# eriksandstroem/Loopy-SLAM

Measured on AMD Instinct MI355X. Metric: rays/s (track+map, Replica room0 per-frame budget, 640x480 synthetic RGB-D), higher is better.
Workload: dtype f32 (decoder products as split products on the 16-bit matrix pipe: fp16x3 forward, bf16x6 / pre-scaled fp16x3 backward, fp32 accumulate; weight gradients on pre-scaled fp16x3 too); 1 GPU; Replica room0 budget: 40 track it x 1500 rays + 60 map it x 5000 rays per frame (24 geometry + 36 colour) on the frustum rows of the mapped frame, S=5, k=8, C=32, rel-pos colour MLP, N=99999 points laid down by radius-de-duplicated insertion (lk_add_points, r_add 0.04), 640x480 synthetic room

## Files before the change

### include/loopy_hip.h

```cpp
#ifndef LOOPY_HIP_H
#define LOOPY_HIP_H

#include <stdint.h>

#ifdef __cplusplus
extern "C" {
#endif

#define LK_ABI_VERSION 1
#define LK_K 8
#define LK_C 32
#define LK_S_MAX 8

#define LK_OK 0
#define LK_ERR_ARG (-1)
#define LK_ERR_HIP (-2)
#define LK_ERR_STATE (-3)
#define LK_ERR_RANGE (-4)

typedef struct lk_knn_s* lk_knn_t;

int lk_version(void);
const char* lk_last_error(void);

// ... 94 lines not shown
    float loss_w_color;
} lk_render_desc;

int64_t lk_render_act_floats(int32_t R, int32_t S, uint32_t flags);
int64_t lk_render_bwd_scratch_floats(int32_t R, int32_t S, uint32_t flags);
int lk_render_fwd(const lk_render_desc* d, void* stream);
int lk_render_bwd(const lk_render_desc* d, void* stream);

#define LK_TRACK_USE_COLOR   1
#define LK_TRACK_MEDIAN_MASK 2
int lk_loss_mapper(int32_t R, const float* depth, const float* color, const uint8_t* valid_ray,
                   const float* gt_depth, const float* gt_color, float w_color, int32_t use_color,
                   float* d_depth, float* d_color, float* out_loss, void* stream);
int lk_loss_tracker(int32_t R, const float* depth, const float* var, const float* color,
                    const float* gt_depth, const float* gt_color, float w_color, int32_t use_color,
                    float* d_depth, float* d_color, float* out_loss, float* scratch , void* stream);

#define LK_ADAM_MAX_SEG 16
typedef struct {
    float* p; float* g; float* m; float* v;
    int64_t n;
    float lr; int32_t step;
    const int32_t* row_index;
    int32_t row_len;
    int32_t zero_grad;
    int32_t p_f16;
    const uint8_t* row_flags;
    int32_t g_compact;
} lk_adam_seg;
int lk_adam_step(const lk_adam_seg* host_segs, int32_t n_seg, float beta1, float beta2, float eps, void* stream);

#define LK_EXPOSURE_MAX_F 32
#define LK_EXPOSURE_GRAD_FLOATS (1024 + 128 + 1536 + 12 + LK_EXPOSURE_MAX_F * 8)
int lk_exposure_fwd(const float* feats, const float* W1, const float* b1, const float* W2, const float* b2, int32_t F,
                    float* aff, float* hid, void* stream);
int lk_exposure_bwd(const float* feats, const float* W1, const float* W2, const float* hid, const float* g_aff, int32_t F,
                    float* g, void* stream);
int lk_loss_mapper_exposure(int32_t R, const float* depth, const float* logits, const uint8_t* valid_ray, const float* gt_depth,
                            const float* gt_color, const int32_t* frame_id, const float* aff, int32_t F, float w_color,
                            float* d_depth, float* d_logits, float* out_loss, float* g_aff, void* stream);

typedef struct lk_copy_seg {
    float* data;
    int64_t n;
    const int32_t* row_index;
    int32_t row_len;
} lk_copy_seg;
int lk_bucket_copy(const lk_copy_seg* host_segs, int32_t n_seg, float* bucket, int32_t unpack, void* stream);

int lk_rays_from_pose(const float* cam7, const float* pix_i, const float* pix_j, int32_t R,
                      float fx, float fy, float cx, float cy, float* rays_o, float* rays_d, void* stream);
int lk_gather_rays(const float* depth_stack, const float* color_stack, const float* c2w_stack, int32_t c2w_stride,
                   const float* r2_map_stack, const int32_t* frame_id, const int32_t* rnd, int32_t R,
                   int32_t H, int32_t W, int32_t H0, int32_t W0, int32_t w, float fx, float fy, float cx, float cy,
                   float* rays_o, float* rays_d, float* gt_depth, float* gt_color, float* pix_i, float* pix_j,
                   float* r2_ray, void* stream);
int lk_pose_bwd(const float* cam7, const float* pix_i, const float* pix_j, int32_t R,
                float fx, float fy, float cx, float cy, const float* g_rays_o, const float* g_rays_d,
                float* g_cam7, void* stream);
int lk_compact(const uint8_t* mask, int32_t n, int32_t* out_index, int32_t* out_count, void* stream);
int lk_compact_large(const uint8_t* mask, int32_t n, int32_t* out_index, int32_t* out_count, int32_t* block_scratch, void* stream);
int lk_touch_rows(const int32_t* nbr_idx, int64_t n, uint8_t* flags, int32_t N, void* stream);
int lk_knn_flag_rows(lk_knn_t knn, const uint8_t* flags, int64_t n, void* stream);
int lk_frustum_rows(const float* pos, int32_t N, const float* w2c12_host, const float* depth, int32_t H, int32_t W,
                    float fx, float fy, float cx, float cy, int32_t edge, float* scratch_depth, uint8_t* scratch_mask,
                    uint32_t* scratch_max, int32_t* out_index, int32_t* out_count, void* stream);
int lk_add_points(lk_knn_t knn, const float* rays_o, const float* rays_d, const float* gt_depth, int32_t n,
                  float r2_static, const float* r2_per_ray, float near_surface, float far_surface, int32_t n_add,
                  uint8_t* scratch_mask, int32_t* out_ray_index, int32_t* out_count, float* out_points, void* stream);
int lk_radius_maps(const float* color, int32_t H, int32_t W, double color_grad_threshold, double radius_add_max,
                   double radius_add_min, double radius_query_ratio, float* grad_mag, float* r2_add, float* r2_query, void* stream);
int lk_top_grad_pixels(const float* grad_mag, int32_t H, int32_t W, int32_t K, int32_t H0, int32_t H1, int32_t W0, int32_t W1,
                       const float* depth, int32_t depth_limit, int32_t* out_index, int32_t* out_count, void* stream);
int lk_inside_mask(const float* depth, int32_t n, uint8_t* mask, float* depth_filtered, float* out_thr,
                   uint32_t* scratch, void* stream);

typedef struct {
    float* feats;
    float* W1; float* b1; float* W2; float* b2;
    int32_t F;
    float* aff;
    float* hid;
    float* g_aff;
    float* g;
    float* adam;
    float lr_mlp;
    float lr_feat;
    int32_t feat_first, feat_count;
    float* bwd_scale;
} lk_exposure_desc;

typedef struct {
    lk_render_desc render;
    const float* depth_img;
    const float* color_img;
    const float* r2_map;
    int32_t H, W, H0, W0, w;
    float fx, fy, cx, cy;
    const int32_t* rnd;
    float* gt_color;
    float* pix_i; float* pix_j;
    float* thr;
    uint32_t* scratch_u32;
    float* loss_scratch;
    float* cam7;
    float* g_cam7;
    float* adam_mv;
    float lr_T, lr_q;
    float w_color; int32_t use_color;
    int32_t hist_post;
    float* hist;
    float* log;
    int32_t iters;
    float* work;
    const lk_exposure_desc* exposure;
} lk_track_desc;
int64_t lk_track_work_floats(int32_t R, int32_t S, int32_t iters);
int lk_track_frame(const lk_track_desc* d, void* stream);

#define LK_MAX_SPANS 8
typedef struct { int64_t offset, n; } lk_blob_span;
typedef struct {
    lk_render_desc render;
    const float* depth_stack; const float* color_stack; const float* c2w_stack; int32_t c2w_stride;
    const float* r2_map_stack;
    const int32_t* frame_id;
    const int32_t* rnd;
    int32_t H, W, H0, W0, w;
    float fx, fy, cx, cy;
    float* gt_color; float* thr; uint32_t* scratch_u32;
    float w_color;
    float* log;
    float* weights_rw;
    float* weights_frag_rw;
    float* geo_feats_rw; float* col_feats_rw;
    const int32_t* rows;
    int64_t n_rows;
    float* adam_rows;
    lk_blob_span geo_dec[LK_MAX_SPANS]; int32_t n_geo_dec;
    lk_blob_span col_dec[LK_MAX_SPANS]; int32_t n_col_dec;
    float* adam_dec;
    float lr[2][3];
    int32_t iters, n_geo_iters;
    float* work;
    const lk_exposure_desc* exposure;
    const float* grad_bucket;
    int64_t bucket_geo_dec[LK_MAX_SPANS], bucket_col_dec[LK_MAX_SPANS];
    int64_t bucket_geo_rows, bucket_col_rows;
    int32_t union_rows_flagged;
    int32_t it_offset;
    int32_t batches_ready;
    int32_t train_geo_decoder;
    int32_t signal_rows;
} lk_map_desc;
int64_t lk_map_work_floats(int32_t R, int32_t S, int32_t iters);
int lk_map_prepare(const lk_map_desc* d, void* stream);
int64_t lk_map_work_nbr_idx(int32_t R, int32_t S, int32_t iters);
int lk_map_frame(const lk_map_desc* d, int32_t it_begin, int32_t it_end, int32_t phases, void* stream);
int lk_map_wait_lists(const lk_map_desc* d, int32_t it, void* stream);
int lk_map_wait_rows(const lk_map_desc* d, void* stream);

int lk_wgrad_single(const float* A, int32_t lda, int32_t a_mode, const float* A2, int32_t lda2,
                    const float* B, int32_t ldb, int32_t N, int32_t K, int64_t rows,
                    float* dW, int32_t ldw, float* db, int32_t chunk, void* stream);

int lk_normals(lk_knn_t knn, const float* pos, int64_t N, float radius, const float* host_camera3,
               float* out_normals , uint8_t* out_valid , void* stream);
#define LK_ICP_POINT_TO_PLANE 0
#define LK_ICP_INFORMATION 1
#define LK_ICP_SUMS 32
int64_t lk_icp_scratch_floats(int64_t P);
int lk_icp_accumulate(lk_knn_t tgt, const float* tgt_pos, const float* tgt_normals, const uint8_t* tgt_valid, const float* src,
                      int64_t P, const float* host_T12, float max_dist, float tukey_k, int32_t mode, int32_t* out_corr,
                      float* scratch, int64_t scratch_floats, double* out_sums, void* stream);
int lk_apply_correction(float* pos, int64_t N, const int32_t* seg_id, const float* mats, int32_t n_seg, void* stream);

#define LK_VOXEL_AXIS_MAX 2097151
int lk_voxel_keys(const float* pos, int64_t N, const float* host_origin3, float voxel, int64_t* out_keys, void* stream);
int lk_voxel_heads(const int64_t* sorted_keys, int64_t N, uint8_t* out_head, void* stream);
int lk_voxel_downsample(const float* pos, int64_t N, const int64_t* order , const int32_t* starts ,
                        int32_t n_vox, float* out_centroids , void* stream);
int lk_knn_canonicalize(lk_knn_t knn, void* stream);
#define LK_FPFH_DIM 33
int lk_fpfh(lk_knn_t knn, const float* pos, const float* normals, const uint8_t* valid, int64_t N, float radius,
            float* out_spfh , float* out_fpfh , void* stream);
int lk_feature_match(const float* A, const uint8_t* validA, int64_t Na, const float* B, const uint8_t* validB, int64_t Nb,
                     int32_t* out_idx, float* out_d2, void* stream);
#define LK_RANSAC_BEST 20
int lk_ransac_gather(const float* src, const float* tgt, const int32_t* corr, int32_t M, float* out_cs, float* out_ct, void* stream);
int lk_ransac_hypotheses(const float* cs, const float* ct, int32_t M, uint64_t seed, uint64_t trial0, int32_t n_trials, float edge_ratio,
                         float dist_thr, int32_t* out_triples, uint8_t* out_ok, float* out_T, void* stream);
int lk_ransac_score(const float* cs, const float* ct, int32_t M, const float* T_all, const int32_t* survivors, const int32_t* n_survivors,
                    int32_t max_survivors, float dist_thr, int32_t* out_count, float* out_sum_d2, void* stream);
int lk_ransac_best(const int32_t* count, const float* sum_d2, const int32_t* survivors, const int32_t* n_survivors, const float* T_all,
                   uint64_t trial0, int32_t* best, void* stream);

int lk_tsdf_touch(const float* depth, int32_t H, int32_t W, const float* host_c2w16, float fx, float fy, float cx, float cy, int32_t stride,
                  float depth_trunc, float sdf_trunc, float voxel, int64_t* out_keys , void* stream);
int lk_tsdf_integrate(float* planes, const int64_t* slot_keys, int32_t n_slots, const int32_t* touched_slots, int32_t n_touched,
                      const float* depth, const float* color, int32_t H, int32_t W, const float* host_c2w16, float fx, float fy, float cx,
                      float cy, float voxel, float sdf_trunc, float depth_trunc, void* stream);
int lk_mc_mark(const float* planes, const int32_t* sorted_slots, const int32_t* nbr, int32_t n_blocks, uint8_t* out_case, uint8_t* out_ntri,
               uint8_t* edge_flag, void* stream);
int lk_mc_vertices(const float* planes, const int64_t* slot_keys, const int32_t* sorted_slots, const int32_t* nbr, int32_t n_blocks,
                   const int32_t* vert_index, int32_t V, float voxel, float* out_pos , float* out_col , void* stream);
int lk_mc_triangles(const int32_t* sorted_slots, const int32_t* nbr, int32_t n_blocks, const uint8_t* cube_case, const int32_t* tri_end,
                    const int32_t* vert_index, int32_t V, int32_t* out_tri , void* stream);

int lk_nearest(lk_knn_t knn, const float* queries, int64_t P, float max_dist, float* out_d2, int32_t* out_idx, void* stream);
int lk_mesh_areas(const float* verts, int64_t V, const int32_t* faces, int64_t F, float* out_area, void* stream);
int lk_mesh_sample(const float* verts, int64_t V, const int32_t* faces, int64_t F, const double* cum_area, uint64_t seed, int64_t S,
                   float* out_pos , int32_t* out_face , float* out_bary , void* stream);
int lk_mesh_cull(const float* points, int64_t N, const float* w2c, int32_t n_poses, int32_t H, int32_t W, float fx, float fy, float cx, float cy,
                 uint8_t* seen, void* stream);
int lk_mesh_depth_setup(const float* verts, int64_t V, const int32_t* faces, int64_t F, const float* host_w2c12, int32_t H, int32_t W, float fx,
                        float fy, float cx, float cy, float near, float far, float* out_rec, int32_t* out_box, int32_t* out_ntiles,
                        float* out_depth , void* stream);
int lk_mesh_depth_raster(const float* rec, const int32_t* box, const int32_t* tile_end, int64_t F, int64_t T, int32_t H, int32_t W, float fx,
                         float fy, float cx, float cy, float near, float far, float* depth , void* stream);

int lk_profile_begin(const char* names);
int lk_set_serial(int32_t on);
int lk_streams_init(void);
int lk_profile_end(char* buf, int cap);
int lk_debug_occupancy(int32_t out[5]);
int lk_debug_side_delay(int32_t us);

#ifdef __cplusplus
}
#endif
#endif
```

### loopy_slam_amd/_ffi.py

```python
import ctypes as C
import os

_HERE = os.path.dirname(os.path.abspath(__file__))
LIB_PATH = os.path.join(_HERE, 'libloopyhip.so')

LK_K = 8
LK_C = 32
LK_S_MAX = 8

FLAG_STAGE_COLOR = 1 << 0
FLAG_TRACKER = 1 << 1
FLAG_REL_POS = 1 << 2
FLAG_COLOR_LOGITS = 1 << 3
FLAG_SAVE_ACT = 1 << 4
FLAG_GRAD_FEATS = 1 << 5
FLAG_GRAD_WEIGHTS = 1 << 6
FLAG_GRAD_RAYS = 1 << 7
FLAG_ALL_DEPTH_POS = 1 << 8
FLAG_ZERO_ABSENT = 1 << 9
FLAG_MAPPER_LOSS = 1 << 10
FLAG_Z_GIVEN = 1 << 12
FLAG_FEATS_F16 = 1 << 13
FLAG_UNIT_LOSS_GRADS = 1 << 11
FLAG_EMBED_GRADS_ONLY = 1 << 14
FLAG_GRAD_GEO_DECODER = 1 << 15
FLAG_CHECK_RANGE = 1 << 16
STATUS_WEIGHT_RANGE, STATUS_ACT_RANGE = 1, 2
ERR_RANGE = -4

EXPOSURE_MAX_F = 32
ICP_POINT_TO_PLANE, ICP_INFORMATION, ICP_SUMS = 0, 1, 32
FPFH_DIM, RANSAC_BEST = 33, 20
ADAM_MAX_SEG = 16

_fp = C.c_void_p


class WeightEntry(C.Structure):
    _fields_ = [('name', C.c_char * 64), ('offset', C.c_int64), ('rows', C.c_int32), ('cols', C.c_int32),
                ('ld', C.c_int32), ('col_split', C.c_int32), ('col_shift', C.c_int32)]


class RenderDesc(C.Structure):
    _fields_ = [
        ('R', C.c_int32), ('S', C.c_int32), ('stats_chunk', C.c_int32), ('flags', C.c_uint32),
        ('rays_o', _fp), ('rays_d', _fp), ('gt_depth', _fp), ('r2_ray', _fp),
        ('knn', _fp), ('pos', _fp), ('geo_feats', _fp), ('col_feats', _fp), ('weights', _fp), ('weights_frag', _fp),
        ('affine', _fp), ('noise_geo', _fp), ('noise_col', _fp),
        ('near_surface', C.c_float), ('far_surface', C.c_float), ('near_end', C.c_float), ('coef', C.c_float),
        ('r2_static', C.c_float), ('min_nn', C.c_int32),
        ('depth', _fp), ('var', _fp), ('color', _fp), ('valid_ray', _fp),
        ('z', _fp), ('nbr_idx', _fp), ('nbr_w', _fp), ('nbr_count', _fp), ('c_geo', _fp), ('c_col', _fp),
        ('raw', _fp), ('far_stats', _fp), ('act', _fp),
        ('d_depth', _fp), ('d_var', _fp), ('d_color', _fp),
        ('g_geo_feats', _fp), ('g_col_feats', _fp), ('g_weights', _fp), ('g_rays_o', _fp), ('g_rays_d', _fp),
        ('g_affine', _fp), ('grad_row_mask', _fp), ('bwd_scratch', _fp), ('bwd_scratch_cap', C.c_int64),
        ('loss_gt_color', _fp), ('loss_out4', _fp), ('loss_w_color', C.c_float),
    ]


class AdamSeg(C.Structure):
    _fields_ = [('p', _fp), ('g', _fp), ('m', _fp), ('v', _fp), ('n', C.c_int64), ('lr', C.c_float),
                ('step', C.c_int32), ('row_index', _fp), ('row_len', C.c_int32), ('zero_grad', C.c_int32), ('p_f16', C.c_int32),
                ('row_flags', _fp), ('g_compact', C.c_int32)]


class CopySeg(C.Structure):
    _fields_ = [('data', _fp), ('n', C.c_int64), ('row_index', _fp), ('row_len', C.c_int32)]


MAX_SPANS = 8


class BlobSpan(C.Structure):
    _fields_ = [('offset', C.c_int64), ('n', C.c_int64)]


EXPOSURE_GRAD_FLOATS = 1024 + 128 + 1536 + 12 + EXPOSURE_MAX_F * 8


class ExposureDesc(C.Structure):
    _fields_ = [('feats', _fp), ('W1', _fp), ('b1', _fp), ('W2', _fp), ('b2', _fp), ('F', C.c_int32),
                ('aff', _fp), ('hid', _fp), ('g_aff', _fp), ('g', _fp), ('adam', _fp),
                ('lr_mlp', C.c_float), ('lr_feat', C.c_float), ('feat_first', C.c_int32), ('feat_count', C.c_int32), ('bwd_scale', _fp)]


class TrackDesc(C.Structure):
    _fields_ = [
        ('render', RenderDesc),
        ('depth_img', _fp), ('color_img', _fp), ('r2_map', _fp),
        ('H', C.c_int32), ('W', C.c_int32), ('H0', C.c_int32), ('W0', C.c_int32), ('w', C.c_int32),
        ('fx', C.c_float), ('fy', C.c_float), ('cx', C.c_float), ('cy', C.c_float),
        ('rnd', _fp), ('gt_color', _fp), ('pix_i', _fp), ('pix_j', _fp), ('thr', _fp), ('scratch_u32', _fp), ('loss_scratch', _fp),
        ('cam7', _fp), ('g_cam7', _fp), ('adam_mv', _fp),
        ('lr_T', C.c_float), ('lr_q', C.c_float), ('w_color', C.c_float), ('use_color', C.c_int32), ('hist_post', C.c_int32),
        ('hist', _fp), ('log', _fp), ('iters', C.c_int32), ('work', _fp), ('exposure', C.POINTER(ExposureDesc)),
    ]


class MapDesc(C.Structure):
    _fields_ = [
        ('render', RenderDesc),
        ('depth_stack', _fp), ('color_stack', _fp), ('c2w_stack', _fp), ('c2w_stride', C.c_int32), ('r2_map_stack', _fp),
        ('frame_id', _fp), ('rnd', _fp),
        ('H', C.c_int32), ('W', C.c_int32), ('H0', C.c_int32), ('W0', C.c_int32), ('w', C.c_int32),
        ('fx', C.c_float), ('fy', C.c_float), ('cx', C.c_float), ('cy', C.c_float),
        ('gt_color', _fp), ('thr', _fp), ('scratch_u32', _fp),
        ('w_color', C.c_float), ('log', _fp),
        ('weights_rw', _fp), ('weights_frag_rw', _fp), ('geo_feats_rw', _fp), ('col_feats_rw', _fp),
        ('rows', _fp), ('n_rows', C.c_int64), ('adam_rows', _fp),
        ('geo_dec', BlobSpan * MAX_SPANS), ('n_geo_dec', C.c_int32),
        ('col_dec', BlobSpan * MAX_SPANS), ('n_col_dec', C.c_int32),
        ('adam_dec', _fp),
        ('lr', (C.c_float * 3) * 2),
        ('iters', C.c_int32), ('n_geo_iters', C.c_int32), ('work', _fp), ('exposure', C.POINTER(ExposureDesc)),
        ('grad_bucket', _fp), ('bucket_geo_dec', C.c_int64 * MAX_SPANS), ('bucket_col_dec', C.c_int64 * MAX_SPANS),
        ('bucket_geo_rows', C.c_int64), ('bucket_col_rows', C.c_int64),
        ('union_rows_flagged', C.c_int32), ('it_offset', C.c_int32), ('batches_ready', C.c_int32), ('train_geo_decoder', C.c_int32), ('signal_rows', C.c_int32),
    ]


class LoopyError(RuntimeError):
    pass


class LoopyLib:

    def __init__(self, path):
        if not os.path.exists(path):
            raise LoopyError(f'{path} not found: build it with `python loopy_slam_amd/csrc/build.py` '
                             f'(or __graft_entry__.build()); there is no CPU fallback')
        self.path = path
        import torch
        self.dll = C.CDLL(path)
        d = self.dll
        d.lk_version.restype = C.c_int
        d.lk_last_error.restype = C.c_char_p
        d.lk_knn_create.argtypes = [C.c_float, C.c_int64, C.c_int64, C.POINTER(C.c_void_p)]
        d.lk_knn_destroy.argtypes = [C.c_void_p]
        d.lk_knn_build.argtypes = [C.c_void_p, _fp, C.c_int64, C.c_void_p]
        d.lk_knn_append.argtypes = [C.c_void_p, _fp, C.c_int64, C.c_void_p]
        d.lk_knn_size.argtypes = [C.c_void_p]
        d.lk_knn_size.restype = C.c_int64
        d.lk_knn_query.argtypes = [C.c_void_p, _fp, C.c_int64, C.c_float, _fp, _fp, _fp, _fp, C.c_void_p]
        d.lk_weight_layout.argtypes = [C.POINTER(WeightEntry), C.c_int]
        d.lk_weight_blob_floats.restype = C.c_int64
        d.lk_weight_frag_floats.restype = C.c_int64
        d.lk_weights_repack.argtypes = [_fp, _fp, C.c_void_p]
        d.lk_render_act_floats.argtypes = [C.c_int32, C.c_int32, C.c_uint32]
        d.lk_render_act_floats.restype = C.c_int64
        d.lk_render_fwd.argtypes = [C.POINTER(RenderDesc), C.c_void_p]
        for name, argtypes, restype in (
            ('lk_render_bwd_scratch_floats', [C.c_int32, C.c_int32, C.c_uint32], C.c_int64),
            ('lk_render_bwd', [C.POINTER(RenderDesc), C.c_void_p], C.c_int),
            ('lk_loss_mapper', [C.c_int32, _fp, _fp, _fp, _fp, _fp, C.c_float, C.c_int32, _fp, _fp, _fp, C.c_void_p], C.c_int),
            ('lk_loss_tracker', [C.c_int32, _fp, _fp, _fp, _fp, _fp, C.c_float, C.c_int32, _fp, _fp, _fp, _fp, C.c_void_p], C.c_int),
            ('lk_adam_step', [C.POINTER(AdamSeg), C.c_int32, C.c_float, C.c_float, C.c_float, C.c_void_p], C.c_int),
            ('lk_bucket_copy', [C.POINTER(CopySeg), C.c_int32, C.c_void_p, C.c_int32, C.c_void_p], C.c_int),
            ('lk_exposure_fwd', [_fp] * 5 + [C.c_int32, _fp, _fp, C.c_void_p], C.c_int),
            ('lk_exposure_bwd', [_fp] * 5 + [C.c_int32, _fp, C.c_void_p], C.c_int),
            ('lk_loss_mapper_exposure', [C.c_int32] + [_fp] * 7 + [C.c_int32, C.c_float, _fp, _fp, _fp, _fp, C.c_void_p], C.c_int),
            ('lk_rays_from_pose', [_fp, _fp, _fp, C.c_int32, C.c_float, C.c_float, C.c_float, C.c_float, _fp, _fp, C.c_void_p], C.c_int),
            ('lk_pose_bwd', [_fp, _fp, _fp, C.c_int32, C.c_float, C.c_float, C.c_float, C.c_float, _fp, _fp, _fp, C.c_void_p], C.c_int),
            ('lk_gather_rays', [_fp, _fp, _fp, C.c_int32, _fp, _fp, _fp, C.c_int32, C.c_int32, C.c_int32, C.c_int32, C.c_int32,
                                C.c_int32, C.c_float, C.c_float, C.c_float, C.c_float, _fp, _fp, _fp, _fp, _fp, _fp, _fp,
                                C.c_void_p], C.c_int),
            ('lk_frustum_rows', [_fp, C.c_int32, C.POINTER(C.c_float), _fp, C.c_int32, C.c_int32, C.c_float, C.c_float, C.c_float,
                                 C.c_float, C.c_int32, _fp, _fp, _fp, _fp, _fp, C.c_void_p], C.c_int),
            ('lk_add_points', [C.c_void_p, _fp, _fp, _fp, C.c_int32, C.c_float, _fp, C.c_float, C.c_float, C.c_int32,
                               _fp, _fp, _fp, _fp, C.c_void_p], C.c_int),
            ('lk_radius_maps', [_fp, C.c_int32, C.c_int32, C.c_double, C.c_double, C.c_double, C.c_double, _fp, _fp, _fp, C.c_void_p], C.c_int),
            ('lk_top_grad_pixels', [_fp, C.c_int32, C.c_int32, C.c_int32, C.c_int32, C.c_int32, C.c_int32, C.c_int32, _fp, C.c_int32,
                                    _fp, _fp, C.c_void_p], C.c_int),
            ('lk_wgrad_single', [_fp, C.c_int32, C.c_int32, _fp, C.c_int32, _fp, C.c_int32, C.c_int32, C.c_int32, C.c_int64,
                                 _fp, C.c_int32, _fp, C.c_int32, C.c_void_p], C.c_int),
            ('lk_profile_begin', [C.c_char_p], C.c_int),
            ('lk_profile_end', [C.c_char_p, C.c_int], C.c_int),
            ('lk_compact', [_fp, C.c_int32, _fp, _fp, C.c_void_p], C.c_int),
            ('lk_set_serial', [C.c_int32], C.c_int),
            ('lk_streams_init', [], C.c_int),
            ('lk_debug_occupancy', [C.POINTER(C.c_int32)], C.c_int),
            ('lk_debug_side_delay', [C.c_int32], C.c_int),
            ('lk_weights_repack_checked', [_fp, _fp, C.c_void_p], C.c_int),
            ('lk_status_peek', [C.POINTER(C.c_uint32)], C.c_int),
            ('lk_status_sync', [C.c_void_p, C.POINTER(C.c_uint32)], C.c_int),
            ('lk_status_clear', [], C.c_int),
            ('lk_track_work_floats', [C.c_int32, C.c_int32, C.c_int32], C.c_int64),
            ('lk_map_work_floats', [C.c_int32, C.c_int32, C.c_int32], C.c_int64),
            ('lk_map_work_nbr_idx', [C.c_int32, C.c_int32, C.c_int32], C.c_int64),
            ('lk_track_frame', [C.POINTER(TrackDesc), C.c_void_p], C.c_int),
            ('lk_map_frame', [C.POINTER(MapDesc), C.c_int32, C.c_int32, C.c_int32, C.c_void_p], C.c_int),
            ('lk_map_prepare', [C.POINTER(MapDesc), C.c_void_p], C.c_int),
            ('lk_inside_mask', [_fp, C.c_int32, _fp, _fp, _fp, _fp, C.c_void_p], C.c_int),
            ('lk_compact_large', [_fp, C.c_int32, _fp, _fp, _fp, C.c_void_p], C.c_int),
            ('lk_touch_rows', [_fp, C.c_int64, _fp, C.c_int32, C.c_void_p], C.c_int),
            ('lk_knn_flag_rows', [C.c_void_p, _fp, C.c_int64, C.c_void_p], C.c_int),
            ('lk_map_wait_lists', [C.POINTER(MapDesc), C.c_int32, C.c_void_p], C.c_int),
            ('lk_map_wait_rows', [C.POINTER(MapDesc), C.c_void_p], C.c_int),
            ('lk_normals', [C.c_void_p, _fp, C.c_int64, C.c_float, C.POINTER(C.c_float), _fp, _fp, C.c_void_p], C.c_int),
            ('lk_icp_scratch_floats', [C.c_int64], C.c_int64),
            ('lk_icp_accumulate', [C.c_void_p, _fp, _fp, _fp, _fp, C.c_int64, C.POINTER(C.c_float), C.c_float, C.c_float, C.c_int32, _fp,
                                   _fp, C.c_int64, _fp, C.c_void_p], C.c_int),
            ('lk_apply_correction', [_fp, C.c_int64, _fp, _fp, C.c_int32, C.c_void_p], C.c_int),
            ('lk_voxel_keys', [_fp, C.c_int64, C.POINTER(C.c_float), C.c_float, _fp, C.c_void_p], C.c_int),
            ('lk_voxel_heads', [_fp, C.c_int64, _fp, C.c_void_p], C.c_int),
            ('lk_voxel_downsample', [_fp, C.c_int64, _fp, _fp, C.c_int32, _fp, C.c_void_p], C.c_int),
            ('lk_knn_canonicalize', [C.c_void_p, C.c_void_p], C.c_int),
            ('lk_fpfh', [C.c_void_p, _fp, _fp, _fp, C.c_int64, C.c_float, _fp, _fp, C.c_void_p], C.c_int),
            ('lk_feature_match', [_fp, _fp, C.c_int64, _fp, _fp, C.c_int64, _fp, _fp, C.c_void_p], C.c_int),
            ('lk_ransac_gather', [_fp, _fp, _fp, C.c_int32, _fp, _fp, C.c_void_p], C.c_int),
            ('lk_ransac_hypotheses', [_fp, _fp, C.c_int32, C.c_uint64, C.c_uint64, C.c_int32, C.c_float, C.c_float, _fp, _fp, _fp,
                                      C.c_void_p], C.c_int),
            ('lk_ransac_score', [_fp, _fp, C.c_int32, _fp, _fp, _fp, C.c_int32, C.c_float, _fp, _fp, C.c_void_p], C.c_int),
            ('lk_ransac_best', [_fp, _fp, _fp, _fp, _fp, C.c_uint64, _fp, C.c_void_p], C.c_int),
            ('lk_tsdf_touch', [_fp, C.c_int32, C.c_int32, C.POINTER(C.c_float), C.c_float, C.c_float, C.c_float, C.c_float, C.c_int32,
                               C.c_float, C.c_float, C.c_float, _fp, C.c_void_p], C.c_int),
            ('lk_tsdf_integrate', [_fp, _fp, C.c_int32, _fp, C.c_int32, _fp, _fp, C.c_int32, C.c_int32, C.POINTER(C.c_float), C.c_float,
                                   C.c_float, C.c_float, C.c_float, C.c_float, C.c_float, C.c_float, C.c_void_p], C.c_int),
            ('lk_mc_mark', [_fp, _fp, _fp, C.c_int32, _fp, _fp, _fp, C.c_void_p], C.c_int),
            ('lk_mc_vertices', [_fp, _fp, _fp, _fp, C.c_int32, _fp, C.c_int32, C.c_float, _fp, _fp, C.c_void_p], C.c_int),
            ('lk_mc_triangles', [_fp, _fp, C.c_int32, _fp, _fp, _fp, C.c_int32, _fp, C.c_void_p], C.c_int),
            ('lk_nearest', [C.c_void_p, _fp, C.c_int64, C.c_float, _fp, _fp, C.c_void_p], C.c_int),
            ('lk_mesh_areas', [_fp, C.c_int64, _fp, C.c_int64, _fp, C.c_void_p], C.c_int),
            ('lk_mesh_sample', [_fp, C.c_int64, _fp, C.c_int64, _fp, C.c_uint64, C.c_int64, _fp, _fp, _fp, C.c_void_p], C.c_int),
            ('lk_mesh_cull', [_fp, C.c_int64, _fp, C.c_int32, C.c_int32, C.c_int32, C.c_float, C.c_float, C.c_float, C.c_float, _fp,
                              C.c_void_p], C.c_int),
            ('lk_mesh_depth_setup', [_fp, C.c_int64, _fp, C.c_int64, C.POINTER(C.c_float), C.c_int32, C.c_int32, C.c_float, C.c_float,
                                     C.c_float, C.c_float, C.c_float, C.c_float, _fp, _fp, _fp, _fp, C.c_void_p], C.c_int),
            ('lk_mesh_depth_raster', [_fp, _fp, _fp, C.c_int64, C.c_int64, C.c_int32, C.c_int32, C.c_float, C.c_float, C.c_float, C.c_float,
                                      C.c_float, C.c_float, _fp, C.c_void_p], C.c_int),
        ):
            if hasattr(d, name):
                fn = getattr(d, name)
                fn.argtypes = argtypes
                fn.restype = restype
        if d.lk_version() != 1:
            raise LoopyError(f'{path}: ABI version {d.lk_version()} != 1')

    def check(self, rc, what=''):
        if rc != 0:
            raise LoopyError(f'{what} failed (rc={rc}): {self.dll.lk_last_error().decode()}')

    def weight_layout(self):
        n = self.dll.lk_weight_layout(None, 0)
        arr = (WeightEntry * n)()
        self.dll.lk_weight_layout(arr, n)
        return [dict(name=e.name.decode(), offset=e.offset, rows=e.rows, cols=e.cols, ld=e.ld,
                     col_split=e.col_split, col_shift=e.col_shift) for e in arr]

    def blob_floats(self):
        return int(self.dll.lk_weight_blob_floats())


_LIB = None


def get_lib():
    global _LIB
    if _LIB is None:
        import torch
        if not torch.cuda.is_available():
            raise LoopyError('loopy_slam_amd needs a HIP device (MI355X); none is visible and there is no CPU fallback')
        _LIB = LoopyLib(LIB_PATH)
    return _LIB


def ptr(t):
    return 0 if t is None else t.data_ptr()
```

### loopy_slam_amd/csrc/lk_adam_dev.h

```cpp
#pragma once
#include "lk_common.h"
#include "lk_kernels.h"

__device__ __forceinline__ float lk_adam_elem(float p, float g, float& m, float& v, float b1, float b2, float eps, float step_size, float bc2_sqrt) {
    m = m * b1 + (1.0f - b1) * g;
    v = v * b2 + (1.0f - b2) * (g * g);
    const float denom = sqrtf(v) / bc2_sqrt + eps;
    return p - step_size * (m / denom);
}

__device__ __forceinline__ void lk_adam_one(const AdamSegDev& S, long long i, long long e, float b1, float b2, float eps) {
    const float g = S.g[S.g_compact ? i : e];
    float m = S.m[i], v = S.v[i];
    if (S.p_f16) {
        _Float16* ph = reinterpret_cast<_Float16*>(S.p) + e;
        *ph = (_Float16)lk_adam_elem((float)*ph, g, m, v, b1, b2, eps, S.step_size, S.bc2_sqrt);
    } else {
        S.p[e] = lk_adam_elem(S.p[e], g, m, v, b1, b2, eps, S.step_size, S.bc2_sqrt);
    }
    S.m[i] = m;
    S.v[i] = v;
    if (S.zero_grad && !S.g_compact) S.g[e] = 0.0f;
}
__device__ __forceinline__ void lk_adam_seg_flagged(const AdamSegDev& S, float b1, float b2, float eps, int bx, int gx) {
    const int lane = (int)threadIdx.x & 63;
    const long long n_rows = S.n / S.row_len;
    const long long wave = (long long)bx * 4 + ((int)threadIdx.x >> 6), n_waves = (long long)gx * 4;
    const bool pair = S.row_len <= 32;
    int RW = 64;
    while (RW > 2 && n_rows < n_waves * RW) RW >>= 1;
    for (long long r0 = wave * RW; r0 < n_rows; r0 += n_waves * RW) {
        const bool on = lane < RW && r0 + lane < n_rows && S.row_flags[r0 + lane] != 0;
        unsigned long long mask = __ballot(on);
        while (mask) {
            const int ra = __ffsll((long long)mask) - 1;
            mask &= mask - 1;
            int rb = -1;
            if (pair && mask) { rb = __ffsll((long long)mask) - 1; mask &= mask - 1; }
            const int half = lane >> 5;
            const int row = pair ? (half ? rb : ra) : ra;
            const int k = pair ? (lane & 31) : lane;
            if (row >= 0 && k < S.row_len) {
                const long long e = (r0 + row) * S.row_len + k;
                lk_adam_one(S, e, e, b1, b2, eps);
            }
        }
    }
}
__device__ __forceinline__ void lk_adam_seg_block(const AdamSegDev& S, float b1, float b2, float eps, int bx, int gx) {
    if (S.row_flags) { lk_adam_seg_flagged(S, b1, b2, eps, bx, gx); return; }
    for (long long i = (long long)bx * 256 + threadIdx.x; i < S.n; i += (long long)gx * 256) {
        long long e = i;
        if (S.row_index) {
            const long long row = i / S.row_len;
            e = (long long)S.row_index[row] * S.row_len + (i - row * S.row_len);
        }
        lk_adam_one(S, i, e, b1, b2, eps);
    }
}
```

### loopy_slam_amd/csrc/lk_api.hip

```cpp
#include "lk_common.h"
#include "lk_kernels.h"

#include <stdarg.h>
#include <stdio.h>
#include <string.h>
#include <stdlib.h>

using namespace lkw;

static thread_local char g_err[512] = "";

void lk_set_error(const char* fmt, ...) {
    va_list ap;
    va_start(ap, fmt);
    vsnprintf(g_err, sizeof(g_err), fmt, ap);
    va_end(ap);
}

extern "C" int lk_version(void) { return LK_ABI_VERSION; }

namespace {
struct StatusWord { volatile unsigned* host = nullptr; unsigned* dev = nullptr; bool tried = false; };
StatusWord& status_word() {
    static StatusWord w;
// ... 416 lines not shown
    SideStream& ss = side_stream();
    LkFeatScatterArgs fs;
    seg_args(d, P, fs);
    if (gf && !(skip & LK_SEG_SORTED)) {
        const int rc2 = seg_sort_async(d, P, false, st);
        if (rc2 != LK_OK) return rc2;
    }

    LkCompositeBwdArgs cb;
    cb.R = d->R; cb.S = d->S; cb.min_nn = d->min_nn; cb.coef = d->coef;
    cb.raw = d->raw; cb.z = d->z; cb.nbr_count = d->nbr_count; cb.gt_depth = d->gt_depth;
    cb.d_depth = d->d_depth; cb.d_var = d->d_var; cb.d_color = color ? d->d_color : nullptr;
    cb.d_raw = S0 + L.d_raw; cb.keep_depth = (flags & LK_FLAG_Z_GIVEN) ? 1 : 0;
    const bool cb_inline = !(skip & LK_SKIP_COMPOSITE_BWD) && !(gw && (flags & LK_FLAG_GRAD_GEO_DECODER));
    if (!(skip & LK_SKIP_COMPOSITE_BWD) && !cb_inline) lk_launch_composite_bwd(cb, st);

    const bool fuse_small = (skip & LK_FUSE_SMALL) && relpos && gr && !gw && !gf && lk_cdiv(P, 32) <= LK_DEEP_MAX_TILES;
    bool fuse_rb = false;
    LkRelposBwdArgs rb_fused;
    LkDecodeBwdArgs db;
    db.R = d->R; db.S = d->S; db.P = P; db.flags = flags;
    db.rays_o = d->rays_o; db.rays_d = d->rays_d; db.z = d->z;
    db.W = d->weights; db.Wfrag = d->weights_frag; db.affine = d->affine;
    db.act = d->act; db.raw = d->raw; db.d_raw = S0 + L.d_raw;
    db.dc_geo = S0 + L.dc_geo; db.dc_col = S0 + L.dc_col; db.dy_col = S0 + L.dy_col; db.dlogit = S0 + L.dlogit;
    db.dp_embed = S0 + L.dp_embed; db.dp_embed_col = S0 + L.dp_embed_col; db.g_weights = d->g_weights; db.g_affine = d->g_affine; db.g_affine_part = S0 + L.aff_part; db.part_bg = S0 + L.part_bg;
    db.live_rays = ex ? ex->live_rays : nullptr;
    db.dscale = ex ? ex->dscale : nullptr;
    db.tl_n_part = 0;
    memset(&db.tl, 0, sizeof(db.tl));
    db.cb_on = cb_inline ? 1 : 0; db.cb = cb;
    db.ml_on = 0; db.ml_row_part = nullptr;
    memset(&db.ml, 0, sizeof(db.ml));
    if ((skip & LK_COMPOSITE_IN_BWD) && (flags & LK_FLAG_MAPPER_LOSS)) {
        LK_REQUIRE(ex && ex->loss_rows && d->d_depth && d->d_color && d->loss_gt_color && (skip & LK_SKIP_COMPOSITE_BWD),
                   "lk_render_bwd: the composite inside the decoder backward needs loss_rows, loss_gt_color, d_depth, d_color");
        LkCompositeArgs& ca = db.ml;
        ca.R = d->R; ca.S = d->S; ca.min_nn = d->min_nn; ca.coef = d->coef;
        ca.raw = d->raw; ca.z = d->z; ca.nbr_count = d->nbr_count; ca.gt_depth = d->gt_depth;
        ca.depth = d->depth; ca.var = d->var; ca.color = d->color; ca.valid_ray = d->valid_ray;
        ca.keep_depth = (flags & LK_FLAG_Z_GIVEN) ? 1 : 0;
        ca.gt_color = d->loss_gt_color; ca.w_color = d->loss_w_color; ca.use_color = color ? 1 : 0;
        ca.d_depth = const_cast<float*>(d->d_depth); ca.d_color = const_cast<float*>(d->d_color);
        db.ml_on = 1; db.ml_row_part = ex->loss_rows;
    }
    if (ex && ex->track_loss) {
        LK_REQUIRE((flags & LK_FLAG_GRAD_RAYS) != 0 && ex->track_n_part > 0, "lk_render_bwd: the inline tracker loss needs ray gradients");
        db.tl = *ex->track_loss; db.tl_n_part = ex->track_n_part;
    }
    lk_launch_decode_bwd(db, st);
    if (gw && (flags & LK_FLAG_GRAD_GEO_DECODER)) {
        LK_REQUIRE(!(flags & LK_FLAG_EMBED_GRADS_ONLY), "lk_render_bwd: GRAD_GEO_DECODER does not combine with EMBED_GRADS_ONLY");
        rc = lk_launch_geo_wgrad(P, d->S, d->rays_o, d->rays_d, d->z, d->weights, d->act, d->c_geo, S0 + L.d_raw, S0 + L.geo_part, d->g_weights, st,
                                 ex ? ex->live_rays : nullptr);
        if (rc != LK_OK) return rc;
    }
    if (color && d->affine && d->g_affine && !(skip & LK_SKIP_AFF_REDUCE)) lk_launch_reduce_partials(S0 + L.aff_part, lk_cdiv(P, 32), 12, d->g_affine, st);
    const bool gwf = gw && !(flags & LK_FLAG_EMBED_GRADS_ONLY);
    const bool defer = gwf && color && (!relpos || lk_relpos_fused(flags));
    LkWgradArgs wdef;
    wdef.n_units = 0; wdef.part = nullptr;
    const bool bg_rides = gw && !defer && gf;
    if (gw && !defer && !bg_rides) lk_launch_reduce_partials(S0 + L.part_bg, lk_cdiv(lk_cdiv(P, 32), 4), 288, d->g_weights + G_EB, st);

    const bool dw2_rides = gf && gwf && relpos && lk_relpos_fused(flags);
    const bool forked = gwf && color && ss.ok;
    const bool split = forked && defer && ex && ex->split_reduce && ex->step && ex->step->n_span > 0 && ex->split_frag && ex->split_master;
    if (ex && ex->split_done) *ex->split_done = split ? 1 : 0;
    hipStream_t wst = st;
    if (forked) {
        (void)hipEventRecord(ss.fork, st);
        (void)hipStreamWaitEvent(ss.st, ss.fork, 0);
        wst = ss.st;
    }
    if (gwf && color) {
        const float* act_h = d->act + (size_t)P * (LK_ACT_GEO_A + LK_ACT_COL_A);
        const float* act_e = d->act + (size_t)P * (LK_ACT_GEO_A + LK_ACT_COL_A + LK_ACT_COL_H);
        const float* dy = S0 + L.dy_col;
        float* G = d->g_weights;
        LkWgradArgs wa;
        memset(&wa, 0, sizeof(wa));
        int nj = 0;
        const int w_off[5] = {C_W0, C_W1, C_W2, C_W3, C_W4}, b_off[5] = {C_B0, C_B1, C_B2, C_B3, C_B4};
        const int w_ld[5] = {EC, HC, HC, EC + HC, HC};
        auto fc_from = [&](LkWgradJob& J, int src, int layer, const float* Wsrc, int rows_u, int ldw, int off) {
            J.k_aux = J.K;
            if (J.B2) { J.B3 = d->c_col; J.ldb3 = LK_C; J.k_split2 = J.K; }
            else { J.B2 = d->c_col; J.ldb2 = LK_C; J.k_split = J.K; }
            J.K += CF;
            LkFcPost& F = wa.fc[wa.n_fc++];
            F.src_job = src; F.rows_u = rows_u; F.ldw = ldw; F.off = off; F.W = Wsrc;
            F.dU = G + C_U0 + layer * C_USTRIDE; F.du = F.dU + a64(HC * CF);
        };
        for (int i = 0; i < 5; ++i) {
            LkWgradJob& J = wa.job[nj++];
            J.A = dy + LK_COL_LAYER(P, i); J.lda = 128; J.a_mode = 0;
            if (i == 0) { J.B = act_e; J.ldb = LK_ACT_COL_E; }
            else if (i == 3) { J.B = act_e; J.ldb = LK_ACT_COL_E; J.B2 = act_h + LK_COL_LAYER(P, 2); J.ldb2 = 128; J.k_split = EC; }
            else { J.B = act_h + LK_COL_LAYER(P, i - 1); J.ldb = 128; }
            J.N = HC; J.K = w_ld[i]; J.rows = P; J.dW = G + w_off[i]; J.ldw = w_ld[i]; J.db = G + b_off[i];
            if (i >= 1) fc_from(J, nj - 1, i - 1, d->weights + w_off[i], HC, w_ld[i], i == 3 ? EC : 0);
        }
        {
            LkWgradJob& J = wa.job[nj++];
            J.A = S0 + L.dlogit; J.lda = 4; J.a_mode = 0;
            J.B = act_h + LK_COL_LAYER(P, 4); J.ldb = 128;
            J.N = 3; J.K = HC; J.rows = P; J.dW = G + C_WO; J.ldw = HC; J.db = G + C_BO;
            fc_from(J, nj - 1, 4, d->weights + C_WO, 3, HC, 0);
        }
        wa.n_jobs = nj; wa.chunk = 0; wa.part = S0 + L.wg_part;
        wa.h16 = (flags & LK_FLAG_UNIT_LOSS_GRADS) && !gr ? 1 : 0;
        wa.live_rays = ex ? ex->live_rays : nullptr; wa.S = d->S; wa.dscale = ex ? ex->dscale : nullptr;
        if (forked && g_side_delay_us > 0) hipLaunchKernelGGL(k_spin_us, dim3(1), dim3(64), 0, wst, (long long)g_side_delay_us * 100);
        lk_launch_wgrad(wa, P, wst, defer ? &wdef : nullptr);
        if (split) {
            LkBwdReduceArgs rt;
            memset(&rt, 0, sizeof(rt));
            lk_launch_bwd_reduce(wdef, rt, false, wst, ex->step, false);
            lk_launch_repack_trunk(ex->step->w_next, ex->split_master, ex->split_frag, wst);
        }
    }

    if (relpos) {
        LkRelposBwdArgs rb;
        rb.R = d->R; rb.S = d->S; rb.P = P; rb.min_nn = d->min_nn; rb.flags = flags;
        rb.rays_o = d->rays_o; rb.rays_d = d->rays_d; rb.z = d->z; rb.pos = d->pos; rb.col_feats = d->col_feats;
        rb.nbr_idx = d->nbr_idx; rb.nbr_w = d->nbr_w; rb.nbr_count = d->nbr_count;
        rb.W = d->weights; rb.Wfrag = d->weights_frag; rb.dc_col = S0 + L.dc_col;
        rb.g_col_feats = d->g_col_feats; rb.g_weights = d->g_weights;
        rb.dw_rel = S0 + L.dw_rel; rb.dp_rel = S0 + L.dp_rel; rb.rows = S0 + L.rows; rb.w_eff = S0 + L.w_eff;
        rb.dfeat = S0 + L.dfeat;
        rb.part_br = S0 + L.part_br; rb.hbar = S0 + L.hbar; rb.w_sum = S0 + L.w_sum; rb.dw1_part = S0 + L.dw1_part;
        rb.live_rays = (ex && lk_relpos_fused(flags)) ? ex->live_rays : nullptr;
        fuse_rb = fuse_small;
        if (fuse_rb) rb_fused = rb;
        else lk_launch_relpos_bwd(rb, st);
        if (forked && !lk_relpos_fused(flags)) { (void)hipEventRecord(ss.mid, st); (void)hipStreamWaitEvent(wst, ss.mid, 0); }
        if (gw && !defer) lk_launch_reduce_partials(S0 + L.part_br, lk_relpos_fused(flags) ? lk_relpos_bwd_parts(P) : lk_cdiv(lk_cdiv(P, 4), 4), 32,
                                                    d->g_weights + R_EB, st);
    }

    if (gf) {
        fs.dc_geo = S0 + L.dc_geo; fs.dc_col = (color && !relpos) ? S0 + L.dc_col : nullptr; fs.dfeat = relpos ? S0 + L.dfeat : nullptr;
        fs.g_geo_feats = d->g_geo_feats; fs.g_col_feats = d->g_col_feats;
        if (ex && ex->seg_list) { fs.seg_list = ex->seg_list; fs.seg_total = ex->seg_total; }
        else if (ss.ok) (void)hipStreamWaitEvent(st, ss.link, 0);
        fs.act_flag = ex ? ex->act_flag : nullptr;
        if (bg_rides) { fs.red_part = S0 + L.part_bg; fs.red_n = lk_cdiv(lk_cdiv(P, 32), 4); fs.red_width = 288; fs.red_out = d->g_weights + G_EB; }
        if (dw2_rides) {
            fs.dw2_dc = S0 + L.dc_col; fs.dw2_w_sum = S0 + L.w_sum; fs.dw2_hbar = S0 + L.hbar; fs.dw2_part = S0 + L.dw2_part;
            fs.dw2_blocks = lk_dw2_parts(P); fs.dw2_live = ex ? ex->live_rays : nullptr; fs.dw2_S = d->S;
        }
        if (ex && ex->xstep) { fs.x_on = 1; fs.x = *ex->xstep; }
        lk_launch_feat_scatter(fs, st);
        if (ex && ex->signal_rows) {
            const int rc3 = rows_event_record(st);
            if (rc3 != LK_OK) return rc3;
        }
    }
    if (gr) {
        LkInterpBwdArgs ib;
        ib.R = d->R; ib.S = d->S; ib.P = P; ib.min_nn = d->min_nn; ib.flags = flags;
        ib.rays_o = d->rays_o; ib.rays_d = d->rays_d; ib.z = d->z; ib.r2_ray = d->r2_ray; ib.r2_static = d->r2_static;
        ib.pos = d->pos; ib.geo_feats = d->geo_feats; ib.col_feats = d->col_feats;
        ib.nbr_idx = d->nbr_idx; ib.nbr_w = d->nbr_w; ib.nbr_count = d->nbr_count;
        ib.dc_geo = S0 + L.dc_geo; ib.dc_col = S0 + L.dc_col;
        ib.dw_rel = relpos ? S0 + L.dw_rel : nullptr;
        ib.dp_embed = S0 + L.dp_embed; ib.dp_embed_col = color ? S0 + L.dp_embed_col : nullptr; ib.dp_rel = relpos ? S0 + L.dp_rel : nullptr;
        ib.g_geo_feats = d->g_geo_feats; ib.g_col_feats = d->g_col_feats; ib.dp_total = S0 + L.dp_total;
        ib.pose_part = ex ? ex->pose_part : nullptr;
        if (ex) { ib.pix_i = ex->pix_i; ib.pix_j = ex->pix_j; ib.fx = ex->fx; ib.fy = ex->fy; ib.cx = ex->cx; ib.cy = ex->cy; }
        else { ib.pix_i = ib.pix_j = nullptr; ib.fx = ib.fy = 1.0f; ib.cx = ib.cy = 0.0f; }
        if (fuse_rb) lk_launch_relpos_interp_bwd(rb_fused, ib, st, (flags & LK_FLAG_UNIT_LOSS_GRADS) && d->affine == nullptr);
        else lk_launch_interp_bwd(ib, st, (ex && !gf) ? ex->xstep : nullptr, ex ? ex->xstep_part : nullptr, ex ? ex->xstep_n_part : 0);
    }
    if (gr && !(skip & LK_SKIP_RAYS_BWD)) {
        LkRaysBwdArgs rr;
        rr.R = d->R; rr.S = d->S; rr.z = d->z; rr.dp_total = S0 + L.dp_total; rr.g_rays_o = d->g_rays_o; rr.g_rays_d = d->g_rays_d;
        lk_launch_rays_bwd(rr, st);
    }
    if (gwf && relpos) {
        float* G = d->g_weights;
        if (lk_relpos_fused(flags)) {
            LkRelposBwdArgs rb;
            memset(&rb, 0, sizeof(rb));
            rb.P = P; rb.S = d->S; rb.dc_col = S0 + L.dc_col; rb.w_sum = S0 + L.w_sum; rb.hbar = S0 + L.hbar; rb.dw1_part = S0 + L.dw1_part;
            rb.live_rays = ex ? ex->live_rays : nullptr;
            if (!dw2_rides) lk_launch_dw2_hbar(rb, S0 + L.dw2_part, st);
        } else {
            LkWgradArgs wr;
            memset(&wr, 0, sizeof(wr));
            const float* rows = S0 + L.rows;
            LkWgradJob& J1 = wr.job[0];
            J1.A = rows; J1.lda = 192; J1.a_mode = 0; J1.B = rows + 128; J1.ldb = 192;
            J1.N = HC; J1.K = KR; J1.rows = 8 * P; J1.dW = G + R_W1; J1.ldw = KRP; J1.db = G + R_B1;
            LkWgradJob& J2 = wr.job[1];
            J2.A = S0 + L.dc_col; J2.lda = LK_C; J2.a_mode = 2; J2.A2 = S0 + L.w_sum; J2.lda2 = 1;
            J2.B = S0 + L.hbar; J2.ldb = 128;
            J2.N = CF; J2.K = HC; J2.rows = P; J2.dW = G + R_W2; J2.ldw = HC; J2.db = G + R_B2;
            wr.n_jobs = 2; wr.chunk = 0; wr.part = S0 + L.wg_part;
            lk_launch_wgrad(wr, 8 * P, wst);
        }
    }
    if (forked) {
        LK_HIP_TRY(hipEventRecord(ss.join, wst));
        if (!split) LK_HIP_TRY(hipStreamWaitEvent(st, ss.join, 0));
    }
    if (defer) {
        float* G = d->g_weights;
        LkBwdReduceArgs r;
        memset(&r, 0, sizeof(r));
        const bool with_rp = relpos;
        if (with_rp) {
            r.part1 = S0 + L.dw1_part; r.n1 = lk_relpos_bwd_parts(P); r.part2 = S0 + L.dw2_part; r.n2 = lk_dw2_parts(P);
            r.dW1 = G + R_W1; r.db1 = G + R_B1; r.dW2 = G + R_W2; r.db2 = G + R_B2;
            r.part_br = S0 + L.part_br; r.n_br = lk_relpos_bwd_parts(P); r.out_br = G + R_EB;
        }
        r.part_bg = S0 + L.part_bg; r.n_bg = lk_cdiv(lk_cdiv(P, 32), 4); r.out_bg = G + G_EB;
        if (split) {
            LkWgradArgs none;
            memset(&none, 0, sizeof(none));
            lk_launch_bwd_reduce(none, r, with_rp, st, ex->step, true);
        } else lk_launch_bwd_reduce(wdef, r, with_rp, st, ex ? ex->step : nullptr);
    }
    LK_LAUNCH_CHECK();
    return LK_OK;
}

extern "C" int lk_wgrad_single(const float* A, int32_t lda, int32_t a_mode, const float* A2, int32_t lda2,
                               const float* B, int32_t ldb, int32_t N, int32_t K, int64_t rows,
                               float* dW, int32_t ldw, float* db, int32_t chunk, void* stream_) {
    LK_REQUIRE(A && B && dW && N > 0 && N <= 128 && K > 0 && K <= 192 && rows >= 0 && chunk >= 32, "lk_wgrad_single: bad arguments");
    LK_REQUIRE((N % 4 == 0 || lda >= ((N + 3) / 4) * 4) && K % 4 == 0 && lda % 4 == 0 && ldb % 4 == 0, "lk_wgrad_single: rows must be float4-addressable");
    if (rows == 0) return LK_OK;
    LkWgradArgs wa;
    memset(&wa, 0, sizeof(wa));
    LkWgradJob& J = wa.job[0];
    J.A = A; J.lda = lda; J.a_mode = a_mode; J.A2 = A2; J.lda2 = lda2; J.B = B; J.ldb = ldb;
    J.N = N; J.K = K; J.rows = (int)rows; J.dW = dW; J.ldw = ldw; J.db = db;
    wa.n_jobs = 1; wa.chunk = chunk;
    lk_launch_wgrad(wa, (int)rows, (hipStream_t)stream_);
    LK_LAUNCH_CHECK();
    return LK_OK;
}

#include <vector>
#include <string>
namespace {
const char* kKernelNames[LKK_COUNT] = {"k_depth_stats", "k_sample_interp", "k_relpos_fwd", "k_decode_fwd", "k_composite",
                                       "k_composite_bwd", "k_decode_bwd", "k_relpos_bwd", "k_interp_bwd", "k_rays_bwd", "k_wgrad", "k_feat_gather", "k_decode_bwd_track"};
struct ProfState {
    bool on = false;
    bool enabled[LKK_COUNT] = {};
    std::vector<hipEvent_t> ev0[LKK_COUNT], ev1[LKK_COUNT];
};
ProfState g_prof;
}

void lk_prof_before(int kid, hipStream_t st) {
    if (!g_prof.on || !g_prof.enabled[kid]) return;
    hipEvent_t e0, e1;
    if (hipEventCreate(&e0) != hipSuccess || hipEventCreate(&e1) != hipSuccess) return;
    g_prof.ev0[kid].push_back(e0);
    g_prof.ev1[kid].push_back(e1);
    (void)hipEventRecord(e0, st);
}
void lk_prof_after(int kid, hipStream_t st) {
    if (!g_prof.on || !g_prof.enabled[kid] || g_prof.ev1[kid].empty()) return;
    (void)hipEventRecord(g_prof.ev1[kid].back(), st);
}

extern "C" int lk_profile_begin(const char* names) {
    LK_REQUIRE(names != nullptr, "lk_profile_begin: NULL names");
    const std::string s(names);
    for (int k = 0; k < LKK_COUNT; ++k) {
        g_prof.enabled[k] = (s == "*") || (("," + s + ",").find(std::string(",") + kKernelNames[k] + ",") != std::string::npos);
        g_prof.ev0[k].clear();
        g_prof.ev1[k].clear();
    }
    g_prof.on = true;
    return LK_OK;
}

extern "C" int lk_profile_end(char* buf, int cap) {
    g_prof.on = false;
    std::string out;
    for (int k = 0; k < LKK_COUNT; ++k) {
        double total = 0.0;
        const size_t n = g_prof.ev0[k].size();
        for (size_t i = 0; i < n; ++i) {
            float ms = 0.0f;
            (void)hipEventSynchronize(g_prof.ev1[k][i]);
            if (hipEventElapsedTime(&ms, g_prof.ev0[k][i], g_prof.ev1[k][i]) == hipSuccess) total += ms;
            (void)hipEventDestroy(g_prof.ev0[k][i]);
            (void)hipEventDestroy(g_prof.ev1[k][i]);
        }
        g_prof.ev0[k].clear();
        g_prof.ev1[k].clear();
        if (n) {
            char line[160];
            snprintf(line, sizeof(line), "%s %zu %.6f\n", kKernelNames[k], n, total);
            out += line;
        }
    }
    if (buf && cap > 0) {
        strncpy(buf, out.c_str(), (size_t)cap - 1);
// ... 5 lines not shown
```

### loopy_slam_amd/csrc/lk_bwd2.hip

```cpp
#include "lk_common.h"
#include "lk_kernels.h"
#include "lk_adam_dev.h"
#include "lk_exposure_dev.h"

using namespace lkw;

LK_CHAIN_DEFINE(bwd2)

__device__ __forceinline__ void interp_bwd_block(const LkInterpBwdArgs& a, int block) {
    const int sub = (int)threadIdx.x & 7;
    const int p_raw = block * 32 + ((int)threadIdx.x >> 3);
    const bool live = p_raw < a.P;
    const int pidx = live ? p_raw : a.P - 1;
    const bool has = a.nbr_count[pidx] >= a.min_nn;
    const bool color = (a.flags & LK_FLAG_STAGE_COLOR) != 0;
    const bool relpos = (a.flags & LK_FLAG_REL_POS) != 0;
    const bool do_col = color && !relpos;
    int id[LK_K];
    float w[LK_K];
    {
        const int4 i0 = *reinterpret_cast<const int4*>(a.nbr_idx + (size_t)pidx * LK_K);
        const int4 i1 = *reinterpret_cast<const int4*>(a.nbr_idx + (size_t)pidx * LK_K + 4);
        const float4 w0 = *reinterpret_cast<const float4*>(a.nbr_w + (size_t)pidx * LK_K);
        const float4 w1 = *reinterpret_cast<const float4*>(a.nbr_w + (size_t)pidx * LK_K + 4);
        id[0] = i0.x; id[1] = i0.y; id[2] = i0.z; id[3] = i0.w; id[4] = i1.x; id[5] = i1.y; id[6] = i1.z; id[7] = i1.w;
        w[0] = w0.x; w[1] = w0.y; w[2] = w0.z; w[3] = w0.w; w[4] = w1.x; w[5] = w1.y; w[6] = w1.z; w[7] = w1.w;
    }
    const float4 dcg = *reinterpret_cast<const float4*>(a.dc_geo + (size_t)pidx * LK_C + sub * 4);
    float4 dcc = make_float4(0.f, 0.f, 0.f, 0.f);
    if (do_col) dcc = *reinterpret_cast<const float4*>(a.dc_col + (size_t)pidx * LK_C + sub * 4);
    if (!(a.flags & LK_FLAG_GRAD_RAYS)) return;
    float dwn[LK_K];
#pragma unroll
    for (int j = 0; j < LK_K; ++j) {
        float part = 0.0f;
        if (has && w[j] != 0.0f) {
            const float4 g = lk_feat4(a.geo_feats, (a.flags & LK_FLAG_FEATS_F16) != 0, (size_t)id[j] * LK_C + sub * 4);
            part = dcg.x * g.x + dcg.y * g.y + dcg.z * g.z + dcg.w * g.w;
            if (do_col) {
                const float4 c = lk_feat4(a.col_feats, (a.flags & LK_FLAG_FEATS_F16) != 0, (size_t)id[j] * LK_C + sub * 4);
                part += dcc.x * c.x + dcc.y * c.y + dcc.z * c.z + dcc.w * c.w;
            }
        }
        part = lk_sum8<true>(part);
        if (color && relpos && a.dw_rel && has) part += a.dw_rel[(size_t)pidx * LK_K + j];
        dwn[j] = part;
    }
    LK_STAMPW(7);
    const int r = pidx / a.S;
    const float z = a.z[pidx];
    const float px = lk_madd_rn(a.rays_o[3 * r], a.rays_d[3 * r], z);
    const float py = lk_madd_rn(a.rays_o[3 * r + 1], a.rays_d[3 * r + 1], z);
    const float pz = lk_madd_rn(a.rays_o[3 * r + 2], a.rays_d[3 * r + 2], z);
    const float r2 = a.r2_ray ? a.r2_ray[r] : a.r2_static;
    float dpx = 0.0f, dpy = 0.0f, dpz = 0.0f;
    if (has) {
        float wr[LK_K], ex[LK_K], ey[LK_K], ez[LK_K];
        float S = 0.0f, dot = 0.0f;
#pragma unroll
        for (int j = 0; j < LK_K; ++j) {
            wr[j] = 0.0f; ex[j] = ey[j] = ez[j] = 0.0f;
            if (id[j] >= 0) {
                const float x = a.pos[3 * (size_t)id[j]], y = a.pos[3 * (size_t)id[j] + 1], zz = a.pos[3 * (size_t)id[j] + 2];
                const float D = lk_dist2(px, py, pz, x, y, zz);
                if (D <= r2) { wr[j] = 1.0f / (D + 1e-10f); ex[j] = x - px; ey[j] = y - py; ez[j] = zz - pz; }
            }
            S += wr[j];
            dot += dwn[j] * w[j];
        }
        const float invS = 1.0f / fmaxf(S, 1e-12f);
#pragma unroll
        for (int j = 0; j < LK_K; ++j) {
            if (wr[j] != 0.0f) {
                const float dw = (dwn[j] - dot) * invS;
                const float dD = -wr[j] * wr[j] * dw;
                dpx += dD * (-2.0f) * ex[j]; dpy += dD * (-2.0f) * ey[j]; dpz += dD * (-2.0f) * ez[j];
            }
        }
    }
    if (live && sub == 0) {
        if (a.dp_embed) { const float4 e = *reinterpret_cast<const float4*>(a.dp_embed + (size_t)pidx * 4); dpx += e.x; dpy += e.y; dpz += e.z; }
        if (color && a.dp_embed_col) { const float4 e = *reinterpret_cast<const float4*>(a.dp_embed_col + (size_t)pidx * 4); dpx += e.x; dpy += e.y; dpz += e.z; }
        if (color && relpos && a.dp_rel) { const float4 e = *reinterpret_cast<const float4*>(a.dp_rel + (size_t)pidx * 4); dpx += e.x; dpy += e.y; dpz += e.z; }
        *reinterpret_cast<float4*>(a.dp_total + (size_t)pidx * 4) = make_float4(dpx, dpy, dpz, 0.0f);
    }
    LK_STAMPW(8);
    if (a.pose_part) {
        __shared__ float s_pp[4][12];
        float v[12];
        const bool mine = live && sub == 0;
        const float d0 = mine ? (a.pix_i[r] - a.cx) / a.fx : 0.0f, d1 = mine ? -(a.pix_j[r] - a.cy) / a.fy : 0.0f, d2 = mine ? -1.0f : 0.0f;
        const float gx = mine ? dpx : 0.0f, gy = mine ? dpy : 0.0f, gz = mine ? dpz : 0.0f;
        const float zx = gx * z, zy = gy * z, zz = gz * z;
        v[0] = zx * d0; v[1] = zx * d1; v[2] = zx * d2; v[3] = zy * d0; v[4] = zy * d1; v[5] = zy * d2; v[6] = zz * d0; v[7] = zz * d1; v[8] = zz * d2;
        v[9] = gx; v[10] = gy; v[11] = gz;
#pragma unroll
        for (int q = 0; q < 12; ++q) {
#pragma unroll
            for (int o = 32; o >= 8; o >>= 1) v[q] += __shfl_xor(v[q], o);
        }
        const int wv = (int)threadIdx.x >> 6;
        if (lk_lane() == 0) {
#pragma unroll
            for (int q = 0; q < 12; ++q) s_pp[wv][q] = v[q];
        }
        __syncthreads();
        if (threadIdx.x < 12) a.pose_part[(size_t)block * 12 + threadIdx.x] = (s_pp[0][threadIdx.x] + s_pp[1][threadIdx.x]) + (s_pp[2][threadIdx.x] + s_pp[3][threadIdx.x]);
    }
    LK_STAMPW(9);
}
__global__ __launch_bounds__(256) void k_interp_bwd(LkInterpBwdArgs a) { interp_bwd_block(a, (int)blockIdx.x); }
__global__ __launch_bounds__(256) void k_interp_bwd_x(LkInterpBwdArgs a, ExposureStepArgs xa, const float* __restrict__ part, int n_part) {
    if (blockIdx.x + 1 == gridDim.x) { lk_exposure_step_body(xa, part, n_part); return; }
    interp_bwd_block(a, (int)blockIdx.x);
}

__global__ __launch_bounds__(256) void k_seg_count(LkFeatScatterArgs a) {
    const long long row = (long long)blockIdx.x * 256 + (int)threadIdx.x;
    if (row >= (long long)a.P * LK_K) return;
    const int y = (int)blockIdx.y;
    const long long grow = (long long)y * a.P * LK_K + row;
    const int s = (int)(row >> 3);
    const int idx = a.nbr_idx[grow];
    int rk = -1;
    const bool skipped = a.live_rays && s >= a.live_rays[y] * a.S;
    if (!skipped && idx >= 0 && a.nbr_w[grow] != 0.0f && a.nbr_count[(size_t)y * a.P + s] >= a.min_nn && (!a.row_mask || a.row_mask[idx])) {
        const int key = a.key_of ? a.key_of[idx] : idx;
        if (key >= 0) rk = atomicAdd(a.seg_cnt + (size_t)y * a.cnt_stride + key, 1);
    }
    a.seg_rank[grow] = rk;
}
__global__ __launch_bounds__(256) void k_seg_place(LkFeatScatterArgs a) {
    const long long row = (long long)blockIdx.x * 256 + (int)threadIdx.x;
    if (row >= (long long)a.P * LK_K) return;
    const int y = (int)blockIdx.y;
    const long long base = (long long)y * a.P * LK_K;
    const int32_t* __restrict__ off = a.seg_off + (size_t)y * a.cnt_stride;
    const int rk = a.seg_rank[base + row];
    if (rk >= 0) {
        const int idx = a.nbr_idx[base + row];
        a.seg_list[base + off[a.key_of ? a.key_of[idx] : idx] + rk] = (int)row;
    }
    if (row == 0 && a.seg_total) a.seg_total[y] = off[a.N];
}

__global__ __launch_bounds__(256) void k_seg_order(LkFeatScatterArgs a) {
    const long long i = (long long)blockIdx.x * 256 + (int)threadIdx.x;
    const int y = (int)blockIdx.y;
    const int32_t* __restrict__ off = a.seg_off + (size_t)y * a.cnt_stride;
    if (i >= off[a.N]) return;
    const long long base = (long long)y * a.P * LK_K;
    const int32_t* __restrict__ tmp = a.seg_tmp + base;
    const int row = tmp[i];
    const int idx = a.nbr_idx[base + row];
    const int key = a.key_of ? a.key_of[idx] : idx;
    const int s = off[key], e = off[key + 1];
    int rk = 0;
    for (int j = s; j < e; ++j) rk += tmp[j] < row;
    a.seg_list[base + s + rk] = row;
}

#define LK_DW2_LDS_SAMPLES 32
__device__ __forceinline__ void dw2_body(const float* __restrict__ dc, const float* __restrict__ w_sum, const float* __restrict__ hbar,
                                         int P_all, const int32_t* __restrict__ live_rays, int S, float* __restrict__ part, int bx, int nb) {
    const int P = live_rays ? min(P_all, *live_rays * S) : P_all;
    __shared__ __attribute__((aligned(16))) float s_h[LK_DW2_LDS_SAMPLES][128];
    __shared__ float s_a[LK_DW2_LDS_SAMPLES][33];
    const int t = (int)threadIdx.x, n = t >> 3, k0 = 16 * (t & 7);
    float acc[16], bsum = 0.0f;
#pragma unroll
    for (int i = 0; i < 16; ++i) acc[i] = 0.0f;
    for (int s0 = bx * 64; s0 < P; s0 += nb * 64) {
        for (int half = 0; half < 64; half += LK_DW2_LDS_SAMPLES) {
            const int ns = min(LK_DW2_LDS_SAMPLES, P - s0 - half);
            if (ns <= 0) break;
            __syncthreads();
#pragma unroll
            for (int q = 0; q < LK_DW2_LDS_SAMPLES * 32 / 256; ++q) {
                const int e = q * 256 + t, sm = e >> 5;
                float4 v = make_float4(0.f, 0.f, 0.f, 0.f);
                float av = 0.0f;
                if (sm < ns) {
                    v = reinterpret_cast<const float4*>(hbar + (size_t)(s0 + half + sm) * 128)[e & 31];
                    av = w_sum[s0 + half + sm] * dc[(size_t)(s0 + half + sm) * LK_C + (e & 31)];
                }
                reinterpret_cast<float4*>(&s_h[sm][0])[e & 31] = v;
                s_a[sm][e & 31] = av;
            }
            __syncthreads();
#pragma unroll 4
            for (int sm = 0; sm < LK_DW2_LDS_SAMPLES; ++sm) {
                const float av = s_a[sm][n];
                const float4* __restrict__ hb = reinterpret_cast<const float4*>(&s_h[sm][k0]);
                bsum += av;
#pragma unroll
                for (int q = 0; q < 4; ++q) {
                    const float4 v = hb[q];
                    acc[4 * q] = fmaf(av, v.x, acc[4 * q]); acc[4 * q + 1] = fmaf(av, v.y, acc[4 * q + 1]);
                    acc[4 * q + 2] = fmaf(av, v.z, acc[4 * q + 2]); acc[4 * q + 3] = fmaf(av, v.w, acc[4 * q + 3]);
                }
            }
        }
    }
    float* __restrict__ out = part + (size_t)bx * (32 * 129) + n * 129;
#pragma unroll
    for (int i = 0; i < 16; ++i) out[k0 + i] = acc[i];
    if (k0 == 0) out[128] = bsum;
}
#define LK_GATHER_CHUNK 16
#define LK_GATHER_WINDOW 32
#define LK_GATHER_BATCH 8
__device__ __forceinline__ void col_reduce_body(const float* __restrict__ part, int n_parts, int width, float* __restrict__ out, int bx, float (*sh)[32],
                                                const LkStepRider& sr);
__device__ __forceinline__ void lk_arrived(float v) { asm volatile("" : : "v"(v)); }
template <int MODE>
__device__ __forceinline__ void feat_walk(const LkFeatScatterArgs& a, int bx) {
    constexpr bool col = MODE != 0;
    const int c = (int)threadIdx.x & 31;
    const long long i0l = ((long long)bx * 8 + ((int)threadIdx.x >> 5)) * LK_GATHER_CHUNK;
    const int total = a.seg_total ? *a.seg_total : a.seg_off[a.N];
    if (i0l >= total) return;
    const int i0 = (int)i0l, e = min(i0 + LK_GATHER_CHUNK, total);
    const float* __restrict__ tab_c = MODE == 2 ? a.dfeat : a.dc_col;
    int cur = -1, carry = -1;
    float sg = 0.0f, sc = 0.0f;
    for (int wb = i0;; wb += LK_GATHER_WINDOW) {
        const int row = a.seg_list[min(wb + c, total - 1)];
        const int before = (wb == i0 && c == 0 && i0 > 0) ? a.seg_list[i0 - 1] : -1;
        const int pt = a.nbr_idx[row];
        const float w = a.nbr_w[row];
        if (before >= 0) carry = a.nbr_idx[before];
        int prev = __shfl_up(pt, 1, 32);
        if (c == 0) prev = carry;
        unsigned m = (wb + c >= total || pt != prev) ? 1u << c : 0u;
#pragma unroll
        for (int o = 16; o >= 1; o >>= 1) m |= __shfl_xor(m, o, 32);
        int u0 = 0;
        if (wb == i0) {
            const unsigned head = m & ((1u << (e - i0)) - 1u);
            if (!head) return;
            u0 = __builtin_ctz(head);
        }
        const unsigned tail = wb == i0 ? m & ~((1u << (e - i0)) - 1u) : m;
        const int u1 = tail ? __builtin_ctz(tail) : LK_GATHER_WINDOW;
        for (int ub = u0; ub < u1; ub += LK_GATHER_BATCH) {
            float vg[LK_GATHER_BATCH], vc[LK_GATHER_BATCH], wr[LK_GATHER_BATCH];
#pragma unroll
            for (int k = 0; k < LK_GATHER_BATCH; ++k) {
                const int uu = min(ub + k, u1 - 1);
                const int r = __shfl(row, uu, 32);
                wr[k] = __shfl(w, uu, 32);
                const size_t s = (size_t)(r >> 3) * LK_C + c;
                vg[k] = a.dc_geo[s];
                if (col) vc[k] = tab_c[MODE == 2 ? (size_t)r * LK_C + c : s];
            }
            int fp[LK_GATHER_BATCH];
            float fg[LK_GATHER_BATCH], fc[LK_GATHER_BATCH];
#pragma unroll
            for (int k = 0; k < LK_GATHER_BATCH; ++k) {
                const int u = ub + k;
                const int pu = __shfl(pt, min(u, LK_GATHER_WINDOW - 1), 32);
                fp[k] = -1; fg[k] = 0.0f; fc[k] = 0.0f;
                if (u >= u1) continue;
                if ((m >> u) & 1u) {
                    fp[k] = cur; fg[k] = sg; fc[k] = sc;
                    cur = pu; sg = 0.0f; sc = 0.0f;
                }
                sg += wr[k] * vg[k];
                if (col) sc += MODE == 1 ? wr[k] * vc[k] : vc[k];
            }
            lk_arrived(vg[LK_GATHER_BATCH - 1]);
            if (col) lk_arrived(vc[LK_GATHER_BATCH - 1]);
#pragma unroll
            for (int k = 0; k < LK_GATHER_BATCH; ++k)
                if (fp[k] >= 0) {
                    atomicAdd(a.g_geo_feats + (size_t)fp[k] * LK_C + c, fg[k]);
                    if (col) atomicAdd(a.g_col_feats + (size_t)fp[k] * LK_C + c, fc[k]);
                    if (a.act_flag && c == 0) a.act_flag[fp[k]] = 1;
                }
        }
        if (tail) break;
        carry = __shfl(pt, LK_GATHER_WINDOW - 1, 32);
    }
    atomicAdd(a.g_geo_feats + (size_t)cur * LK_C + c, sg);
    if (col) atomicAdd(a.g_col_feats + (size_t)cur * LK_C + c, sc);
    if (a.act_flag && c == 0) a.act_flag[cur] = 1;
}
__global__ __launch_bounds__(256) void k_feat_gather(LkFeatScatterArgs a) {
    const int xb = a.x_on ? 1 : 0;
    if (xb && blockIdx.x == 0) { lk_exposure_step_body(a.x, nullptr, 0); return; }
    if ((int)blockIdx.x - xb < a.dw2_blocks) {
        dw2_body(a.dw2_dc, a.dw2_w_sum, a.dw2_hbar, a.P, a.dw2_live, a.dw2_S, a.dw2_part, (int)blockIdx.x - xb, a.dw2_blocks);
        return;
    }
    const int bx = (int)blockIdx.x - xb - a.dw2_blocks;
    if (a.red_part && bx >= a.red_block0) {
        __shared__ float sh[8][32];
        LkStepRider none; none.n_span = 0;
        col_reduce_body(a.red_part, a.red_n, a.red_width, a.red_out, bx - a.red_block0, sh, none);
        return;
    }
    if (a.dfeat) feat_walk<2>(a, bx);
    else if (a.dc_col) feat_walk<1>(a, bx);
    else feat_walk<0>(a, bx);
}

__global__ __launch_bounds__(256) void k_rays_bwd(LkRaysBwdArgs a) {
    const int r = blockIdx.x * 256 + (int)threadIdx.x;
    if (r >= a.R) return;
    float ox = 0.f, oy = 0.f, oz = 0.f, dx = 0.f, dy = 0.f, dz = 0.f;
    for (int s = 0; s < a.S; ++s) {
        const int p = r * a.S + s;
        const float4 g = *reinterpret_cast<const float4*>(a.dp_total + (size_t)p * 4);
        const float z = a.z[p];
        ox += g.x; oy += g.y; oz += g.z;
        dx = fmaf(g.x, z, dx); dy = fmaf(g.y, z, dy); dz = fmaf(g.z, z, dz);
    }
    a.g_rays_o[3 * r] = ox; a.g_rays_o[3 * r + 1] = oy; a.g_rays_o[3 * r + 2] = oz;
    a.g_rays_d[3 * r] = dx; a.g_rays_d[3 * r + 1] = dy; a.g_rays_d[3 * r + 2] = dz;
}

__device__ __forceinline__ float rp_embed_unit(const float* __restrict__ B, int u, float a0, float a1, float a2) {
    const int xi = (u < 10) ? u : u - 10;
    const float x = lk_fourier_arg(a0, a1, a2, B[xi], B[10 + xi], B[20 + xi]);
    return (u < 10) ? lk_sinf(x) : lk_cosf(x);
}

template <bool F16, bool H16 = false>
__device__ __forceinline__ void relpos_bwd_wave(const LkRelposBwdArgs& a, int sample0, float* __restrict__ part) {
    typedef BwdPiece<H16> PC;
    typedef typename PC::T Piece;
    constexpr float SC = H16 ? 1024.0f : 1.0f, ISC = H16 ? 1.0f / 1024.0f : 1.0f;
    const int lane = lk_lane();
    const int h = lane >> 5;
    const int j = lane & 31;
    const int sample = sample0 + (j >> 3);
    const bool live = sample < a.P;
    const int sp = live ? sample : a.P - 1;
    const int nb_i = j & 7;
    const int r = sp / a.S;
    const float z = a.z[sp];
    const float px = lk_madd_rn(a.rays_o[3 * r], a.rays_d[3 * r], z);
    const float py = lk_madd_rn(a.rays_o[3 * r + 1], a.rays_d[3 * r + 1], z);
    const float pz = lk_madd_rn(a.rays_o[3 * r + 2], a.rays_d[3 * r + 2], z);
    int idx = a.nbr_idx[(size_t)sp * LK_K + nb_i];
    const bool has = a.nbr_count[sp] >= a.min_nn;
    float wgt = (idx >= 0 && has && live) ? a.nbr_w[(size_t)sp * LK_K + nb_i] : 0.0f;
    if (idx < 0) idx = 0;
    const float a0 = __fmul_rn(LK_TWO_PI, __fsub_rn(a.pos[3 * (size_t)idx], px));
    const float a1 = __fmul_rn(LK_TWO_PI, __fsub_rn(a.pos[3 * (size_t)idx + 1], py));
    const float a2 = __fmul_rn(LK_TWO_PI, __fsub_rn(a.pos[3 * (size_t)idx + 2], pz));
    const float* __restrict__ W = a.W;
    const u32x4* __restrict__ FB = reinterpret_cast<const u32x4*>(a.Wfrag);
    const u32x4* __restrict__ FP = FB + (H16 ? FRAGB_U4 : 0);
    const size_t frow = (size_t)idx * LK_C;
    constexpr bool f16 = F16;
    const bool want_w = !H16 && (a.flags & LK_FLAG_GRAD_WEIGHTS) != 0;
    const bool want_p = (a.flags & LK_FLAG_GRAD_RAYS) != 0;
    f32x16 x0, x1;
#pragma unroll
    for (int g = 0; g < 4; ++g) {
        const int u0 = 8 * g + 4 * h;
        if (u0 < ER) {
#pragma unroll
            for (int t = 0; t < 4; ++t) x0[4 * g + t] = rp_embed_unit(W + R_EB, u0 + t, a0, a1, a2);
        } else {
            const float4 v = lk_feat4(a.col_feats, f16, frow + (u0 - ER));
            x0[4 * g] = v.x; x0[4 * g + 1] = v.y; x0[4 * g + 2] = v.z; x0[4 * g + 3] = v.w;
        }
    }
    x1 = lk_zero16();
#pragma unroll
    for (int g = 0; g < 3; ++g) {
        const int u0 = 32 + 8 * g + 4 * h;
        if (u0 < KR) {
            const float4 v = lk_feat4(a.col_feats, f16, frow + (u0 - ER));
            x1[4 * g] = v.x; x1[4 * g + 1] = v.y; x1[4 * g + 2] = v.z; x1[4 * g + 3] = v.w;
        }
    }
    LK_STAMPW(1);
    f32x16 hid[4];
#pragma unroll
    for (int nb = 0; nb < 4; ++nb) hid[nb] = lk_rowvec_tile(W + R_B1, nb * 32, lane);
    const u32x4* __restrict__ FH = FB + FRAGB_U4;
    lk_gemm_h3<4, 2>(hid, FH + FM20_FWDH, 4, 0, 0, x0, 0, lane);
    lk_gemm_h3<4, 2>(hid, FH + FM20_FWDH, 4, 2, 0, x1, 0, lane);
#pragma unroll
    for (int nb = 0; nb < 4; ++nb) {
#pragma unroll
        for (int q = 0; q < 16; ++q) hid[nb][q] = lk_softplus100(hid[nb][q]);
    }
    LK_STAMP(2);
    f32x16 dout[1];
    const float* dcrow = a.dc_col + (size_t)sp * LK_C;
#pragma unroll
    for (int g = 0; g < 4; ++g) {
        const float4 v = *reinterpret_cast<const float4*>(dcrow + 8 * g + 4 * h);
        dout[0][4 * g] = v.x; dout[0][4 * g + 1] = v.y; dout[0][4 * g + 2] = v.z; dout[0][4 * g + 3] = v.w;
    }
    if (want_p) {
        f32x16 out[1];
        out[0] = lk_rowvec_tile(W + R_B2, 0, lane);
#pragma unroll
        for (int kb = 0; kb < 4; ++kb) lk_gemm_h3<1, 2>(out, FH + FM21_FWDH, 1, 2 * kb, 0, hid[kb], 0, lane);
        float part = 0.0f;
#pragma unroll
        for (int q = 0; q < 16; ++q) part = fmaf(dout[0][q], out[0][q], part);
        part += __shfl_xor(part, 32);
        if (live && h == 0) a.dw_rel[(size_t)sp * LK_K + nb_i] = (has && a.nbr_idx[(size_t)sp * LK_K + nb_i] >= 0) ? part : 0.0f;
    }
    {
        const float ws = H16 ? wgt * SC : wgt;
#pragma unroll
        for (int q = 0; q < 16; ++q) dout[0][q] *= ws;
    }
    if (want_w) {
        float wsum = wgt;
        wsum = lk_sum8<true>(wsum);
        if (live && h == 0 && nb_i == 0) a.w_sum[sp] = wsum;
    }
    f32x16 (&dhid)[4] = hid;
    const Piece db0 = PC::split(dout[0], 0), db1 = PC::split(dout[0], 1);
    Piece fa0 = PC::load(FP + PC::tr(21), 4, 0, 0, lane), fa1 = PC::load(FP + PC::tr(21), 4, 1, 0, lane);
    Piece fx[4];
#pragma unroll
    for (int nb = 0; nb < 4; ++nb) {
        f32x16 t = lk_zero16();
        t = PC::mma(fa0, db0, t);
        t = PC::mma(fa1, db1, t);
        if (nb < 3) {
            fa0 = PC::load(FP + PC::tr(21), 4, 0, nb + 1, lane);
            fa1 = PC::load(FP + PC::tr(21), 4, 1, nb + 1, lane);
        } else {
#pragma unroll
            for (int q = 0; q < 4; ++q) fx[q] = PC::load(FP + PC::tr(20), 2, q >> 1, q & 1, lane);
        }
        __builtin_amdgcn_sched_barrier(0);
        if (want_w) {
#pragma unroll
            for (int g = 0; g < 4; ++g) {
                float v[4];
#pragma unroll
                for (int tt = 0; tt < 4; ++tt) {
                    float sred = wgt * hid[nb][4 * g + tt];
                    sred = lk_sum8<true>(sred);
                    v[tt] = sred;
                }
                if (live && nb_i == 0)
                    *reinterpret_cast<float4*>(a.hbar + (size_t)sp * 128 + nb * 32 + 8 * g + 4 * h) = make_float4(v[0], v[1], v[2], v[3]);
            }
        }
#pragma unroll
        for (int q = 0; q < 16; ++q) dhid[nb][q] = t[q] * lk_softplus100_grad_from_out(hid[nb][q]);
    }
    LK_STAMP(3);
    f32x16 dx[2];
    dx[0] = lk_zero16(); dx[1] = lk_zero16();
// ... 692 lines not shown
    __syncthreads();
    if (q != 0) return;
    s = ((sh[0][e] + sh[1][e]) + (sh[2][e] + sh[3][e])) + ((sh[4][e] + sh[5][e]) + (sh[6][e] + sh[7][e]));
    if (in_acc) {
        const int blk = idx >> 10, r = (idx >> 6) & 15, lane = idx & 63, h = lane >> 5, j = lane & 31;
        const int bn = blk / kv, bk = blk - bn * kv;
        const int nn = U.n0 + nv * lk_frag_row(r, h) + bn, k = U.k0 + kv * j + bk;
        if (nn < J.N && k < (J.k_aux ? J.k_aux : J.K)) grad_commit(J.dW + (size_t)nn * J.ldw + k, s, sr);
    } else if (in_bias) {
        const int tcol = idx - 4 * 16 * 64;
        if (J.db && U.k0 == 0 && U.n0 + tcol < J.N) grad_commit(J.db + U.n0 + tcol, s, sr);
    }
}
__global__ __launch_bounds__(256) void k_wgrad_reduce(LkWgradArgs a) {
    __shared__ float sh[8][32];
    LkStepRider none; none.n_span = 0;
    wgrad_reduce_body(a, (int)blockIdx.x, (int)blockIdx.y, sh, none);
}

#define LK_FC_POST_COLS 33
#define LK_FC_MAX_TILES 16
struct LkFcPostLds { float part[4][128]; float m[128]; float half[2][128]; };
__device__ __forceinline__ void fc_post_body(const LkWgradArgs& a, int f, int kc, LkFcPostLds& sh, const LkStepRider& sr) {
    const LkFcPost& F = a.fc[f];
    const LkWgradJob& J = a.job[F.src_job];
    const int t = (int)threadIdx.x;
    const bool bias = kc == 32;
    {
        const int g = t >> 6, e = t & 63;
        float s2[2] = {0.0f, 0.0f};
        int which = 0;
        for (int u = 0; u < a.n_units && which < 2; ++u) {
            const LkWgradUnit& U = a.unit[u];
            if (U.job != F.src_job || U.k0 != (bias ? 0 : J.k_aux)) continue;
            const int nblk = 8 * U.n_waves, nv = U.nv;
            const float* __restrict__ src = a.part + (size_t)8 * U.wave0 * LK_WG_TILE;
            const int off = bias ? 4 * 16 * 64 + e : kc * 64 + e;
            float s = 0.0f;
            for (int y0 = 0; y0 < nblk; y0 += 4 * LK_FC_MAX_TILES) {
                float v[LK_FC_MAX_TILES];
#pragma unroll
                for (int q = 0; q < LK_FC_MAX_TILES; ++q) {
                    const int y = y0 + g + 4 * q;
                    v[q] = (y < nblk && e < 32 * nv && lk_wg_tile_stored(U, y)) ? src[(size_t)y * LK_WG_TILE + off] : 0.0f;
                }
#pragma unroll
                for (int q = 0; q < LK_FC_MAX_TILES; ++q) s += v[q];
            }
            s2[which++] = s;
        }
        sh.part[g][e] = s2[0]; sh.part[g][64 + e] = s2[1];
    }
    __syncthreads();
    if (t < 128) {
        const int which = t >> 6, e = t & 63;
        const float s = ((sh.part[0][t] + sh.part[1][t]) + sh.part[2][t]) + sh.part[3][t];
        const int nv = J.N > 32 ? 2 : 1;
        const int n = 64 * which + e;
        const bool ok = (nv == 2 || (which == 0 && e < 32)) && n < 128;
        if (ok) sh.m[n] = (n < J.N) ? s : 0.0f;
    }
    if (J.N <= 32 && t >= 32 && t < 128) sh.m[t] = 0.0f;
    __syncthreads();
    const int v = t & 127, uh = t >> 7;
    const int u0 = uh * 64, u1 = F.rows_u < u0 + 64 ? F.rows_u : u0 + 64;
    const float* __restrict__ Wv = F.W + F.off + v;
    float w[64];
#pragma unroll
    for (int q = 0; q < 64; ++q) w[q] = (u0 + q < u1) ? Wv[(size_t)(u0 + q) * F.ldw] : 0.0f;
    float acc = 0.0f;
#pragma unroll
    for (int q = 0; q < 64; ++q) acc = fmaf(w[q], sh.m[u0 + q], acc);
    sh.half[uh][v] = acc;
    __syncthreads();
    if (t < 128) {
        const float r = sh.half[0][t] + sh.half[1][t];
        if (bias) grad_commit(F.du + t, r, sr); else grad_commit(F.dU + (size_t)t * 32 + kc, r, sr);
    }
}
__global__ __launch_bounds__(256) void k_fc_post(LkWgradArgs a) {
    __shared__ LkFcPostLds sh;
    LkStepRider none; none.n_span = 0;
    fc_post_body(a, (int)blockIdx.x / LK_FC_POST_COLS, (int)blockIdx.x % LK_FC_POST_COLS, sh, none);
}

__device__ __forceinline__ void col_reduce_body(const float* __restrict__ part, int n_parts, int width, float* __restrict__ out, int bx, float (*sh)[32],
                                                const LkStepRider& sr) {
    const int e = (int)threadIdx.x & 31, q = (int)threadIdx.x >> 5;
    const int col = bx * 32 + e;
    float s = 0.0f;
    if (col < width) {
#pragma unroll 4
        for (int y = q; y < n_parts; y += 8) s += part[(size_t)y * width + col];
    }
    sh[q][e] = s;
    __syncthreads();
    if (q == 0 && col < width) grad_commit(out + col, ((sh[0][e] + sh[1][e]) + (sh[2][e] + sh[3][e])) + ((sh[4][e] + sh[5][e]) + (sh[6][e] + sh[7][e])), sr);
}

__global__ __launch_bounds__(256) void k_bwd_reduce(LkWgradArgs wa, LkBwdReduceArgs r, LkStepRider step) {
    __shared__ float sh[8][32];
    __shared__ LkFcPostLds sh_fc;
    const LkStepRider& sr = step;
    const int n_fc = r.b_fc - r.b_pr;
    if ((int)blockIdx.x < n_fc) { fc_post_body(wa, (int)blockIdx.x / LK_FC_POST_COLS, (int)blockIdx.x % LK_FC_POST_COLS, sh_fc, sr); return; }
    const int b = (int)blockIdx.x - n_fc;
    if (b < r.b_wg) wgrad_reduce_body(wa, b / r.ny, b % r.ny, sh, sr);
    else if (b < r.b_rp) rp_reduce_body(r.part1, r.n1, r.part2, r.n2, r.dW1, r.db1, r.dW2, r.db2, b - r.b_wg, sh, sr);
    else if (b < r.b_pg) col_reduce_body(r.part_bg, r.n_bg, 288, r.out_bg, b - r.b_rp, sh, sr);
    else if (b < r.b_pr) col_reduce_body(r.part_br, r.n_br, 32, r.out_br, b - r.b_pg, sh, sr);
    else {
        const int q = b - r.b_pr;
        if (q < step.feat_gx) lk_adam_seg_block(step.feat[0], step.beta1, step.beta2, step.eps, q, step.feat_gx);
        else lk_adam_seg_block(step.feat[1], step.beta1, step.beta2, step.eps, q - step.feat_gx, step.feat_gx);
    }
}
int lk_launch_bwd_reduce(const LkWgradArgs& wa, LkBwdReduceArgs r, bool with_rp, hipStream_t st, const LkStepRider* step, bool feat_rows) {
    r.ny = lk_cdiv(LK_WG_TILE, 32);
    r.b_wg = wa.part && wa.n_units > 0 ? wa.n_units * r.ny : 0;
    r.b_rp = r.b_wg + (with_rp ? LK_RP_REDUCE_BLOCKS : 0);
    r.b_pg = r.b_rp + (r.part_bg ? lk_cdiv(288, 32) : 0);
    r.b_pr = r.b_pg + (r.part_br ? 1 : 0);
    r.b_fc = r.b_pr + (r.b_wg > 0 ? wa.n_fc * LK_FC_POST_COLS : 0);
    LkStepRider sr;
    if (step) sr = *step; else sr = LkStepRider{};
    r.b_ad = r.b_fc + ((sr.n_span > 0 && feat_rows) ? sr.n_feat * sr.feat_gx : 0);
    if (r.b_ad > 0) hipLaunchKernelGGL(k_bwd_reduce, dim3(r.b_ad), dim3(256), 0, st, wa, r, sr);
    return LK_OK;
}

int lk_launch_relpos_interp_bwd(const LkRelposBwdArgs& rb, const LkInterpBwdArgs& ib, hipStream_t st, bool h16) {
    LkProfScope prof_(LKK_RELPOS_BWD, st);
    const dim3 grid(lk_cdiv(rb.P, 32));
    if (rb.flags & LK_FLAG_FEATS_F16) {
        if (h16) hipLaunchKernelGGL((k_relpos_interp_bwd<true, true>), grid, dim3(512), 0, st, rb, ib);
        else hipLaunchKernelGGL((k_relpos_interp_bwd<true, false>), grid, dim3(512), 0, st, rb, ib);
    } else {
        if (h16) hipLaunchKernelGGL((k_relpos_interp_bwd<false, true>), grid, dim3(512), 0, st, rb, ib);
        else hipLaunchKernelGGL((k_relpos_interp_bwd<false, false>), grid, dim3(512), 0, st, rb, ib);
    }
    return LK_OK;
}
int lk_launch_interp_bwd(const LkInterpBwdArgs& a, hipStream_t st, const ExposureStepArgs* xstep, const float* xstep_part, int xstep_n_part) {
    LkProfScope prof_(LKK_INTERP_BWD, st);
    if (xstep) hipLaunchKernelGGL(k_interp_bwd_x, dim3(lk_cdiv(a.P, 32) + 1), dim3(256), 0, st, a, *xstep, xstep_part, xstep_n_part);
    else hipLaunchKernelGGL(k_interp_bwd, dim3(lk_cdiv(a.P, 32)), dim3(256), 0, st, a);
    return LK_OK;
}
int lk_launch_feat_scatter(const LkFeatScatterArgs& a, hipStream_t st) {
    LkProfScope prof_(LKK_FEAT_SCATTER, st);
    LkFeatScatterArgs b = a;
    b.red_block0 = lk_cdiv((long long)a.P * LK_K, 8 * LK_GATHER_CHUNK);
    if (!b.dw2_part) b.dw2_blocks = 0;
    hipLaunchKernelGGL(k_feat_gather, dim3((b.x_on ? 1 : 0) + b.dw2_blocks + b.red_block0 + (a.red_part ? lk_cdiv(a.red_width, 32) : 0)), dim3(256), 0, st, b);
    return LK_OK;
}
int lk_launch_seg_sort(const LkFeatScatterArgs& a, bool counted, hipStream_t st, int batch) {
    const int nb = lk_cdiv((long long)a.P * LK_K, 256);
    if (!counted) hipLaunchKernelGGL(k_seg_count, dim3(nb, batch), dim3(256), 0, st, a);
    lk_launch_scan_i32(a.seg_cnt, a.seg_off, a.seg_sums, a.N + 1, st, batch, a.cnt_stride, a.sums_stride);
    LkFeatScatterArgs t = a;
    t.seg_list = a.seg_tmp;
    hipLaunchKernelGGL(k_seg_place, dim3(nb, batch), dim3(256), 0, st, t);
    hipLaunchKernelGGL(k_seg_order, dim3(nb, batch), dim3(256), 0, st, a);
    return LK_OK;
}
int lk_launch_rays_bwd(const LkRaysBwdArgs& a, hipStream_t st) {
    LkProfScope prof_(LKK_RAYS_BWD, st);
    hipLaunchKernelGGL(k_rays_bwd, dim3(lk_cdiv(a.R, 256)), dim3(256), 0, st, a);
    return LK_OK;
}
int lk_relpos_bwd_parts(int P) { const int n = lk_cdiv(lk_cdiv(P, 4), 4); return n < LK_RPF_MAX_PARTS ? n : LK_RPF_MAX_PARTS; }
int lk_launch_relpos_bwd(const LkRelposBwdArgs& a, hipStream_t st) {
    LkProfScope prof_(LKK_RELPOS_BWD, st);
    const int waves = lk_cdiv(a.P, 4);
    if (lk_relpos_fused(a.flags)) {
        const bool wg = !(a.flags & LK_FLAG_EMBED_GRADS_ONLY), f16 = (a.flags & LK_FLAG_FEATS_F16) != 0;
        const dim3 grid(lk_relpos_bwd_parts(a.P));
        if (wg && f16) hipLaunchKernelGGL((k_relpos_bwd_fused<true, true>), grid, dim3(256), 0, st, a);
        else if (wg) hipLaunchKernelGGL((k_relpos_bwd_fused<true, false>), grid, dim3(256), 0, st, a);
        else if (f16) hipLaunchKernelGGL((k_relpos_bwd_fused<false, true>), grid, dim3(256), 0, st, a);
        else hipLaunchKernelGGL((k_relpos_bwd_fused<false, false>), grid, dim3(256), 0, st, a);
    }
    else if (a.flags & LK_FLAG_FEATS_F16) hipLaunchKernelGGL(k_relpos_bwd<true>, dim3(lk_cdiv(waves, 4)), dim3(256), 0, st, a);
    else hipLaunchKernelGGL(k_relpos_bwd<false>, dim3(lk_cdiv(waves, 4)), dim3(256), 0, st, a);
    return LK_OK;
}
int lk_dw2_parts(int P) { const int n = lk_cdiv(P, LK_DW2_SAMPLES); return n < 1 ? 1 : (n < LK_DW2_PARTS ? n : LK_DW2_PARTS); }
int64_t lk_dw2_part_floats(int P) { return (int64_t)lk_dw2_parts(P) * LK_DW2_TILE; }
int lk_launch_dw2_hbar(const LkRelposBwdArgs& a, float* dw2_part, hipStream_t st) {
    hipLaunchKernelGGL(k_dw2_hbar, dim3(lk_dw2_parts(a.P)), dim3(256), 0, st, a.dc_col, a.w_sum, a.hbar, a.P, a.live_rays, a.S, dw2_part);
    return LK_OK;
}
int lk_occupancy_relpos_bwd_fused() {
    int n = -1;
    (void)hipOccupancyMaxActiveBlocksPerMultiprocessor(&n, k_relpos_bwd_fused<true, false>, 256, 0);
    return n;
}
int lk_occupancy_wgrad() {
    int n = -1;
    (void)hipOccupancyMaxActiveBlocksPerMultiprocessor(&n, k_wgrad<true>, 256, 0);
    return n;
}
int lk_launch_wgrad(const LkWgradArgs& a_in, int max_rows, hipStream_t st, LkWgradArgs* deferred) {
    if (deferred) deferred->n_units = 0;
    if (a_in.n_jobs == 0 || max_rows <= 0) return LK_OK;
    if (a_in.n_fc > 0 && !a_in.part) return LK_ERR_ARG;
    LkWgradArgs a = a_in;
    a.n_units = 0;
    double work[LK_WGRAD_MAX_UNITS], total = 0.0;
    for (int j = 0; j < a.n_jobs; ++j) {
        const LkWgradJob& J = a.job[j];
        for (int n0 = 0; n0 < J.N; n0 += 64) {
            const int nv = (J.N - n0 > 32) ? 2 : 1;
            const int k_main = J.k_aux ? J.k_aux : J.K;
            for (int k0 = 0; k0 < J.K; k0 += (k0 < k_main && k0 + 64 > k_main) ? k_main - k0 : 64) {
                const int k_end = k0 < k_main ? k_main : J.K;
                const int kv = (k_end - k0 > 32) ? 2 : 1;
                if (a.n_units >= LK_WGRAD_MAX_UNITS) return LK_ERR_ARG;
                LkWgradUnit& U = a.unit[a.n_units];
                U.job = j; U.n0 = n0; U.k0 = k0; U.nv = nv; U.kv = kv;
                work[a.n_units] = (double)J.rows * (nv + kv);
                total += work[a.n_units++];
            }
        }
    }
    int next = 0;
    for (int u = 0; u < a.n_units; ++u) {
        LkWgradUnit& U = a.unit[u];
        const int n_chunks_x = lk_cdiv(lk_cdiv(a.job[U.job].rows, WG_CHUNK), 8);
        int w = (int)((LK_WG_MAX_WAVES / 8 - a.n_units) * (work[u] / total)) + 1;
        if (w > n_chunks_x) w = n_chunks_x > 0 ? n_chunks_x : 1;
        U.wave0 = next; U.n_waves = w;
        next += w;
    }
    a.n_waves = next;
    {
        LkProfScope prof_(LKK_WGRAD, st);
        if (a.h16) hipLaunchKernelGGL(k_wgrad<true>, dim3(8 * lk_cdiv(a.n_waves, 4)), dim3(256), 0, st, a);
        else hipLaunchKernelGGL(k_wgrad<false>, dim3(8 * lk_cdiv(a.n_waves, 4)), dim3(256), 0, st, a);
    }
    if (deferred) { *deferred = a; return LK_OK; }
    if (a.part) hipLaunchKernelGGL(k_wgrad_reduce, dim3(a.n_units, lk_cdiv(LK_WG_TILE, 32)), dim3(256), 0, st, a);
    if (a.part && a.n_fc > 0) hipLaunchKernelGGL(k_fc_post, dim3(a.n_fc * LK_FC_POST_COLS), dim3(256), 0, st, a);
    return LK_OK;
}
```

### loopy_slam_amd/csrc/lk_kernels.h

```cpp
#pragma once
#include "lk_common.h"

template <bool H16> struct BwdPiece;
template <> struct BwdPiece<false> {
    typedef LkB8 T;
    static constexpr int NP = 3;
    static __device__ __forceinline__ T split(const f32x16& x, int G) { return lk_split_ct(x, G); }
    static __device__ __forceinline__ f32x16 mma(const T& a, const T& b, f32x16 c) { return lk_mma6(a, b, c); }
    static __device__ __forceinline__ T load(const u32x4* f, int NBT, int G, int nb, int lane) { return lk_fragb_load(f, NBT, G, nb, lane); }
    static __device__ __forceinline__ int tr(int idx) { return lkw::FRAG_TRB[idx]; }
};
template <> struct BwdPiece<true> {
    typedef LkH8 T;
    static constexpr int NP = 2;
    static __device__ __forceinline__ T split(const f32x16& x, int G) { return lk_split_cth(x, G); }
    static __device__ __forceinline__ f32x16 mma(const T& a, const T& b, f32x16 c) { return lk_mma3h(a, b, c); }
    static __device__ __forceinline__ T load(const u32x4* f, int NBT, int G, int nb, int lane) { return lk_fragh_load(f, NBT, G, nb, lane); }
    static __device__ __forceinline__ int tr(int idx) { return lkw::FRAG_TRH[idx]; }
};


enum LkKernelId { LKK_DEPTH_STATS = 0, LKK_SAMPLE_INTERP, LKK_RELPOS_FWD, LKK_DECODE_FWD, LKK_COMPOSITE, LKK_COMPOSITE_BWD,
                  LKK_DECODE_BWD, LKK_RELPOS_BWD, LKK_INTERP_BWD, LKK_RAYS_BWD, LKK_WGRAD, LKK_FEAT_SCATTER, LKK_DECODE_BWD_TRACK, LKK_COUNT };
void lk_prof_before(int kid, hipStream_t st);
void lk_prof_after(int kid, hipStream_t st);
struct LkProfScope {
    int kid; hipStream_t st;
    LkProfScope(int k, hipStream_t s) : kid(k), st(s) { lk_prof_before(kid, st); }
    ~LkProfScope() { lk_prof_after(kid, st); }
};

struct LkSampleArgs {
    int R, S, P, stats_chunk;
    unsigned flags;
    const float* rays_o; const float* rays_d; const float* gt_depth; const float* r2_ray; const float* far_stats;
    const LkGrid* grid; const float4* sorted; const int32_t* cell_start;
    const float* geo_feats; const float* col_feats; const float* noise_geo; const float* noise_col;
    float near_surface, far_surface, near_end, r2_static;
    int min_nn;
    float* z; int32_t* nbr_idx; float* nbr_w; int32_t* nbr_count; float* c_geo; float* c_col;
    int32_t* seg_cnt; int32_t* seg_rank; const uint8_t* row_mask;
    int seg_P, seg_cnt_stride; const int32_t* seg_live;
    const int32_t* seg_key;
    const float* rp_plain; float* rp_frag; int rp_block0;
    float* rp_copy_dst; int rp_copy_n, rp_block1;
    int rp_m_lo, rp_m_hi, rp_skip_lo, rp_skip_hi;
    const int32_t* live_rays;
};

struct LkCompositeArgs {
    int R, S, min_nn;
    float coef;
    const float* raw; const float* z; const int32_t* nbr_count; const float* gt_depth;
    float* depth; float* var; float* color; uint8_t* valid_ray;
    const float* gt_color; float w_color; int use_color;
    float* d_depth; float* d_color; float* loss_out;
    float* d_raw;
    int keep_depth;
};

struct LkDecodeArgs {
    int R, S, P;
    unsigned flags;
    const float* rays_o; const float* rays_d; const float* z;
    const float* c_geo; const float* c_col;
    const float* W;
    const float* Wfrag;
    const float* affine;
    float* raw;
    float* act;
    const int32_t* live_rays;
    int tile_stride;
    unsigned* status;
};

struct LkRelposArgs {
    int R, S, P, min_nn;
    const float* rays_o; const float* rays_d; const float* z;
    const float* pos;
    const float* col_feats;
    const int32_t* nbr_idx; const float* nbr_w; const int32_t* nbr_count;
    const float* W; const float* Wfrag; const float* noise_col;
    float* c_col;
    int feats_f16;
    const int32_t* live_rays;
    unsigned* status;
};

struct LkCompositeBwdArgs {
    int R, S, min_nn;
    float coef;
    const float* raw; const float* z; const int32_t* nbr_count; const float* gt_depth;
    const float* d_depth; const float* d_var; const float* d_color;
    float* d_raw;
    int keep_depth;
};

struct LkTrackLossArgs {
    int R, S, min_nn;
    float coef, w_color;
    int use_color;
    const float* raw; const float* z; const int32_t* nbr_count; const float* gt_depth; const float* gt_color;
    float* depth; float* var; float* color; uint8_t* valid_ray;
    float* d_depth; float* d_color; float* d_raw; float* out4;
    float* resid;
    float* part;
    int median;
    float* row_part;
};

struct LkDecodeBwdArgs {
    int R, S, P;
    unsigned flags;
    const float* rays_o; const float* rays_d; const float* z;
    const float* W; const float* Wfrag; const float* affine;
    const float* act; const float* raw; const float* d_raw;
    float* dc_geo; float* dc_col;
    float* dy_col;
    float* dlogit;
    float* dp_embed;
    float* dp_embed_col;
    float* g_weights; float* g_affine;
    float* g_affine_part;
    float* part_bg;
    const int32_t* live_rays;
    const float* dscale;
    int cb_on;
    LkCompositeBwdArgs cb;
    int ml_on;
    LkCompositeArgs ml;
    float* ml_row_part;
    int tl_n_part;
    LkTrackLossArgs tl;
};

struct LkTrackFinalArgs {
    int R, n_part;
    float fx, fy, cx, cy;
    const float* pose_part;
    float* cam; float* g_cam; float* adam_mv; float* hist_pre; float* hist_post;
    float step_T, step_q, bc2_sqrt, beta1, beta2, eps;
    const float* next_pix_i; const float* next_pix_j; float* rays_o; float* rays_d;
    int do_update;
    const float* cam_in; const float* mv_in;
    const float* loss_part; int n_loss_part; float* log_row;
};
struct LkInterpBwdArgs {
    int R, S, P, min_nn;
    unsigned flags;
    const float* rays_o; const float* rays_d; const float* z; const float* r2_ray; float r2_static;
    const float* pos; const float* geo_feats; const float* col_feats;
    const int32_t* nbr_idx; const float* nbr_w; const int32_t* nbr_count;
    const float* dc_geo; const float* dc_col;
    const float* dw_rel;
    const float* dp_embed; const float* dp_embed_col; const float* dp_rel;
    float* g_geo_feats; float* g_col_feats;
    float* dp_total;
    float* pose_part; const float* pix_i; const float* pix_j; float fx, fy, cx, cy;
};
struct AdamSegDev {
    float* p; float* g; float* m; float* v; long long n; float step_size, bc2_sqrt;
    const int32_t* row_index; int row_len; int zero_grad; int p_f16;
    const uint8_t* row_flags;
    int g_compact;
};
struct LkStepSpan { int off, n; float step_size, bc2_sqrt; };
struct LkStepRider {
    int n_span;
    LkStepSpan span[16];
    float* g; const float* p; float* w_next; float* m; float* v;
    float beta1, beta2, eps;
    AdamSegDev feat[2]; int n_feat, feat_gx;
};
struct ExposureStepArgs;
struct LkBwdExtra { float* pose_part; const float* pix_i; const float* pix_j; float fx, fy, cx, cy;
                    int32_t* seg_list; int32_t* seg_total; const int32_t* live_rays; const LkStepRider* step; const float* dscale;
                    uint8_t* act_flag; int signal_rows; const LkTrackLossArgs* track_loss; int track_n_part;
                    float* loss_rows;
                    int split_reduce; float* split_frag; float* split_master; int* split_done;
                    const ExposureStepArgs* xstep;
                    const float* xstep_part; int xstep_n_part; };
inline int lk_bwd_pose_parts(int64_t P) { return (int)((P + 31) / 32); }

struct ExposureStepArgs {
    float* feats; float* W1; float* b1; float* W2; float* b2; int F;
    float* aff; float* hid; float* g_aff; float* g; float* m; float* v; float* bwd_scale;
    float step_mlp, step_feat, bc2_sqrt, beta1, beta2, eps;
    int feat_first, feat_count, mode;
};

struct LkFeatScatterArgs {
    int P, min_nn;
    const int32_t* nbr_idx; const float* nbr_w; const int32_t* nbr_count;
    const float* dc_geo; const float* dc_col; const float* dfeat;
    float* g_geo_feats; float* g_col_feats;
    const uint8_t* row_mask;
    int32_t* seg_cnt;
    int32_t* seg_off;
    int32_t* seg_sums;
    int32_t* seg_rank;
    int32_t* seg_list;
    int32_t* seg_tmp;
    int32_t* seg_total;
    int cnt_stride, sums_stride;
    const float* red_part; int red_n, red_width, red_block0; float* red_out;
    int x_on; ExposureStepArgs x;
    const float* dw2_dc; const float* dw2_w_sum; const float* dw2_hbar; float* dw2_part; int dw2_blocks; const int32_t* dw2_live; int dw2_S;
    const int32_t* live_rays; int S;
    int N;
    uint8_t* act_flag;
    const int32_t* key_of;
};
int lk_launch_seg_sort(const LkFeatScatterArgs& a, bool counted, hipStream_t st, int batch = 1);
int lk_launch_scan_i32(int32_t* data, int32_t* out, int32_t* block_sums, int total, hipStream_t st,
                       int batch = 1, int dstride = 0, int sstride = 0);

struct LkRaysBwdArgs { int R, S; const float* z; const float* dp_total; float* g_rays_o; float* g_rays_d; };

struct LkRelposBwdArgs {
    int R, S, P, min_nn;
    unsigned flags;
    const float* rays_o; const float* rays_d; const float* z;
    const float* pos; const float* col_feats;
    const int32_t* nbr_idx; const float* nbr_w; const int32_t* nbr_count;
    const float* W; const float* Wfrag;
    const float* dc_col;
    float* g_col_feats; float* g_weights;
    float* dw_rel;
    float* dp_rel;
    float* rows;
    float* hbar;
    float* w_sum;
    float* dfeat;
    float* w_eff;
    float* part_br;
    float* dw1_part;
    const int32_t* live_rays;
};
#ifndef LK_RPF_MAX_PARTS
#define LK_RPF_MAX_PARTS 512
#endif
static inline bool lk_relpos_fused(unsigned flags) {
    return (flags & LK_FLAG_GRAD_WEIGHTS) && (flags & LK_FLAG_UNIT_LOSS_GRADS) && !(flags & LK_FLAG_GRAD_RAYS);
}
int lk_relpos_bwd_parts(int P);
int64_t lk_dw2_part_floats(int P);
int lk_launch_dw2_hbar(const LkRelposBwdArgs& a, float* dw2_part, hipStream_t st);

struct LkWgradJob {
    const float* A; int lda; int a_mode;
    const float* A2; int lda2;
    const float* B; int ldb;
    const float* B2; int ldb2; int k_split;
    const float* B3; int ldb3; int k_split2;
    int k_aux;
    int N, K;
    int rows;
    float* dW; int ldw;
    float* db;
};
#define LK_WGRAD_MAX_JOBS 12
#define LK_WGRAD_MAX_UNITS 48
struct LkFcPost {
    int src_job, rows_u, ldw, off;
    const float* W;
    float* dU; float* du;
};
struct LkWgradUnit { int job, n0, k0; short nv, kv; int wave0, n_waves; };
struct LkWgradArgs {
    LkWgradJob job[LK_WGRAD_MAX_JOBS]; int n_jobs;
    int chunk;
    LkWgradUnit unit[LK_WGRAD_MAX_UNITS]; int n_units, n_waves;
    float* part;
    int h16;
    LkFcPost fc[5]; int n_fc;
    const int32_t* live_rays; int S;
    const float* dscale;
};
static_assert(sizeof(LkWgradArgs) <= 3600, "LkWgradArgs travels as a kernel argument next to LkBwdReduceArgs (4 KB limit)");
#ifndef LK_WG_MAX_WAVES
#define LK_WG_MAX_WAVES 2048
#endif
#define LK_WG_TILE (4 * 16 * 64 + 64)
inline int64_t lk_wgrad_part_floats(int64_t, bool) { return (int64_t)LK_WG_MAX_WAVES * LK_WG_TILE; }

enum { LK_SKIP_COMPOSITE = 1, LK_SKIP_COMPOSITE_BWD = 2, LK_SKIP_RAYS_BWD = 4, LK_FUSE_COMPOSITE_BWD = 8, LK_LOSS_PREZEROED = 16,
       LK_SEG_SORTED = 32 ,
       LK_PRESAMPLED = 64 ,
       LK_SKIP_AFF_REDUCE = 256 ,
       LK_COMPOSITE_IN_BWD = 512 ,
       LK_FUSE_SMALL = 128  };
struct LkPresampleCount { int P_iter; int32_t* seg_rank; const int32_t* live_rays; const int32_t* key_of; };
int lk_presample(const lk_render_desc* d, hipStream_t st, const LkPresampleCount* cnt = nullptr);
int lk_wait_rows_event(hipStream_t st);
bool lk_serial_mode();
#define LK_PRE_CHUNKS 16
struct LkAuxStream { hipStream_t st = nullptr; hipEvent_t e0 = nullptr; hipEvent_t ev[LK_PRE_CHUNKS] = {}; hipEvent_t e1 = nullptr, e2 = nullptr; bool ok = false; };
LkAuxStream& lk_aux_stream();
struct LkRepackRider { float* frag; const float* src; float* copy_dst; int copy_n;
                       int skip_trunk; };
int lk_launch_repack_trunk(const float* src, float* dst, float* frag, hipStream_t st);
int lk_render_fwd_impl(const lk_render_desc* d, hipStream_t st, unsigned skip, const int32_t* live_rays = nullptr, const LkRepackRider* repack = nullptr,
                       const LkTrackFinalArgs* pose = nullptr, const LkTrackLossArgs* comp = nullptr, int* comp_tiles = nullptr,
                       bool join_side_before_decode = false);
int lk_render_bwd_impl(const lk_render_desc* d, hipStream_t st, unsigned skip, const LkBwdExtra* ex = nullptr);
struct LkBwdOffsets { int64_t d_raw, dp_total, aff_part; };
LkBwdOffsets lk_bwd_offsets(int64_t P, uint32_t flags);

int lk_launch_composite_bwd(const LkCompositeBwdArgs& a, hipStream_t st);
int lk_launch_decode_bwd(const LkDecodeBwdArgs& a, hipStream_t st);
int lk_launch_interp_bwd(const LkInterpBwdArgs& a, hipStream_t st, const ExposureStepArgs* xstep = nullptr, const float* xstep_part = nullptr, int xstep_n_part = 0);
int lk_launch_rays_bwd(const LkRaysBwdArgs& a, hipStream_t st);
int lk_launch_feat_scatter(const LkFeatScatterArgs& a, hipStream_t st);
int lk_launch_relpos_bwd(const LkRelposBwdArgs& a, hipStream_t st);
int lk_launch_wgrad(const LkWgradArgs& a, int max_rows, hipStream_t st, LkWgradArgs* deferred = nullptr);
struct LkBwdReduceArgs {
    int b_wg, ny, b_rp, b_pg, b_pr, b_fc, b_ad;
    const float* part1; int n1; const float* part2; int n2; float* dW1; float* db1; float* dW2; float* db2;
    const float* part_bg; int n_bg; float* out_bg;
    const float* part_br; int n_br; float* out_br;
};
int lk_launch_bwd_reduce(const LkWgradArgs& wa, LkBwdReduceArgs r, bool with_rp, hipStream_t st, const LkStepRider* step = nullptr, bool feat_rows = true);
int lk_dw2_parts(int P);
int lk_launch_reduce_partials(const float* part, int n_parts, int width, float* out, hipStream_t st);
int64_t lk_geo_wgrad_part_floats(int P);
int lk_launch_geo_wgrad(int P, int S, const float* rays_o, const float* rays_d, const float* z, const float* W, const float* act,
                        const float* c_geo, const float* d_raw, float* part, float* g_weights, hipStream_t st, const int32_t* live_rays = nullptr);

int lk_launch_depth_stats(const float* gt, int R, int chunk, float* far_out, hipStream_t st);
int lk_launch_sample_interp(const LkSampleArgs& a, hipStream_t st, int mode = 0, const LkTrackFinalArgs* pose = nullptr);
int lk_launch_composite(const LkCompositeArgs& a, hipStream_t st);
int lk_launch_decode_fwd(const LkDecodeArgs& a, hipStream_t st);
int lk_launch_relpos_fwd(const LkRelposArgs& a, hipStream_t st);
bool lk_relpos_decode_fusable(const LkDecodeArgs& a);
struct LkTrackLossArgs;
int lk_launch_relpos_decode_fwd(const LkRelposArgs& ra, const LkDecodeArgs& a, hipStream_t st, const LkTrackLossArgs* comp = nullptr, int* comp_tiles = nullptr);
int lk_launch_relpos_interp_bwd(const LkRelposBwdArgs& rb, const LkInterpBwdArgs& ib, hipStream_t st, bool h16);

#define LK_ACT_GEO_A (5 * 32)
#define LK_ACT_COL_A (5 * 128)
#define LK_ACT_COL_H (5 * 128)
#define LK_ACT_COL_E 40
#define LK_ACT_FLOATS_PER_SAMPLE (LK_ACT_GEO_A + LK_ACT_COL_A + LK_ACT_COL_H + LK_ACT_COL_E)
#ifndef LK_DEEP_MAX_TILES
#define LK_DEEP_MAX_TILES 512
#endif
#ifndef LK_DEEP_MAX_TILES_FWD
#define LK_DEEP_MAX_TILES_FWD 512
#endif
#define LK_COL_LAYER(P, layer) ((size_t)(layer) * (size_t)(P) * 128)
#define LK_COL_SLAYER(P, layer) ((size_t)(layer) * (size_t)(P) * 64)

int lk_occupancy_decode_fwd();
int lk_occupancy_relpos_fwd();
int lk_occupancy_decode_bwd();
int lk_occupancy_relpos_bwd_fused();
int lk_occupancy_wgrad();

#define LK_REG_OUT LK_ICP_SUMS
```

### loopy_slam_amd/csrc/lk_loop.hip

```cpp
#include "lk_common.h"
#include "lk_kernels.h"
#include "lk_composite_dev.h"
#include "lk_mask_dev.h"
#include "lk_track_dev.h"
#include "lk_exposure_dev.h"

#include <math.h>
#include <string.h>

using namespace lkw;

int lk_launch_exposure_step(const lk_exposure_desc& x, int mode, int step, float beta1, float beta2, float eps, hipStream_t st);
int lk_exposure_step_args(const lk_exposure_desc& x, int mode, int step, float beta1, float beta2, float eps, ExposureStepArgs* out);
int lk_adam_step_x(const lk_adam_seg* segs, int32_t n_seg, float beta1, float beta2, float eps, const ExposureStepArgs* xa, void* stream_);
int lk_launch_composite_loss_exposure(const LkCompositeArgs& ca, const float* gt_color, const int32_t* frame_id, const float* aff, int F, float w_color,
                                      float* d_depth, float* d_logits, float* out_loss, float* g_aff, hipStream_t st);

#define LK_TRACK_FUSED_MAX_R LK_MASK_REG_MAX

struct LkPregatherArgs {
    const float* depth; const float* color; const float* c2w; int c2w_stride; const float* r2_map; const int32_t* frame_id;
    const int32_t* rnd;
    int R, H, W, H0, W0, w;
    float fx, fy, cx, cy;
// ... 317 lines not shown
            pa.next_pix_i = W0 + wk.pix_i + (size_t)it * R; pa.next_pix_j = W0 + wk.pix_j + (size_t)it * R;
            pa.loss_part = W0 + wk.row_part; pa.n_loss_part = n_pose; pa.log_row = d->log + (size_t)(it - 1) * 4;
        }
        LkTrackLossArgs la;
        memset(&la, 0, sizeof(la));
        if (fused) {
            la.R = R; la.S = S; la.min_nn = rd.min_nn; la.coef = rd.coef; la.w_color = d->w_color;
            la.use_color = d->use_color & LK_TRACK_USE_COLOR; la.median = (d->use_color & LK_TRACK_MEDIAN_MASK) ? 1 : 0;
            la.raw = rd.raw; la.z = rd.z; la.nbr_count = rd.nbr_count; la.gt_depth = rd.gt_depth; la.gt_color = gt_color;
            la.depth = rd.depth; la.var = rd.var; la.color = rd.color; la.valid_ray = rd.valid_ray;
            la.d_depth = const_cast<float*>(rd.d_depth); la.d_color = const_cast<float*>(rd.d_color);
            la.d_raw = rd.bwd_scratch + off.d_raw; la.out4 = log_row; la.resid = W0 + wk.resid; la.part = W0 + wk.loss_part;
            la.row_part = W0 + wk.row_part;
        }
        int comp_tiles = 0;
        int rc = lk_render_fwd_impl(&rd, st, fused ? (LK_SKIP_COMPOSITE | LK_FUSE_SMALL) : 0, nullptr, nullptr, (prologue && it > 0) ? &pa : nullptr,
                                    fused ? &la : nullptr, &comp_tiles);
        if (rc != LK_OK) return rc;
        const int n_part = comp_tiles > 0 ? comp_tiles : n_lp;
        if (fused) {
            if (comp_tiles == 0) hipLaunchKernelGGL(k_track_composite, dim3(n_lp), dim3(256), 0, st, la);
            if (la.median) hipLaunchKernelGGL(k_track_median, dim3(1), dim3(1024), 0, st, la);
        } else {
            rc = lk_loss_tracker(R, rd.depth, rd.var, rd.color, rd.gt_depth, d->gt_color, d->w_color, d->use_color,
                                 const_cast<float*>(rd.d_depth), const_cast<float*>(rd.d_color), log_row, d->loss_scratch, st);
            if (rc != LK_OK) return rc;
        }
        LkBwdExtra ex;
        memset(&ex, 0, sizeof(ex));
        if (fused) { ex.track_loss = &la; ex.track_n_part = n_part; }
        ex.pose_part = fused ? W0 + wk.pose_part : nullptr;
        ex.dscale = (xd && (rd.flags & LK_FLAG_UNIT_LOSS_GRADS)) ? xd->bwd_scale : nullptr;
        ex.pix_i = W0 ? W0 + wk.pix_i + (size_t)it * R : nullptr; ex.pix_j = W0 ? W0 + wk.pix_j + (size_t)it * R : nullptr;
        ex.fx = d->fx; ex.fy = d->fy; ex.cx = d->cx; ex.cy = d->cy;
        ExposureStepArgs xa_bwd;
        if (x_in_bwd) {
            rc = lk_exposure_step_args(*xd, 3, it + 1, beta1, beta2, eps, &xa_bwd);
            if (rc != LK_OK) return rc;
            ex.xstep = &xa_bwd; ex.xstep_part = rd.bwd_scratch + off.aff_part; ex.xstep_n_part = lk_cdiv(R * S, 32);
        }
        rc = lk_render_bwd_impl(&rd, st, fused ? (LK_SKIP_COMPOSITE_BWD | LK_SKIP_RAYS_BWD | LK_FUSE_SMALL | (xd ? LK_SKIP_AFF_REDUCE : 0)) : 0, fused ? &ex : nullptr);
        if (rc != LK_OK) return rc;
        if (xd && !fused) {
            rc = lk_launch_exposure_step(*xd, 3, it + 1, beta1, beta2, eps, st);
            if (rc != LK_OK) return rc;
        }
        float step_T, step_q, bc2s;
        adam_scalars(d->lr_T, it + 1, beta1, beta2, &step_T, &bc2s);
        adam_scalars(d->lr_q, it + 1, beta1, beta2, &step_q, &bc2s);
        if (fused && prologue && it + 1 < iters) {
        } else if (fused) {
            if (prologue) {
                fa.cam_in = W0 + wk.ring + 8 * (it & 1); fa.mv_in = W0 + wk.ring + 16 + 16 * (it & 1);
            }
            fa.step_T = step_T; fa.step_q = step_q; fa.bc2_sqrt = bc2s; fa.do_update = 1;
            fa.loss_part = W0 + wk.row_part; fa.n_loss_part = n_pose; fa.log_row = log_row;
            fa.hist_pre = d->hist_post ? nullptr : hist_row; fa.hist_post = d->hist_post ? hist_row : nullptr;
            const bool more = it + 1 < iters;
            fa.rays_o = more ? const_cast<float*>(rd.rays_o) : nullptr; fa.rays_d = const_cast<float*>(rd.rays_d);
            fa.next_pix_i = W0 + wk.pix_i + (size_t)(it + 1) * R * (more ? 1 : 0); fa.next_pix_j = W0 + wk.pix_j + (size_t)(it + 1) * R * (more ? 1 : 0);
            ExposureStepArgs xa;
            memset(&xa, 0, sizeof(xa));
            const bool x_here = xd != nullptr && !x_in_bwd;
            if (x_here) {
                rc = lk_exposure_step_args(*xd, 3, it + 1, beta1, beta2, eps, &xa);
                if (rc != LK_OK) return rc;
            }
            hipLaunchKernelGGL(k_track_final, dim3(x_here ? 2 : 1), dim3(1024), 0, st, fa, xa,
                               x_here ? (const float*)(rd.bwd_scratch + off.aff_part) : (const float*)nullptr, x_here ? lk_cdiv(R * S, 32) : 0);
        }
        if (!fused) {
            rc = lk_pose_bwd(d->cam7, d->pix_i, d->pix_j, R, d->fx, d->fy, d->cx, d->cy, rd.g_rays_o, rd.g_rays_d, d->g_cam7, st);
            if (rc != LK_OK) return rc;
            lk_adam_seg seg[2];
            memset(seg, 0, sizeof(seg));
            seg[0].p = d->cam7 + 4; seg[0].g = d->g_cam7 + 4; seg[0].m = d->adam_mv + 4; seg[0].v = d->adam_mv + 11; seg[0].n = 3; seg[0].lr = d->lr_T; seg[0].step = it + 1;
            seg[1].p = d->cam7; seg[1].g = d->g_cam7; seg[1].m = d->adam_mv; seg[1].v = d->adam_mv + 7; seg[1].n = 4; seg[1].lr = d->lr_q; seg[1].step = it + 1;
            rc = lk_adam_step(seg, 2, beta1, beta2, eps, st);
            if (rc != LK_OK) return rc;
            if (d->hist_post) LK_HIP_TRY(hipMemcpyAsync(hist_row, d->cam7, 7 * sizeof(float), hipMemcpyDeviceToDevice, st));
        }
    }
    LK_LAUNCH_CHECK();
    return LK_OK;
}

static void map_join_and_pregather(const lk_map_desc* d, const MapWork& wk, int R, const lk_exposure_desc* xd, hipStream_t st) {
    float* W0 = d->work;
    {
        PreStream& pj = pre_stream();
        if (pj.ok) { (void)hipEventRecord(pj.e1, pj.st); (void)hipStreamWaitEvent(st, pj.e1, 0); }
    }
    {
        LkPregatherArgs pa;
        memset(&pa, 0, sizeof(pa));
        pa.depth = d->depth_stack; pa.color = d->color_stack; pa.c2w = d->c2w_stack; pa.c2w_stride = d->c2w_stride; pa.r2_map = d->r2_map_stack;
        pa.frame_id = d->frame_id; pa.rnd = d->rnd;
        pa.R = R; pa.H = d->H; pa.W = d->W; pa.H0 = d->H0; pa.W0 = d->W0; pa.w = d->w;
        pa.fx = d->fx; pa.fy = d->fy; pa.cx = d->cx; pa.cy = d->cy;
        pa.rays_o = W0 + wk.rays_o; pa.rays_d = W0 + wk.rays_d; pa.gt_depth = W0 + wk.gt_depth; pa.gt_color = W0 + wk.gt_color;
        pa.r2_ray = d->render.r2_ray ? W0 + wk.r2_ray : nullptr; pa.thr = W0 + wk.thr; pa.zero4 = d->log;
        pa.n_live = reinterpret_cast<int32_t*>(W0 + wk.n_live);
        if (xd) pa.frame_out = reinterpret_cast<int32_t*>(W0 + wk.frame_id);
        if (R <= LK_MASK_REG_MAX) hipLaunchKernelGGL(k_pregather<LK_MASK_VPT>, dim3(d->iters), dim3(1024), 0, st, pa);
        else hipLaunchKernelGGL(k_pregather<LK_LOOP_MAX_R / 1024>, dim3(d->iters), dim3(1024), 0, st, pa);
    }
}
extern "C" int lk_map_prepare(const lk_map_desc* d, void* stream_) {
    LK_REQUIRE(d != nullptr && d->iters >= 0 && d->render.R >= 0, "lk_map_prepare: bad descriptor");
    if (d->iters == 0 || d->render.R == 0) return LK_OK;
    LK_REQUIRE(d->work != nullptr && d->render.R <= LK_LOOP_MAX_R, "lk_map_prepare: needs `work` and at most 16384 rays");
    LK_REQUIRE(d->depth_stack && d->color_stack && d->c2w_stack && d->rnd && d->log, "lk_map_prepare: NULL batch buffer");
    LK_REQUIRE(!d->exposure || d->frame_id, "lk_map_prepare: exposure encoding needs frame_id");
    const MapWork wk = map_work(d->render.R, d->render.S, d->iters);
    map_join_and_pregather(d, wk, d->render.R, d->exposure, (hipStream_t)stream_);
    LK_LAUNCH_CHECK();
    return LK_OK;
}

extern "C" int lk_map_frame(const lk_map_desc* d, int32_t it_begin, int32_t it_end, int32_t phases, void* stream_) {
    LK_REQUIRE(d != nullptr, "lk_map_frame: NULL descriptor");
    { const int rcg = lk_status_gate("lk_map_frame"); if (rcg != LK_OK) return rcg; }
    LK_REQUIRE(it_begin >= 0 && it_end <= d->iters && it_begin <= it_end && (phases & 3), "lk_map_frame: bad iteration range / phases");
    LK_REQUIRE(d->n_geo_dec >= 0 && d->n_geo_dec <= LK_MAX_SPANS && d->n_col_dec >= 0 && d->n_col_dec <= LK_MAX_SPANS, "lk_map_frame: too many spans");
    if (it_begin == it_end || d->render.R == 0) return LK_OK;
    LK_REQUIRE(d->it_offset >= 0, "lk_map_frame: negative it_offset");
    const int goff = d->it_offset, n_geo_l = d->n_geo_iters - goff;
    LK_REQUIRE(d->depth_stack && d->color_stack && d->c2w_stack && d->rnd && d->log, "lk_map_frame: NULL batch buffer");
    LK_REQUIRE(d->weights_rw && d->weights_frag_rw && d->geo_feats_rw && d->col_feats_rw && d->adam_rows && d->adam_dec && d->n_rows >= 0,
               "lk_map_frame: NULL optimiser buffer");
    LK_REQUIRE(d->render.g_geo_feats && d->render.g_col_feats && d->render.g_weights && d->render.d_depth && d->render.d_color &&
               d->render.bwd_scratch && d->render.act, "lk_map_frame: the render descriptor needs gradient buffers, d_depth/d_color, bwd_scratch and act");
    hipStream_t st = (hipStream_t)stream_;
    const int R = d->render.R;
    const bool pre = d->work != nullptr && R <= LK_LOOP_MAX_R;
    if (!pre) LK_REQUIRE(d->gt_color && d->thr && d->scratch_u32, "lk_map_frame: without `work` (or above 16384 rays) the per-iteration batch buffers are needed");
    const lk_exposure_desc* xd = d->exposure;
    LK_REQUIRE(!xd || (pre && d->frame_id), "lk_map_frame: exposure encoding needs `work` (<= 16384 rays) and frame_id");
    const float beta1 = 0.9f, beta2 = 0.999f, eps = 1e-8f;
    const int64_t nb = lk_weight_blob_floats();
    const int64_t nrow = d->n_rows * LK_C;
    lk_knn_s* kn_h = d->render.knn;
    const bool act_rows = d->rows == nullptr && ((phases & 3) == 3 || d->union_rows_flagged) && kn_h->act_flag != nullptr && d->n_rows <= kn_h->capacity;
    if (act_rows && it_begin == 0 && goff == 0 && (phases & 1)) LK_HIP_TRY(hipMemsetAsync(kn_h->act_flag, 0, (size_t)d->n_rows, st));
    const MapWork wk = map_work(R, d->render.S, d->iters);
    const int64_t Pn = (int64_t)R * d->render.S;
    const int pre_chunk = map_pre_chunk(d->iters);
    auto chunk_start = [&](int c) { return c == 0 ? 0 : 1 + (c - 1) * pre_chunk; };
    auto chunk_of = [&](int it) { return it == 0 ? 0 : 1 + (it - 1) / pre_chunk; };
    float* W0 = d->work;
    if (pre && it_begin == 0 && (phases & 1) && !d->batches_ready) map_join_and_pregather(d, wk, R, xd, st);
    const bool sort_ahead = pre && d->render.g_geo_feats != nullptr;
    const bool key_rows = sort_ahead && d->rows != nullptr && kn_h->row_rank != nullptr && d->n_rows > 0;
    auto enqueue_chunk = [&](int c) -> int {
        const int c0 = chunk_start(c);
        if (c0 >= d->iters) return LK_OK;
        PreStream& ps = pre_stream();
        hipStream_t pst = ps.ok ? ps.st : st;
        if (ps.ok && c == 0) { (void)hipEventRecord(ps.e0, st); (void)hipStreamWaitEvent(pst, ps.e0, 0); }
        const int c1 = chunk_start(c + 1) < d->iters ? chunk_start(c + 1) : d->iters, nc = c1 - c0;
        lk_render_desc sd = d->render;
        sd.flags = (d->render.flags & LK_FLAG_REL_POS) | LK_FLAG_ZERO_ABSENT;
        sd.R = nc * R; sd.stats_chunk = sd.R;
        sd.rays_o = W0 + wk.rays_o + (size_t)c0 * R * 3; sd.rays_d = W0 + wk.rays_d + (size_t)c0 * R * 3;
        sd.gt_depth = W0 + wk.gt_depth + (size_t)c0 * R;
        sd.r2_ray = d->render.r2_ray ? W0 + wk.r2_ray + (size_t)c0 * R : nullptr;
        sd.z = W0 + wk.z + (size_t)c0 * Pn; sd.nbr_count = reinterpret_cast<int32_t*>(W0 + wk.nbr_count) + (size_t)c0 * Pn;
        sd.nbr_idx = reinterpret_cast<int32_t*>(W0 + wk.nbr_idx) + (size_t)c0 * Pn * LK_K; sd.nbr_w = W0 + wk.nbr_w + (size_t)c0 * Pn * LK_K;
        const bool counted = sort_ahead && nc <= LK_SEG_BATCH;
        LkPresampleCount pc;
        pc.P_iter = (int)Pn; pc.seg_rank = reinterpret_cast<int32_t*>(W0 + wk.seg_rank); pc.live_rays = reinterpret_cast<const int32_t*>(W0 + wk.n_live) + c0;
        pc.key_of = key_rows ? kn_h->row_rank : nullptr;
        sd.grad_row_mask = d->render.grad_row_mask;
        int rc = lk_presample(&sd, pst, counted ? &pc : nullptr);
        if (rc != LK_OK) return rc;
        for (int it = c0; sort_ahead && it < c0 + nc; it += LK_SEG_BATCH) {
            const int nbatch = c0 + nc - it < LK_SEG_BATCH ? c0 + nc - it : LK_SEG_BATCH;
            const lk_knn_s* kn = d->render.knn;
            LkFeatScatterArgs fs;
            memset(&fs, 0, sizeof(fs));
            fs.P = (int)Pn; fs.min_nn = d->render.min_nn; fs.row_mask = d->render.grad_row_mask; fs.N = key_rows ? (int)d->n_rows : (int)kn->n;
            fs.key_of = key_rows ? kn_h->row_rank : nullptr;
            fs.nbr_idx = reinterpret_cast<int32_t*>(W0 + wk.nbr_idx) + (size_t)it * Pn * LK_K; fs.nbr_w = W0 + wk.nbr_w + (size_t)it * Pn * LK_K;
            fs.nbr_count = reinterpret_cast<int32_t*>(W0 + wk.nbr_count) + (size_t)it * Pn;
            fs.seg_cnt = kn->seg_cnt; fs.seg_off = kn->seg_off; fs.seg_sums = kn->seg_sums;
            fs.cnt_stride = kn->seg_stride; fs.sums_stride = kn->seg_sums_stride;
            fs.seg_rank = reinterpret_cast<int32_t*>(W0 + wk.seg_rank); fs.seg_tmp = reinterpret_cast<int32_t*>(W0 + wk.seg_tmp);
            fs.seg_list = reinterpret_cast<int32_t*>(W0 + wk.seg_list) + (size_t)it * Pn * LK_K;
            fs.seg_total = reinterpret_cast<int32_t*>(W0 + wk.seg_total) + it;
            fs.live_rays = reinterpret_cast<const int32_t*>(W0 + wk.n_live) + it; fs.S = d->render.S;
            rc = lk_launch_seg_sort(fs, counted, pst, nbatch);
            if (rc != LK_OK) return rc;
        }
        if (ps.ok) (void)hipEventRecord(ps.ev[c % LK_PRE_CHUNKS], pst);
        return LK_OK;
    };
    if (key_rows && it_begin == 0 && (phases & 1)) {
        LK_HIP_TRY(hipMemsetAsync(kn_h->row_rank, 0xFF, sizeof(int32_t) * (size_t)kn_h->n, st));
        hipLaunchKernelGGL(k_row_rank, dim3(lk_cdiv(d->n_rows, 256)), dim3(256), 0, st, d->rows, (int)d->n_rows, (int)kn_h->n, kn_h->row_rank);
    }
    if (pre && it_begin == 0 && (phases & 1)) {
        const int rc = enqueue_chunk(0);
        if (rc != LK_OK) return rc;
    }
    auto build_segs = [&](int it, bool color, lk_adam_seg* seg, int& ns) -> bool {
        const float* lr = d->lr[color ? 1 : 0];
        ns = 0;
        auto dec_seg = [&](const lk_blob_span& sp, int step) {
            lk_adam_seg& s = seg[ns++];
            s.p = d->weights_rw + sp.offset; s.g = d->render.g_weights + sp.offset; s.m = d->adam_dec + sp.offset; s.v = d->adam_dec + nb + sp.offset;
            s.n = sp.n; s.lr = lr[0]; s.step = step; s.zero_grad = 1;
        };
        for (int k = 0; k < d->n_geo_dec; ++k) dec_seg(d->geo_dec[k], goff + it + 1);
        if (color) for (int k = 0; k < d->n_col_dec; ++k) dec_seg(d->col_dec[k], it - n_geo_l + 1);
        if (ns + 2 > LK_ADAM_MAX_SEG) return false;
        {
            lk_adam_seg& s = seg[ns++];
            s.p = d->geo_feats_rw; s.g = d->render.g_geo_feats; s.m = d->adam_rows; s.v = d->adam_rows + nrow; s.n = nrow; s.lr = lr[1]; s.step = goff + it + 1;
            s.row_index = d->rows; s.row_len = d->rows ? LK_C : 1; s.zero_grad = 1; s.p_f16 = (d->render.flags & LK_FLAG_FEATS_F16) ? 1 : 0;
            if (act_rows) { s.row_len = LK_C; s.row_flags = kn_h->act_flag; }
        }
        if (color) {
            lk_adam_seg& s = seg[ns++];
            s.p = d->col_feats_rw; s.g = d->render.g_col_feats; s.m = d->adam_rows + 2 * nrow; s.v = d->adam_rows + 3 * nrow; s.n = nrow; s.lr = lr[2];
            s.step = it - n_geo_l + 1; s.row_index = d->rows; s.row_len = d->rows ? LK_C : 1; s.zero_grad = 1;
            s.p_f16 = (d->render.flags & LK_FLAG_FEATS_F16) ? 1 : 0;
            if (act_rows) { s.row_len = LK_C; s.row_flags = kn_h->act_flag; }
        }
        return true;
    };
    bool repack_pending = false, stepped_pending = false;
    int split_pending = 0;
    const bool train_geo = d->train_geo_decoder != 0;
    const bool rider_ok = pre && !xd && !train_geo && (phases & 3) == 3 && d->render.weights == d->weights_rw && d->render.g_weights != nullptr &&
                          (!(d->render.flags & LK_FLAG_REL_POS) || lk_relpos_fused(d->render.flags | LK_FLAG_GRAD_WEIGHTS)) &&
                          d->n_geo_dec + d->n_col_dec <= 16 && nb < (1ll << 31);
    bool embed_only = true;
    for (int k = 0; k < d->n_col_dec; ++k)
        embed_only = embed_only && d->col_dec[k].offset >= R_EB && d->col_dec[k].offset + d->col_dec[k].n <= R_EB + 3 * 10;
    if (train_geo) embed_only = false;
    bool w_next_ready = false;
    bool x_early = false;
    int sum_lo = -1, sum_hi = -1;
    bool x_fwd_done = it_begin > n_geo_l;
    for (int it = it_begin; it < it_end; ++it) {
        const bool color = it >= n_geo_l;
        const bool use_rider = rider_ok && !embed_only && color && it + 1 < it_end && d->n_col_dec > 0;
        lk_render_desc rd = d->render;
        const bool xit = xd != nullptr && color;
        rd.flags = (d->render.flags & (LK_FLAG_REL_POS | LK_FLAG_UNIT_LOSS_GRADS | LK_FLAG_FEATS_F16)) | (color ? LK_FLAG_STAGE_COLOR : 0) | LK_FLAG_SAVE_ACT |
                   LK_FLAG_GRAD_FEATS | LK_FLAG_GRAD_WEIGHTS | LK_FLAG_ZERO_ABSENT | LK_FLAG_MAPPER_LOSS | (embed_only && color ? LK_FLAG_EMBED_GRADS_ONLY : 0) |
                   (train_geo ? LK_FLAG_GRAD_GEO_DECODER : 0);
        const bool x_unit = xd && xd->bwd_scale && !(d->render.flags & LK_FLAG_REL_POS);
        if (xd && !x_unit) rd.flags &= ~LK_FLAG_UNIT_LOSS_GRADS;
        if (x_unit) rd.flags |= LK_FLAG_UNIT_LOSS_GRADS;
        if (xit) rd.flags = (rd.flags & ~LK_FLAG_MAPPER_LOSS) | LK_FLAG_COLOR_LOGITS;
        rd.stats_chunk = R;
        rd.loss_gt_color = d->gt_color; rd.loss_w_color = d->w_color; rd.loss_out4 = d->log + (size_t)it * 4;
        if (pre) {
            rd.rays_o = W0 + wk.rays_o + (size_t)it * R * 3; rd.rays_d = W0 + wk.rays_d + (size_t)it * R * 3;
            rd.gt_depth = W0 + wk.gt_depth + (size_t)it * R; rd.loss_gt_color = W0 + wk.gt_color + (size_t)it * R * 3;
            if (rd.r2_ray) rd.r2_ray = W0 + wk.r2_ray + (size_t)it * R;
            rd.z = W0 + wk.z + (size_t)it * Pn; rd.nbr_count = reinterpret_cast<int32_t*>(W0 + wk.nbr_count) + (size_t)it * Pn;
            rd.nbr_idx = reinterpret_cast<int32_t*>(W0 + wk.nbr_idx) + (size_t)it * Pn * LK_K; rd.nbr_w = W0 + wk.nbr_w + (size_t)it * Pn * LK_K;
            if ((goff + it) & 1) rd.c_col = W0 + wk.c_col_alt;
            const int ck = chunk_of(it);
            if ((phases & 1) && it == chunk_start(ck)) {
                const int rc = enqueue_chunk(ck + 1);
                if (rc != LK_OK) return rc;
            }
            if ((phases & 1) && (it == chunk_start(ck) || it == it_begin)) {
                PreStream& ps = pre_stream();
                if (ps.ok) (void)hipStreamWaitEvent(st, ps.ev[ck % LK_PRE_CHUNKS], 0);
            }
        }
        if (phases & 1) {
            int rc;
            if (!pre) {
                rc = lk_gather_rays(d->depth_stack, d->color_stack, d->c2w_stack, d->c2w_stride, d->r2_map_stack, d->frame_id, d->rnd + (size_t)it * R, R,
                                    d->H, d->W, d->H0, d->W0, d->w, d->fx, d->fy, d->cx, d->cy, const_cast<float*>(rd.rays_o),
                                    const_cast<float*>(rd.rays_d), const_cast<float*>(rd.gt_depth), d->gt_color, nullptr, nullptr,
                                    const_cast<float*>(rd.r2_ray), st);
                if (rc != LK_OK) return rc;
                rc = lk_inside_mask(rd.gt_depth, R, nullptr, const_cast<float*>(rd.gt_depth), d->thr, d->scratch_u32, st);
                if (rc != LK_OK) return rc;
            }
            const int32_t* live = pre ? reinterpret_cast<const int32_t*>(W0 + wk.n_live) + it : nullptr;
            LkRepackRider rr;
            rr.frag = d->weights_frag_rw; rr.src = stepped_pending ? W0 + wk.w_next : nullptr;
            rr.copy_dst = stepped_pending ? d->weights_rw : nullptr; rr.copy_n = (int)nb;
            rr.skip_trunk = (stepped_pending && split_pending) ? 1 : 0;
            const bool join_side = rr.skip_trunk != 0;
            if (xit && it == (n_geo_l > it_begin ? n_geo_l : it_begin) && !x_fwd_done) {
                rc = lk_launch_exposure_step(*xd, 2, 1, beta1, beta2, eps, st);
                if (rc != LK_OK) return rc;
            }
            x_fwd_done = x_fwd_done || xit;
            const bool split_repack = pre && (phases & 3) == 1 && it == it_begin && it > n_geo_l && !embed_only && d->n_col_dec > 0 &&
                                      d->render.weights == d->weights_rw;
            const bool comp_bwd = pre && !xit && !train_geo;
            if (comp_bwd) { if (sum_lo < 0) sum_lo = it; sum_hi = it + 1; }
            rc = lk_render_fwd_impl(&rd, st, (xit ? LK_SKIP_COMPOSITE : LK_FUSE_COMPOSITE_BWD) | (pre ? (LK_LOSS_PREZEROED | LK_PRESAMPLED) : 0) |
                                    (sort_ahead ? LK_SEG_SORTED : 0) | (comp_bwd ? LK_COMPOSITE_IN_BWD : 0), live,
                                    (repack_pending || stepped_pending || split_repack) ? &rr : nullptr, nullptr, nullptr, nullptr, join_side);
            repack_pending = false; stepped_pending = false; split_pending = 0;
            if (rc != LK_OK) return rc;
            if (xit) {
                LkCompositeArgs ca;
                memset(&ca, 0, sizeof(ca));
                ca.R = R; ca.S = rd.S; ca.min_nn = rd.min_nn; ca.coef = rd.coef;
                ca.raw = rd.raw; ca.z = rd.z; ca.nbr_count = rd.nbr_count; ca.gt_depth = rd.gt_depth;
                ca.depth = rd.depth; ca.var = rd.var; ca.color = rd.color; ca.valid_ray = rd.valid_ray;
                ca.keep_depth = (rd.flags & LK_FLAG_Z_GIVEN) ? 1 : 0;
                rc = lk_launch_composite_loss_exposure(ca, rd.loss_gt_color, reinterpret_cast<const int32_t*>(W0 + wk.frame_id) + (size_t)it * R, xd->aff, xd->F,
                                                       d->w_color, const_cast<float*>(rd.d_depth), const_cast<float*>(rd.d_color), rd.loss_out4, xd->g_aff, st);
                if (rc != LK_OK) return rc;
            }
            LkBwdExtra ex;
            memset(&ex, 0, sizeof(ex));
            if (sort_ahead) {
                ex.seg_list = reinterpret_cast<int32_t*>(W0 + wk.seg_list) + (size_t)it * Pn * LK_K;
                ex.seg_total = reinterpret_cast<int32_t*>(W0 + wk.seg_total) + it;
            }
            ex.live_rays = live;
            ex.act_flag = act_rows ? kn_h->act_flag : nullptr;
            ex.signal_rows = ((phases & 3) == 1) ? d->signal_rows : 0;
            ex.dscale = (xd && (rd.flags & LK_FLAG_UNIT_LOSS_GRADS)) ? xd->bwd_scale : nullptr;
            LkStepRider sr;
            if (use_rider) {
                lk_adam_seg seg[LK_ADAM_MAX_SEG];
                memset(seg, 0, sizeof(seg));
                int ns = 0;
                LK_REQUIRE(build_segs(it, color, seg, ns), "lk_map_frame: too many optimiser segments");
                memset(&sr, 0, sizeof(sr));
                sr.g = d->render.g_weights; sr.p = d->weights_rw; sr.w_next = W0 + wk.w_next; sr.m = d->adam_dec; sr.v = d->adam_dec + nb;
                sr.beta1 = beta1; sr.beta2 = beta2; sr.eps = eps;
                long long nmax = 0;
                for (int q = 0; q < ns; ++q) {
                    const double bc1 = 1.0 - pow((double)beta1, (double)seg[q].step), bc2 = 1.0 - pow((double)beta2, (double)seg[q].step);
                    const float step_size = (float)((double)seg[q].lr / bc1), bc2_sqrt = (float)sqrt(bc2);
                    if (q < ns - 2) {
                        LkStepSpan& sp = sr.span[sr.n_span++];
                        sp.off = (int)(seg[q].p - d->weights_rw); sp.n = (int)seg[q].n; sp.step_size = step_size; sp.bc2_sqrt = bc2_sqrt;
                    } else {
                        AdamSegDev& f = sr.feat[sr.n_feat++];
                        f.p = seg[q].p; f.g = seg[q].g; f.m = seg[q].m; f.v = seg[q].v; f.n = seg[q].n; f.step_size = step_size; f.bc2_sqrt = bc2_sqrt;
                        f.row_index = seg[q].row_index; f.row_len = seg[q].row_len > 0 ? seg[q].row_len : 1; f.zero_grad = seg[q].zero_grad; f.p_f16 = seg[q].p_f16;
                        f.row_flags = seg[q].row_flags; f.g_compact = seg[q].g_compact;
                        if (seg[q].n > nmax) nmax = seg[q].n;
                    }
                }
                sr.feat_gx = (int)(nmax > 0 ? (lk_cdiv(nmax, 256) > 2048 ? 2048 : lk_cdiv(nmax, 256)) : 1);
                if (!w_next_ready) {
                    LK_HIP_TRY(hipMemcpyAsync(W0 + wk.w_next, d->weights_rw, sizeof(float) * (size_t)nb, hipMemcpyDeviceToDevice, st));
                    w_next_ready = true;
                }
                ex.step = &sr;
                ex.split_reduce = 1; ex.split_frag = d->weights_frag_rw; ex.split_master = d->weights_rw; ex.split_done = &split_pending;
            }
            if (comp_bwd) ex.loss_rows = W0 + wk.loss_rows + (size_t)it * 4 * lk_cdiv(Pn, 32);
            ExposureStepArgs xa_early;
            x_early = false;
            if (xit && pre && (phases & 3) == 3) {
                rc = lk_exposure_step_args(*xd, 1, it - n_geo_l + 1, beta1, beta2, eps, &xa_early);
                if (rc != LK_OK) return rc;
                ex.xstep = &xa_early;
                x_early = true;
            }
            rc = lk_render_bwd_impl(&rd, st, (xit ? 0 : LK_SKIP_COMPOSITE_BWD) | LK_SEG_SORTED | (comp_bwd ? LK_COMPOSITE_IN_BWD : 0), pre ? &ex : nullptr);
            if (rc != LK_OK) return rc;
        }
        if (phases & 2) {
            lk_adam_seg seg[LK_ADAM_MAX_SEG];
            memset(seg, 0, sizeof(seg));
            int ns = 0;
            LK_REQUIRE(build_segs(it, color, seg, ns), "lk_map_frame: too many optimiser segments");
            if (d->grad_bucket && (phases & 3) == 2) {
                LK_REQUIRE(d->rows != nullptr && !xd, "lk_map_frame: grad_bucket needs a row list and no exposure encoding");
                int q = 0;
                for (int k = 0; k < d->n_geo_dec; ++k, ++q) { seg[q].g = const_cast<float*>(d->grad_bucket) + d->bucket_geo_dec[k]; seg[q].zero_grad = 0; }
                if (color) for (int k = 0; k < d->n_col_dec; ++k, ++q) { seg[q].g = const_cast<float*>(d->grad_bucket) + d->bucket_col_dec[k]; seg[q].zero_grad = 0; }
                seg[q].g = const_cast<float*>(d->grad_bucket) + d->bucket_geo_rows; seg[q].g_compact = 1; seg[q].zero_grad = 0; ++q;
                if (color) { seg[q].g = const_cast<float*>(d->grad_bucket) + d->bucket_col_rows; seg[q].g_compact = 1; seg[q].zero_grad = 0; ++q; }
                LK_REQUIRE(q == ns, "lk_map_frame: segment order changed under grad_bucket");
            }
            if (use_rider) {
                stepped_pending = true;
                continue;
            }
            int rc;
            if (xit) {
                ExposureStepArgs xa;
                rc = lk_exposure_step_args(*xd, x_early ? 2 : 3, it - n_geo_l + 1, beta1, beta2, eps, &xa);
                if (rc != LK_OK) return rc;
                rc = lk_adam_step_x(seg, ns, beta1, beta2, eps, &xa, st);
            } else {
                rc = lk_adam_step(seg, ns, beta1, beta2, eps, st);
            }
            if (rc != LK_OK) return rc;
            if ((color && !embed_only) || train_geo) {
                if (pre && (phases & 3) == 3 && it + 1 < it_end && d->render.weights == d->weights_rw) repack_pending = true;
                else if (color && !embed_only && pre && (phases & 3) == 2 && it + 1 < d->iters && d->render.weights == d->weights_rw) {
                } else {
                    rc = lk_weights_repack(d->weights_rw, d->weights_frag_rw, st);
                    if (rc != LK_OK) return rc;
                }
            }
        }
    }
    if ((phases & 3) != 3) {
        sum_lo = -1;
        if ((phases & 1) && it_end == d->iters && pre && !train_geo) {
            sum_lo = 0;
            sum_hi = xd ? (n_geo_l < 0 ? 0 : (n_geo_l > d->iters ? d->iters : n_geo_l)) : d->iters;
        }
    }
    if (sum_lo >= 0) {
        if (sum_hi > sum_lo)
            hipLaunchKernelGGL(k_loss_rows_sum, dim3(sum_hi - sum_lo), dim3(256), 0, st, W0 + wk.loss_rows, lk_cdiv(Pn, 32), (int)Pn, d->render.S,
                               reinterpret_cast<const int32_t*>(W0 + wk.n_live), sum_lo, d->log);
    }
    LK_LAUNCH_CHECK();
    return LK_OK;
}

extern "C" int lk_map_wait_rows(const lk_map_desc* d, void* stream_) {
    LK_REQUIRE(d != nullptr, "lk_map_wait_rows: NULL descriptor");
    return lk_wait_rows_event((hipStream_t)stream_);
}

extern "C" int lk_map_wait_lists(const lk_map_desc* d, int32_t it, void* stream_) {
    LK_REQUIRE(d != nullptr && it >= 0 && it < d->iters, "lk_map_wait_lists: bad arguments");
    PreStream& ps = pre_stream();
    if (!ps.ok || d->work == nullptr || d->render.R > LK_LOOP_MAX_R) return LK_OK;
    const int pre_chunk = map_pre_chunk(d->iters);
    const int ck = it == 0 ? 0 : 1 + (it - 1) / pre_chunk;
    LK_HIP_TRY(hipStreamWaitEvent((hipStream_t)stream_, ps.ev[ck % LK_PRE_CHUNKS], 0));
    return LK_OK;
}
```

### loopy_slam_amd/steps.py

```python
import os

import torch

from . import _ffi, core, optim
from ._ffi import ptr

GEO_DECODER_PARAMS = ('geo_decoder.embedder._B',)
GEO_DECODER_ALL_PARAMS = tuple(
    ['geo_decoder.embedder._B'] +
    [f'geo_decoder.pts_linears.{i}.{w}' for i in range(5) for w in ('weight', 'bias')] +
    [f'geo_decoder.fc_c.{i}.{w}' for i in range(5) for w in ('weight', 'bias')] +
    ['geo_decoder.output_linear.weight', 'geo_decoder.output_linear.bias'])
COLOR_DECODER_PARAMS = tuple(
    [f'color_decoder.pts_linears.{i}.{w}' for i in range(5) for w in ('weight', 'bias')] +
    [f'color_decoder.fc_c.{i}.{w}' for i in range(5) for w in ('weight', 'bias')] +
    ['color_decoder.output_linear.weight', 'color_decoder.output_linear.bias',
     'color_decoder.embedder_rel_pos._B',
     'color_decoder.mlp_col_neighbor.linear1.weight', 'color_decoder.mlp_col_neighbor.linear1.bias',
     'color_decoder.mlp_col_neighbor.linear2.weight', 'color_decoder.mlp_col_neighbor.linear2.bias'])


class RayBatch:

    def __init__(self, eng, R, dynamic_radius=False):
        e = eng
        self.R = R
        self.rays_o, self.rays_d = e.empty(R, 3), e.empty(R, 3)
        self.gt_depth, self.gt_color = e.empty(R), e.empty(R, 3)
        self.pix_i, self.pix_j = e.empty(R), e.empty(R)
        self.r2_ray = e.empty(R) if dynamic_radius else None
        self.d_depth, self.d_color = e.empty(R), e.empty(R, 3)
        self.thr = e.empty(1)
        self.scratch_u32 = e.empty(R, dtype=torch.int32)
        self.loss_scratch = e.empty(R + 8)

    def as_out(self):
        d = dict(rays_o=self.rays_o, rays_d=self.rays_d, gt_depth=self.gt_depth, gt_color=self.gt_color,
                 pix_i=self.pix_i, pix_j=self.pix_j)
        if self.r2_ray is not None:
            d['r2_ray'] = self.r2_ray
        return d


class ExposureState:

    LR = 0.001

    def __init__(self, eng, mlp, feats):
        self.eng = eng
        self.W1, self.b1, self.W2, self.b2 = (mlp[0].weight.data, mlp[0].bias.data, mlp[2].weight.data, mlp[2].bias.data)
        for t in (self.W1, self.b1, self.W2, self.b2):
            assert t.is_contiguous() and t.dtype == torch.float32
        assert tuple(self.W1.shape) == (128, 8) and tuple(self.W2.shape) == (12, 128)
        self.single = torch.is_tensor(feats)
        self.orig = [feats] if self.single else list(feats)
        self.F = len(self.orig)
        assert 1 <= self.F <= _ffi.EXPOSURE_MAX_F
        self.feats = feats.data if self.single else torch.stack([f.detach() for f in self.orig]).contiguous()
        self.aff, self.hid = eng.zeros(self.F, 12), eng.zeros(self.F, 128)
        self.g_aff = eng.zeros(self.F, 12)
        self.g = eng.zeros(_ffi.EXPOSURE_GRAD_FLOATS)
        self._desc = None

    def desc(self, lr_mlp, lr_feat=None, only_last_feature=False):
        d = _ffi.ExposureDesc()
        d.feats, d.W1, d.b1, d.W2, d.b2, d.F = ptr(self.feats), ptr(self.W1), ptr(self.b1), ptr(self.W2), ptr(self.b2), self.F
        d.aff, d.hid, d.g_aff, d.g = ptr(self.aff), ptr(self.hid), ptr(self.g_aff), ptr(self.g)
        self.adam_mv = self.eng.zeros(2 * _ffi.EXPOSURE_GRAD_FLOATS)
        d.adam = ptr(self.adam_mv)
        d.lr_mlp = -1.0 if lr_mlp is None else float(lr_mlp)
        d.lr_feat = self.LR if lr_feat is None else float(lr_feat)
        d.feat_first, d.feat_count = (self.F - 1, 1) if only_last_feature else (0, self.F)
        self.bwd_scale = self.eng.zeros(1) + 1.0
        d.bwd_scale = ptr(self.bwd_scale)
        self._desc = d
        return d

    def forward(self):
        e = self.eng
        e.lib.check(e.lib.dll.lk_exposure_fwd(ptr(self.feats), ptr(self.W1), ptr(self.b1), ptr(self.W2), ptr(self.b2), self.F,
                                              ptr(self.aff), ptr(self.hid), e.stream), 'lk_exposure_fwd')
        return self.aff

    def backward(self, g_aff):
        e = self.eng
        e.lib.check(e.lib.dll.lk_exposure_bwd(ptr(self.feats), ptr(self.W1), ptr(self.W2), ptr(self.hid), ptr(g_aff), self.F,
                                              ptr(self.g), e.stream), 'lk_exposure_bwd')

    def adam_segs(self, mlp_lr=None, only_last_feature=False):
        g, lr = self.g, self.LR
        segs = []
        if mlp_lr is not False:
            ml = lr if mlp_lr is None else mlp_lr
            segs += [('xW1', self.W1.view(-1), g[0:1024], ml), ('xb1', self.b1, g[1024:1152], ml), ('xW2', self.W2.view(-1), g[1152:2688], ml),
                     ('xb2', self.b2, g[2688:2700], ml)]
        if only_last_feature:
            k = self.F - 1
            segs.append(('xf', self.feats.view(-1)[8 * k:8 * k + 8], g[2700 + 8 * k:2700 + 8 * k + 8], lr))
        else:
            segs.append(('xf', self.feats.view(-1), g[2700:2700 + self.F * 8], lr))
        return segs

    def finish(self):
        if not self.single:
            with torch.no_grad():
                for k, t in enumerate(self.orig):
                    t.copy_(self.feats[k])


class MapOptimizer:

    _tokens = 0

    @classmethod
    def _next_token(cls):
        cls._tokens += 1
        return cls._tokens

    def __init__(self, eng, cfg, dec, knn, pos, geo_feats, col_feats, row_index, R, lrs, w_color=0.1,
                 dynamic_radius=False, fix_color_decoder=False, dist=None, exposure=None, fix_geo_decoder=True):
        self.eng, self.cfg, self.dec, self.knn = eng, cfg, dec, knn
        self.pos, self.geo, self.col = pos, geo_feats, col_feats
        self.rows = row_index
        self.call_token = self._next_token()
        self.lrs, self.w_color = lrs, w_color
        self.R = R
        self.batch = RayBatch(eng, R, dynamic_radius)
        self.st = core.RenderState(eng, R, cfg.S, need_act=True)
        N = geo_feats.shape[0]
        self.gs = core.GradState(eng, N, R, dec.n, feats=True, weights=True)
        self.adam = optim.Adam(eng)
        cnames = [n for n in COLOR_DECODER_PARAMS if n in dec.layout] if not fix_color_decoder else \
            ['color_decoder.embedder_rel_pos._B']
        if not cfg.rel_pos:
            cnames = [n for n in cnames if 'mlp_col_neighbor' not in n and 'embedder_rel_pos' not in n]
        self.fix_color_decoder = fix_color_decoder
        self.fix_geo_decoder = fix_geo_decoder
        self.gs.geo_decoder = not fix_geo_decoder
        self.geo_dec_ranges = dec.param_ranges(list(GEO_DECODER_PARAMS if fix_geo_decoder else GEO_DECODER_ALL_PARAMS),
                                               bridge_padding=not fix_geo_decoder)
        self.col_dec_ranges = dec.param_ranges(cnames)
        self.loss_log = None
        self.dist = dist
        self.it = 0
        self.native_loop = True
        self.max_call_iters = int(os.environ.get('LOOPY_MAX_CALL_ITERS', '384'))
        self._work = None
        self._nat, self._nat_dirty = None, False
        self._prepared = None
        self.exposure = ExposureState(eng, exposure[0], exposure[1]) if exposure is not None else None
        self.ba = None

    def enable_ba(self, cams7, trainable, lr_of_iteration):
        eng = self.eng
        F = cams7.shape[0]
        assert cams7.is_contiguous() and cams7.shape == (F, 7) and len(trainable) == F and self.R % F == 0
        self.ba = dict(cams=cams7, g=eng.zeros(F, 7), trainable=[bool(t) for t in trainable], pix=self.R // F, lr=lr_of_iteration)
        if self.gs.g_rays_o is None:
            self.gs.g_rays_o, self.gs.g_rays_d = eng.zeros(self.R, 3), eng.zeros(self.R, 3)

    def iterate(self, stage, frames, rnd, frame_id, window, intr, H, W, log_row=None):
        eng, b, st, gs = self.eng, self.batch, self.st, self.gs
        depth_stack, color_stack, c2w_stack, r2_stack = frames
        optim.gather_rays(eng, depth_stack, color_stack, c2w_stack, frame_id, rnd, H, W, window, intr, b.as_out(), r2_stack)
        optim.inside_mask(eng, b.gt_depth, None, b.thr, b.scratch_u32, depth_filtered=b.gt_depth)
        ba = self.ba
        if ba is not None:
            n = ba['pix']
            for f, tr in enumerate(ba['trainable']):
                if tr:
                    sl = slice(f * n, (f + 1) * n)
                    optim.rays_from_pose(eng, ba['cams'][f], b.pix_i[sl], b.pix_j[sl], intr, b.rays_o[sl], b.rays_d[sl])
        out4 = log_row if log_row is not None else self._out4()
        xs = self.exposure if stage == 'color' else None
        fused = None if xs is not None else (b.gt_color, self.w_color, b.d_depth, b.d_color, out4)
        core.render_forward(eng, self.cfg, st, b.rays_o, b.rays_d, b.gt_depth, self.knn, self.pos, self.geo, self.col,
                            self.dec, stage, r2_ray=b.r2_ray, save_act=True, tracker=ba is not None,
                            extra_flags=_ffi.FLAG_ZERO_ABSENT | (_ffi.FLAG_UNIT_LOSS_GRADS if self.exposure is None else 0),
                            color_logits=self.exposure is not None, mapper_loss=fused)
        if xs is not None:
            xs.forward()
            eng.lib.check(eng.lib.dll.lk_loss_mapper_exposure(self.R, ptr(st.depth), ptr(st.color), ptr(st.valid_ray), ptr(b.gt_depth),
                                                              ptr(b.gt_color), ptr(frame_id), ptr(xs.aff), xs.F,
                                                              _ffi.C.c_float(self.w_color), ptr(b.d_depth), ptr(b.d_color), ptr(out4),
                                                              ptr(xs.g_aff), eng.stream), 'lk_loss_mapper_exposure')
        core.render_backward(eng, st, gs, b.d_depth, b.d_color)
        if ba is not None:
            n = ba['pix']
            for f, tr in enumerate(ba['trainable']):
                if tr:
                    sl = slice(f * n, (f + 1) * n)
                    optim.pose_bwd(eng, ba['cams'][f], b.pix_i[sl], b.pix_j[sl], intr, gs.g_rays_o[sl], gs.g_rays_d[sl], ba['g'][f])
        if self.dist is not None:
            self.dist.all_reduce_grads(self, stage, it=None)
            if ba is not None:
                self.dist.all_reduce_vec(ba['g'])
        dlr, glr, clr = self.lrs[stage]
        segs = [(('gdec', k), self.dec.blob[o:o + n], gs.g_weights[o:o + n], dlr) for k, (o, n) in enumerate(self.geo_dec_ranges)]
        if stage == 'color':
            segs += [(('cdec', k), self.dec.blob[o:o + n], gs.g_weights[o:o + n], dlr) for k, (o, n) in enumerate(self.col_dec_ranges)]
        if self.rows is not None:
            segs.append(('geo', self.geo, gs.g_geo, glr, self.rows))
            if stage == 'color':
                segs.append(('col', self.col, gs.g_col, clr, self.rows))
        else:
            segs.append(('geo', self.geo.view(-1), gs.g_geo.view(-1), glr))
            if stage == 'color':
                segs.append(('col', self.col.view(-1), gs.g_col.view(-1), clr))
        if xs is not None:
            xs.backward(xs.g_aff)
            segs += xs.adam_segs(mlp_lr=False if self.fix_color_decoder else dlr, only_last_feature=True)
        if ba is not None:
            segs.append(('cams', ba['cams'].view(-1), ba['g'].view(-1), float(ba['lr'](self.it))))
        self.adam.step(segs, zero_grad=True)
        if stage == 'color' or not self.fix_geo_decoder:
            self.dec.repack()
        self.it += 1
        return out4

    def run(self, n_iters, n_geo_iters, frames, rnd_all, frame_id, window, intr, H, W, log):
        if not self._takes_native_loop():
            for it in range(n_iters):
                self.iterate('geometry' if it < n_geo_iters else 'color', frames, rnd_all[it], frame_id, window, intr, H, W, log_row=log[it])
            return log
        eng = self.eng
        d, seg_iters = self._native_desc(n_iters, n_geo_iters, frames, rnd_all, frame_id, window, intr, H, W, log)
        C = _ffi.C
        dll = eng.lib.dll
        prepared, self._prepared = self._prepared, None
        if self.dist is None:
            for s0 in range(0, n_iters, seg_iters):
                n = min(seg_iters, n_iters - s0)
                d.it_offset, d.iters = s0, n
                d.rnd, d.log = ptr(rnd_all[s0:]), ptr(log[s0:])
                d.batches_ready = 1 if (s0 == 0 and prepared == self._prepare_key(n_iters, frames, rnd_all, frame_id, window, intr, H, W, log)) else 0
                eng.lib.check(dll.lk_map_frame(C.byref(d), 0, n, 3, eng.stream), 'lk_map_frame')
        else:
            self._nat_desc = d
            d.signal_rows = 1 if self.dist.overlaps_rows(self) else 0
            for it in range(n_iters):
                eng.lib.check(dll.lk_map_frame(C.byref(d), it, it + 1, 1, eng.stream), 'lk_map_frame')
                if self.rows is None and it + 1 < n_iters and self._nat_lists is not None:
                    self.dist.prefetch_touched(self, it + 1)
                self.dist.all_reduce_grads(self, 'geometry' if it < n_geo_iters else 'color', it=it, desc=d)
                if self.rows is None:
                    self.dist.flag_union(self)
                eng.lib.check(dll.lk_map_frame(C.byref(d), it, it + 1, 2, eng.stream), 'lk_map_frame')
        self.it += n_iters
        return log

    def _takes_native_loop(self):
        return self.native_loop and self.ba is None and not (self.exposure is not None and self.R > 16384)

    def prepare(self, n_iters, n_geo_iters, frames, rnd_all, frame_id, window, intr, H, W, log):
        self._prepared = None
        if not self._takes_native_loop() or self.dist is not None or self.R > 16384:
            return False
        self.gs.zero_()
        d, seg_iters = self._native_desc(n_iters, n_geo_iters, frames, rnd_all, frame_id, window, intr, H, W, log, rows_known=False)
        d.iters, d.it_offset = min(seg_iters, n_iters), 0
        self.eng.lib.check(self.eng.lib.dll.lk_map_prepare(_ffi.C.byref(d), self.eng.stream), 'lk_map_prepare')
        self._prepared = self._prepare_key(n_iters, frames, rnd_all, frame_id, window, intr, H, W, log)
        return True

    def _prepare_key(self, n_iters, frames, rnd_all, frame_id, window, intr, H, W, log):
        ptrs = tuple(t.data_ptr() if t is not None else 0 for t in (rnd_all, log, frame_id, self._work) + tuple(frames))
        return (n_iters, ptrs, tuple(int(x) for x in window), tuple(float(x) for x in intr), int(H), int(W))

    def _native_desc(self, n_iters, n_geo_iters, frames, rnd_all, frame_id, window, intr, H, W, log, rows_known=True):
        eng, b, st, gs = self.eng, self.batch, self.st, self.gs
        depth_stack, color_stack, c2w_stack, r2_stack = frames
        core.fill_desc(eng, self.cfg, st, b.rays_o, b.rays_d, b.gt_depth, self.knn, self.pos, self.geo, self.col, self.dec, 'color',
                       r2_ray=b.r2_ray, save_act=True)
        unit = _ffi.FLAG_UNIT_LOSS_GRADS if self.exposure is None else 0
        base = (_ffi.FLAG_REL_POS if self.cfg.rel_pos else 0) | unit | _ffi.FLAG_SAVE_ACT | _ffi.FLAG_GRAD_FEATS | \
            _ffi.FLAG_GRAD_WEIGHTS | _ffi.FLAG_ZERO_ABSENT | _ffi.FLAG_MAPPER_LOSS | (0 if self.fix_geo_decoder else _ffi.FLAG_GRAD_GEO_DECODER)
        need = max(int(eng.lib.dll.lk_render_bwd_scratch_floats(self.R, self.cfg.S, base | extra)) for extra in (0, _ffi.FLAG_STAGE_COLOR))
        if gs.scratch is None or gs.scratch.numel() < need:
            gs.scratch = eng.empty(max(1, need))
        d = _ffi.MapDesc()
        C = _ffi.C
        C.memmove(C.byref(d.render), C.byref(st.desc), C.sizeof(_ffi.RenderDesc))
        r = d.render
        r.flags = (_ffi.FLAG_REL_POS if self.cfg.rel_pos else 0) | unit
        if self.geo.dtype == torch.float16:
            r.flags |= _ffi.FLAG_FEATS_F16
        r.d_depth, r.d_color = ptr(b.d_depth), ptr(b.d_color)
        r.g_geo_feats, r.g_col_feats, r.g_weights = ptr(gs.g_geo), ptr(gs.g_col), ptr(gs.g_weights)
        r.grad_row_mask, r.bwd_scratch, r.bwd_scratch_cap = ptr(gs.row_mask), ptr(gs.scratch), gs.scratch.numel()
        H0, H1, W0, W1 = window
        d.depth_stack, d.color_stack, d.c2w_stack, d.c2w_stride = ptr(depth_stack), ptr(color_stack), ptr(c2w_stack), c2w_stack.shape[-2] * 4
        d.r2_map_stack, d.frame_id = ptr(r2_stack), ptr(frame_id)
        rnd_all = rnd_all.contiguous()
        assert rnd_all.dtype == torch.int32 and rnd_all.shape[0] >= n_iters and rnd_all.shape[1] == self.R and log.is_contiguous()
        d.rnd = ptr(rnd_all)
        d.H, d.W, d.H0, d.W0, d.w = H, W, H0, W0, W1 - W0
        d.fx, d.fy, d.cx, d.cy = intr
        d.gt_color, d.thr, d.scratch_u32 = ptr(b.gt_color), ptr(b.thr), ptr(b.scratch_u32)
        d.w_color, d.log = self.w_color, ptr(log)
        d.weights_rw, d.weights_frag_rw = ptr(self.dec.blob), ptr(self.dec.frag)
        d.geo_feats_rw, d.col_feats_rw = ptr(self.geo), ptr(self.col)
        n_rows = self.rows.numel() if self.rows is not None else self.geo.shape[0]
        d.rows, d.n_rows = ptr(self.rows), n_rows
        if rows_known:
            if self._nat is None or self._nat[0].numel() != 4 * n_rows * 32:
                self._nat = (eng.zeros(4 * n_rows * 32), eng.zeros(2 * self.dec.n))
            elif self._nat_dirty:
                self._nat[0].zero_(); self._nat[1].zero_()
            self._nat_dirty = True
            d.adam_rows, d.adam_dec = ptr(self._nat[0]), ptr(self._nat[1])
        assert len(self.geo_dec_ranges) <= _ffi.MAX_SPANS and len(self.col_dec_ranges) <= _ffi.MAX_SPANS
        for k, (o, n) in enumerate(self.geo_dec_ranges):
            d.geo_dec[k].offset, d.geo_dec[k].n = o, n
        for k, (o, n) in enumerate(self.col_dec_ranges):
            d.col_dec[k].offset, d.col_dec[k].n = o, n
        d.n_geo_dec, d.n_col_dec = len(self.geo_dec_ranges), len(self.col_dec_ranges)
        for si, stage in enumerate(('geometry', 'color')):
            for k in range(3):
                d.lr[si][k] = self.lrs[stage][k]
        d.iters, d.n_geo_iters = n_iters, n_geo_iters
        d.train_geo_decoder = 0 if self.fix_geo_decoder else 1
        if self.exposure is not None:
            xd = self.exposure.desc(None if self.fix_color_decoder else self.lrs['color'][0], only_last_feature=True)
            d.exposure = C.pointer(xd)
        seg_iters = n_iters if (self.dist is not None or n_iters <= self.max_call_iters) else self.max_call_iters
        d.iters = seg_iters
        need = int(eng.lib.dll.lk_map_work_floats(self.R, self.cfg.S, seg_iters)) if self.R <= 16384 else 0
        if need and (self._work is None or self._work.numel() < need):
            self._work = eng.empty(need)
        d.work = ptr(self._work) if need else 0
        d.union_rows_flagged = 1 if (self.dist is not None and self.rows is None and self.geo.shape[0] <= self.knn.capacity) else 0
        self._nat_lists = (int(eng.lib.dll.lk_map_work_nbr_idx(self.R, self.cfg.S, n_iters)), n_iters) if need else None
        self._keep_native = (depth_stack, color_stack, c2w_stack, r2_stack, frame_id, rnd_all, log)
        return d, seg_iters

    def nbr_idx_of(self, it=None):
        if it is not None and getattr(self, '_nat_lists', None) is not None and self.native_loop:
            off, _ = self._nat_lists
            P8 = self.R * self.cfg.S * 8
            return self._work[off + it * P8: off + (it + 1) * P8].view(torch.int32)
        return self.st.nbr_idx

    def wait_lists(self, it):
        if getattr(self, '_nat_desc', None) is not None and getattr(self, '_nat_lists', None) is not None:
            self.eng.lib.check(self.eng.lib.dll.lk_map_wait_lists(_ffi.C.byref(self._nat_desc), it, self.eng.stream), 'lk_map_wait_lists')

    def finish(self):
        if self.exposure is not None:
            self.exposure.finish()

    def _out4(self):
        if self.loss_log is None:
            self.loss_log = self.eng.zeros(4)
        return self.loss_log

    def new_frame(self, row_index, row_mask=None, zero=True):
        self.rows = row_index
        self.call_token = self._next_token()
        self.gs.row_mask = row_mask
        self.adam = optim.Adam(self.eng)
        if zero:
            self.gs.zero_()
        self._nat_dirty = True

    def begin_frame(self):
        self.gs.zero_()


class TrackOptimizer:

    def __init__(self, eng, cfg, dec, knn, pos, geo_feats, col_feats, R, cam_lr, separate_lr=True, w_color=0.5,
                 use_color=True, dynamic_radius=False, dist=None, handle_dynamic=True, shard_rays=False):
        self.eng, self.cfg, self.dec, self.knn = eng, cfg, dec, knn
        self.pos, self.geo, self.col = pos, geo_feats, col_feats
        self.R, self.cam_lr, self.separate_lr = R, cam_lr, separate_lr
        self.w_color, self.use_color = w_color, use_color
        self.handle_dynamic = handle_dynamic
        self.shard_rays = bool(shard_rays and dist is not None and dist.world > 1)
        self.R_own = R
        if self.shard_rays:
            from . import parallel
            self.own = parallel.ray_range(R, dist.rank, dist.world, 1)
            self.R_own = max(1, max(parallel.ray_range(R, r, dist.world, 1)[1] - parallel.ray_range(R, r, dist.world, 1)[0] for r in range(dist.world)))
        self.batch = RayBatch(eng, self.R_own, dynamic_radius)
        self.st = core.RenderState(eng, self.R_own, cfg.S, need_act=True)
        self.gs = core.GradState(eng, geo_feats.shape[0], self.R_own, dec.n, feats=False, weights=False, rays=True)
        self.g_cam = eng.zeros(7)
        self.eye = None
        self.dist = dist
        self.native_loop = not self.shard_rays

    def track(self, cam7_init, depth_img, color_img, iters, window, intr, rnd_all, r2_map=None, exposure=None):
        eng, b, st, gs = self.eng, self.batch, self.st, self.gs
        H, W = depth_img.shape
        cam = cam7_init.clone().contiguous()
        adam = optim.Adam(eng)
        xs = None
        if exposure is not None:
            xs = ExposureState(eng, exposure[0], exposure[1])
            if gs.g_affine is None:
                gs.g_affine = eng.zeros(12)
        log = eng.zeros(iters, 4)
        hist = eng.empty(iters, 7)
        if self.native_loop:
            self._track_native(cam, depth_img, color_img, iters, window, intr, rnd_all, r2_map, hist, log, xs)
            best = torch.argmin(log[:, 0])
            return self._agree(hist.index_select(0, best.reshape(1))[0], xs), log
        if self.eye is None:
            self.eye = torch.eye(4, device=eng.device).reshape(1, 4, 4).contiguous()
        dstack, cstack = depth_img.reshape(1, H, W), color_img.reshape(1, H, W, 3)
        r2s = r2_map.reshape(1, H, W) if r2_map is not None else None
        xch = eng.zeros(7 + 4 + 12) if self.shard_rays else None
        for it in range(iters):
            if self.separate_lr:
                hist[it].copy_(cam)
            draws = rnd_all[it]
            if self.shard_rays:
                lo, hi = self.own
                draws = draws[lo:hi] if hi > lo else draws[:1]
                if draws.shape[0] < self.R_own:
                    draws = torch.cat([draws, draws[-1:].expand(self.R_own - draws.shape[0])])
                draws = draws.contiguous()
            optim.gather_rays(eng, dstack, cstack, self.eye, None, draws, H, W, window, intr, b.as_out(), r2s)
            if self.shard_rays and hi - lo < self.R_own:
                b.gt_depth[max(hi - lo, 0):].zero_()
            optim.rays_from_pose(eng, cam, b.pix_i, b.pix_j, intr, b.rays_o, b.rays_d)
            optim.inside_mask(eng, b.gt_depth, None, b.thr, b.scratch_u32, depth_filtered=b.gt_depth)
            aff = None
            if xs is not None:
                aff = xs.forward()[0]
                gs.g_affine.zero_()
            core.render_forward(eng, self.cfg, st, b.rays_o, b.rays_d, b.gt_depth, self.knn, self.pos, self.geo, self.col,
                                self.dec, 'color', tracker=True, r2_ray=b.r2_ray, save_act=True, affine=aff,
                                extra_flags=_ffi.FLAG_ZERO_ABSENT)
            optim.loss_tracker(eng, st, b.gt_depth, b.gt_color, self.w_color, self.use_color, b.d_depth, b.d_color,
                               log[it], b.loss_scratch, handle_dynamic=self.handle_dynamic)
            core.render_backward(eng, st, gs, b.d_depth, b.d_color)
            optim.pose_bwd(eng, cam, b.pix_i, b.pix_j, intr, gs.g_rays_o, gs.g_rays_d, self.g_cam)
            if self.shard_rays:
                xch[:7].copy_(self.g_cam); xch[7:11].copy_(log[it])
                if xs is not None:
                    xch[11:].copy_(gs.g_affine)
                self.dist.all_reduce_vec(xch)
                self.g_cam.copy_(xch[:7]); log[it].copy_(xch[7:11])
                if xs is not None:
                    gs.g_affine.copy_(xch[11:])
            if self.separate_lr:
                segs = [('T', cam[4:7], self.g_cam[4:7], self.cam_lr), ('q', cam[0:4], self.g_cam[0:4], 0.2 * self.cam_lr)]
            else:
                segs = [('cam', cam, self.g_cam, self.cam_lr)]
            if xs is not None:
                xs.backward(gs.g_affine)
                segs = segs + xs.adam_segs()
            adam.step(segs)
            if not self.separate_lr:
                hist[it].copy_(cam)
        best = torch.argmin(log[:, 0])
        return self._agree(hist.index_select(0, best.reshape(1))[0], xs), log

    def _agree(self, cam7, xs=None):
        if self.dist is not None:
            self.dist.broadcast(cam7, src=0)
            if xs is not None:
                for t in (xs.feats, xs.W1, xs.b1, xs.W2, xs.b2):
                    self.dist.broadcast(t, src=0)
        return cam7

    def _track_native(self, cam, depth_img, color_img, iters, window, intr, rnd_all, r2_map, hist, log, xs=None):
        eng, b, st, gs = self.eng, self.batch, self.st, self.gs
        H, W = depth_img.shape
        H0, H1, W0, W1 = window
        core.fill_desc(eng, self.cfg, st, b.rays_o, b.rays_d, b.gt_depth, self.knn, self.pos, self.geo, self.col, self.dec, 'color',
                       tracker=True, r2_ray=b.r2_ray, save_act=True, extra_flags=_ffi.FLAG_ZERO_ABSENT)
        flags = st.desc.flags | _ffi.FLAG_GRAD_RAYS
        need = int(eng.lib.dll.lk_render_bwd_scratch_floats(self.R, self.cfg.S, flags))
        if gs.scratch is None or gs.scratch.numel() < need:
            gs.scratch = eng.empty(max(1, need))
        d = _ffi.TrackDesc()
        C = _ffi.C
        C.memmove(C.byref(d.render), C.byref(st.desc), C.sizeof(_ffi.RenderDesc))
        r = d.render
        r.flags = (_ffi.FLAG_REL_POS if self.cfg.rel_pos else 0) | (_ffi.FLAG_FEATS_F16 if self.geo.dtype == torch.float16 else 0)
        r.d_depth, r.d_color = ptr(b.d_depth), ptr(b.d_color)
        r.g_rays_o, r.g_rays_d, r.bwd_scratch, r.bwd_scratch_cap = ptr(gs.g_rays_o), ptr(gs.g_rays_d), ptr(gs.scratch), gs.scratch.numel()
        d.depth_img, d.color_img, d.r2_map = ptr(depth_img), ptr(color_img), ptr(r2_map)
        d.H, d.W, d.H0, d.W0, d.w = H, W, H0, W0, W1 - W0
        d.fx, d.fy, d.cx, d.cy = intr
        rnd_all = rnd_all.contiguous()
        assert rnd_all.dtype == torch.int32 and rnd_all.shape[0] >= iters and rnd_all.shape[1] == self.R
        d.rnd, d.gt_color, d.pix_i, d.pix_j = ptr(rnd_all), ptr(b.gt_color), ptr(b.pix_i), ptr(b.pix_j)
        d.thr, d.scratch_u32, d.loss_scratch = ptr(b.thr), ptr(b.scratch_u32), ptr(b.loss_scratch)
        if getattr(self, 'adam_mv', None) is None:
            self.adam_mv = eng.zeros(14)
        d.cam7, d.g_cam7, d.adam_mv = ptr(cam), ptr(self.g_cam), ptr(self.adam_mv)
        d.lr_T, d.lr_q = self.cam_lr, (0.2 * self.cam_lr if self.separate_lr else self.cam_lr)
        d.w_color, d.use_color, d.hist_post = self.w_color, optim.track_loss_flags(self.use_color, self.handle_dynamic), int(not self.separate_lr)
        d.hist, d.log, d.iters = ptr(hist), ptr(log), iters
        need = int(eng.lib.dll.lk_track_work_floats(self.R, self.cfg.S, iters)) if self.R <= 8192 else 0
        if need and (getattr(self, '_work', None) is None or self._work.numel() < need):
            self._work = eng.empty(need)
        d.work = ptr(self._work) if need else 0
        if xs is not None:
            d.exposure = C.pointer(xs.desc(ExposureState.LR))
        self._keep_native = (depth_img, color_img, r2_map, rnd_all, cam, hist, log, xs)
        eng.lib.check(eng.lib.dll.lk_track_frame(C.byref(d), eng.stream), 'lk_track_frame')
```

Baseline: 20.34 million rays/s.

## Fuse geometry-stage row Adam step into feature scatter and skip gradient zeroing

```diff
diff --git a/include/loopy_hip.h b/include/loopy_hip.h
--- a/include/loopy_hip.h
+++ b/include/loopy_hip.h
@@ -270,6 +270,7 @@
     int32_t batches_ready;
     int32_t train_geo_decoder;
     int32_t signal_rows;
+    uint8_t* row_step_flags;
 } lk_map_desc;
 int64_t lk_map_work_floats(int32_t R, int32_t S, int32_t iters);
 int lk_map_prepare(const lk_map_desc* d, void* stream);
diff --git a/loopy_slam_amd/_ffi.py b/loopy_slam_amd/_ffi.py
--- a/loopy_slam_amd/_ffi.py
+++ b/loopy_slam_amd/_ffi.py
@@ -117,6 +117,7 @@
         ('grad_bucket', _fp), ('bucket_geo_dec', C.c_int64 * MAX_SPANS), ('bucket_col_dec', C.c_int64 * MAX_SPANS),
         ('bucket_geo_rows', C.c_int64), ('bucket_col_rows', C.c_int64),
         ('union_rows_flagged', C.c_int32), ('it_offset', C.c_int32), ('batches_ready', C.c_int32), ('train_geo_decoder', C.c_int32), ('signal_rows', C.c_int32),
+        ('row_step_flags', _fp),
     ]
 
 
diff --git a/loopy_slam_amd/csrc/lk_adam_dev.h b/loopy_slam_amd/csrc/lk_adam_dev.h
--- a/loopy_slam_amd/csrc/lk_adam_dev.h
+++ b/loopy_slam_amd/csrc/lk_adam_dev.h
@@ -9,8 +9,7 @@
     return p - step_size * (m / denom);
 }
 
-__device__ __forceinline__ void lk_adam_one(const AdamSegDev& S, long long i, long long e, float b1, float b2, float eps) {
-    const float g = S.g[S.g_compact ? i : e];
+__device__ __forceinline__ void lk_adam_at(const AdamSegDev& S, long long i, long long e, float g, float b1, float b2, float eps) {
     float m = S.m[i], v = S.v[i];
     if (S.p_f16) {
         _Float16* ph = reinterpret_cast<_Float16*>(S.p) + e;
@@ -20,6 +19,9 @@
     }
     S.m[i] = m;
     S.v[i] = v;
+}
+__device__ __forceinline__ void lk_adam_one(const AdamSegDev& S, long long i, long long e, float b1, float b2, float eps) {
+    lk_adam_at(S, i, e, S.g[S.g_compact ? i : e], b1, b2, eps);
     if (S.zero_grad && !S.g_compact) S.g[e] = 0.0f;
 }
 __device__ __forceinline__ void lk_adam_seg_flagged(const AdamSegDev& S, float b1, float b2, float eps, int bx, int gx) {
@@ -47,6 +49,13 @@
         }
     }
 }
+__device__ __forceinline__ void lk_adam_seg_gap_rows(const AdamSegDev& S, float b1, float b2, float eps, int bx, int gx) {
+    for (long long i = (long long)bx * 256 + threadIdx.x; i < S.n; i += (long long)gx * 256) {
+        const long long row = i / S.row_len;
+        if (!S.row_flags[row]) continue;
+        lk_adam_at(S, i, (long long)S.row_index[row] * S.row_len + (i - row * S.row_len), 0.0f, b1, b2, eps);
+    }
+}
 __device__ __forceinline__ void lk_adam_seg_block(const AdamSegDev& S, float b1, float b2, float eps, int bx, int gx) {
     if (S.row_flags) { lk_adam_seg_flagged(S, b1, b2, eps, bx, gx); return; }
     for (long long i = (long long)bx * 256 + threadIdx.x; i < S.n; i += (long long)gx * 256) {
diff --git a/loopy_slam_amd/csrc/lk_api.hip b/loopy_slam_amd/csrc/lk_api.hip
--- a/loopy_slam_amd/csrc/lk_api.hip
+++ b/loopy_slam_amd/csrc/lk_api.hip
@@ -592,6 +592,8 @@
             fs.dw2_blocks = lk_dw2_parts(P); fs.dw2_live = ex ? ex->live_rays : nullptr; fs.dw2_S = d->S;
         }
         if (ex && ex->xstep) { fs.x_on = 1; fs.x = *ex->xstep; }
+        if (ex && ex->row_step) { fs.step = *ex->row_step; fs.act_flag = nullptr; }
+        if (ex && ex->red_step && bg_rides) fs.red_step = *ex->red_step;
         lk_launch_feat_scatter(fs, st);
         if (ex && ex->signal_rows) {
             const int rc3 = rows_event_record(st);
diff --git a/loopy_slam_amd/csrc/lk_bwd2.hip b/loopy_slam_amd/csrc/lk_bwd2.hip
--- a/loopy_slam_amd/csrc/lk_bwd2.hip
+++ b/loopy_slam_amd/csrc/lk_bwd2.hip
@@ -148,6 +148,8 @@
     const long long i = (long long)blockIdx.x * 256 + (int)threadIdx.x;
     const int y = (int)blockIdx.y;
     const int32_t* __restrict__ off = a.seg_off + (size_t)y * a.cnt_stride;
+    if (a.gap_flags)
+        for (long long key = i; key < a.N; key += (long long)gridDim.x * 256) a.gap_flags[(size_t)y * a.N + key] = off[key + 1] == off[key] ? 1 : 0;
     if (i >= off[a.N]) return;
     const long long base = (long long)y * a.P * LK_K;
     const int32_t* __restrict__ tmp = a.seg_tmp + base;
@@ -213,7 +215,18 @@
 __device__ __forceinline__ void col_reduce_body(const float* __restrict__ part, int n_parts, int width, float* __restrict__ out, int bx, float (*sh)[32],
                                                 const LkStepRider& sr);
 __device__ __forceinline__ void lk_arrived(float v) { asm volatile("" : : "v"(v)); }
-template <int MODE>
+template <bool COL, bool STEP>
+__device__ __forceinline__ void feat_flush(const LkFeatScatterArgs& a, int point, int key, int c, float sg, float sc) {
+    const long long e = (long long)point * LK_C + c;
+    if (STEP) {
+        lk_adam_at(a.step.tab, (long long)key * LK_C + c, e, 0.0f + sg, a.step.beta1, a.step.beta2, a.step.eps);
+    } else {
+        atomicAdd(a.g_geo_feats + e, sg);
+        if (COL) atomicAdd(a.g_col_feats + e, sc);
+        if (a.act_flag && c == 0) a.act_flag[point] = 1;
+    }
+}
+template <int MODE, bool STEP>
 __device__ __forceinline__ void feat_walk(const LkFeatScatterArgs& a, int bx) {
     constexpr bool col = MODE != 0;
     const int c = (int)threadIdx.x & 31;
@@ -223,12 +236,14 @@
     const int i0 = (int)i0l, e = min(i0 + LK_GATHER_CHUNK, total);
     const float* __restrict__ tab_c = MODE == 2 ? a.dfeat : a.dc_col;
     int cur = -1, carry = -1;
+    int curk = -1;
     float sg = 0.0f, sc = 0.0f;
     for (int wb = i0;; wb += LK_GATHER_WINDOW) {
         const int row = a.seg_list[min(wb + c, total - 1)];
         const int before = (wb == i0 && c == 0 && i0 > 0) ? a.seg_list[i0 - 1] : -1;
         const int pt = a.nbr_idx[row];
         const float w = a.nbr_w[row];
+        const int ky = STEP ? a.step.key_of[pt] : -1;
         if (before >= 0) carry = a.nbr_idx[before];
         int prev = __shfl_up(pt, 1, 32);
         if (c == 0) prev = carry;
@@ -254,17 +269,18 @@
                 vg[k] = a.dc_geo[s];
                 if (col) vc[k] = tab_c[MODE == 2 ? (size_t)r * LK_C + c : s];
             }
-            int fp[LK_GATHER_BATCH];
+            int fp[LK_GATHER_BATCH], fk[LK_GATHER_BATCH];
             float fg[LK_GATHER_BATCH], fc[LK_GATHER_BATCH];
 #pragma unroll
             for (int k = 0; k < LK_GATHER_BATCH; ++k) {
                 const int u = ub + k;
                 const int pu = __shfl(pt, min(u, LK_GATHER_WINDOW - 1), 32);
-                fp[k] = -1; fg[k] = 0.0f; fc[k] = 0.0f;
+                const int ku = STEP ? __shfl(ky, min(u, LK_GATHER_WINDOW - 1), 32) : -1;
+                fp[k] = -1; fk[k] = -1; fg[k] = 0.0f; fc[k] = 0.0f;
                 if (u >= u1) continue;
                 if ((m >> u) & 1u) {
-                    fp[k] = cur; fg[k] = sg; fc[k] = sc;
-                    cur = pu; sg = 0.0f; sc = 0.0f;
+                    fp[k] = cur; fk[k] = curk; fg[k] = sg; fc[k] = sc;
+                    cur = pu; curk = ku; sg = 0.0f; sc = 0.0f;
                 }
                 sg += wr[k] * vg[k];
                 if (col) sc += MODE == 1 ? wr[k] * vc[k] : vc[k];
@@ -273,18 +289,12 @@
             if (col) lk_arrived(vc[LK_GATHER_BATCH - 1]);
 #pragma unroll
             for (int k = 0; k < LK_GATHER_BATCH; ++k)
-                if (fp[k] >= 0) {
-                    atomicAdd(a.g_geo_feats + (size_t)fp[k] * LK_C + c, fg[k]);
-                    if (col) atomicAdd(a.g_col_feats + (size_t)fp[k] * LK_C + c, fc[k]);
-                    if (a.act_flag && c == 0) a.act_flag[fp[k]] = 1;
-                }
+                if (fp[k] >= 0) feat_flush<col, STEP>(a, fp[k], fk[k], c, fg[k], fc[k]);
         }
         if (tail) break;
         carry = __shfl(pt, LK_GATHER_WINDOW - 1, 32);
     }
-    atomicAdd(a.g_geo_feats + (size_t)cur * LK_C + c, sg);
-    if (col) atomicAdd(a.g_col_feats + (size_t)cur * LK_C + c, sc);
-    if (a.act_flag && c == 0) a.act_flag[cur] = 1;
+    feat_flush<col, STEP>(a, cur, curk, c, sg, sc);
 }
 __global__ __launch_bounds__(256) void k_feat_gather(LkFeatScatterArgs a) {
     const int xb = a.x_on ? 1 : 0;
@@ -293,16 +303,21 @@
         dw2_body(a.dw2_dc, a.dw2_w_sum, a.dw2_hbar, a.P, a.dw2_live, a.dw2_S, a.dw2_part, (int)blockIdx.x - xb, a.dw2_blocks);
         return;
     }
-    const int bx = (int)blockIdx.x - xb - a.dw2_blocks;
+    int bx = (int)blockIdx.x - xb - a.dw2_blocks;
+    const int n_red = a.red_part ? (a.red_width + 31) / 32 : 0;
+    if (bx >= a.red_block0 + n_red) {
+        lk_adam_seg_gap_rows(a.step.tab, a.step.beta1, a.step.beta2, a.step.eps, bx - a.red_block0 - n_red, a.step.rider_blocks);
+        return;
+    }
     if (a.red_part && bx >= a.red_block0) {
         __shared__ float sh[8][32];
-        LkStepRider none; none.n_span = 0;
-        col_reduce_body(a.red_part, a.red_n, a.red_width, a.red_out, bx - a.red_block0, sh, none);
+        col_reduce_body(a.red_part, a.red_n, a.red_width, a.red_out, bx - a.red_block0, sh, a.red_step);
         return;
     }
-    if (a.dfeat) feat_walk<2>(a, bx);
-    else if (a.dc_col) feat_walk<1>(a, bx);
-    else feat_walk<0>(a, bx);
+    if (a.dfeat) feat_walk<2, false>(a, bx);
+    else if (a.dc_col) feat_walk<1, false>(a, bx);
+    else if (a.step.on) feat_walk<0, true>(a, bx);
+    else feat_walk<0, false>(a, bx);
 }
 
 __global__ __launch_bounds__(256) void k_rays_bwd(LkRaysBwdArgs a) {
@@ -1301,7 +1316,9 @@
     LkFeatScatterArgs b = a;
     b.red_block0 = lk_cdiv((long long)a.P * LK_K, 8 * LK_GATHER_CHUNK);
     if (!b.dw2_part) b.dw2_blocks = 0;
-    hipLaunchKernelGGL(k_feat_gather, dim3((b.x_on ? 1 : 0) + b.dw2_blocks + b.red_block0 + (a.red_part ? lk_cdiv(a.red_width, 32) : 0)), dim3(256), 0, st, b);
+    if (!b.step.on) b.step.rider_blocks = 0;
+    hipLaunchKernelGGL(k_feat_gather, dim3((b.x_on ? 1 : 0) + b.dw2_blocks + b.step.rider_blocks + b.red_block0 + (a.red_part ? lk_cdiv(a.red_width, 32) : 0)),
+                       dim3(256), 0, st, b);
     return LK_OK;
 }
 int lk_launch_seg_sort(const LkFeatScatterArgs& a, bool counted, hipStream_t st, int batch) {
diff --git a/loopy_slam_amd/csrc/lk_kernels.h b/loopy_slam_amd/csrc/lk_kernels.h
--- a/loopy_slam_amd/csrc/lk_kernels.h
+++ b/loopy_slam_amd/csrc/lk_kernels.h
@@ -172,6 +172,13 @@
     float beta1, beta2, eps;
     AdamSegDev feat[2]; int n_feat, feat_gx;
 };
+struct LkRowStep {
+    int on;
+    AdamSegDev tab;
+    float beta1, beta2, eps;
+    const int32_t* key_of;
+    int rider_blocks;
+};
 struct ExposureStepArgs;
 struct LkBwdExtra { float* pose_part; const float* pix_i; const float* pix_j; float fx, fy, cx, cy;
                     int32_t* seg_list; int32_t* seg_total; const int32_t* live_rays; const LkStepRider* step; const float* dscale;
@@ -179,7 +186,9 @@
                     float* loss_rows;
                     int split_reduce; float* split_frag; float* split_master; int* split_done;
                     const ExposureStepArgs* xstep;
-                    const float* xstep_part; int xstep_n_part; };
+                    const float* xstep_part; int xstep_n_part;
+                    const LkRowStep* row_step;
+                    const LkStepRider* red_step; };
 inline int lk_bwd_pose_parts(int64_t P) { return (int)((P + 31) / 32); }
 
 struct ExposureStepArgs {
@@ -204,12 +213,15 @@
     int32_t* seg_total;
     int cnt_stride, sums_stride;
     const float* red_part; int red_n, red_width, red_block0; float* red_out;
+    LkStepRider red_step;
     int x_on; ExposureStepArgs x;
     const float* dw2_dc; const float* dw2_w_sum; const float* dw2_hbar; float* dw2_part; int dw2_blocks; const int32_t* dw2_live; int dw2_S;
     const int32_t* live_rays; int S;
     int N;
     uint8_t* act_flag;
     const int32_t* key_of;
+    LkRowStep step;
+    uint8_t* gap_flags;
 };
 int lk_launch_seg_sort(const LkFeatScatterArgs& a, bool counted, hipStream_t st, int batch = 1);
 int lk_launch_scan_i32(int32_t* data, int32_t* out, int32_t* block_sums, int total, hipStream_t st,
diff --git a/loopy_slam_amd/csrc/lk_loop.hip b/loopy_slam_amd/csrc/lk_loop.hip
--- a/loopy_slam_amd/csrc/lk_loop.hip
+++ b/loopy_slam_amd/csrc/lk_loop.hip
@@ -493,6 +493,10 @@
     if (pre && it_begin == 0 && (phases & 1) && !d->batches_ready) map_join_and_pregather(d, wk, R, xd, st);
     const bool sort_ahead = pre && d->render.g_geo_feats != nullptr;
     const bool key_rows = sort_ahead && d->rows != nullptr && kn_h->row_rank != nullptr && d->n_rows > 0;
+    const bool row_step = d->row_step_flags != nullptr && pre && (phases & 3) == 3 && sort_ahead && key_rows && !act_rows;
+    bool geo_span_rides = row_step && d->train_geo_decoder == 0 && d->render.weights == d->weights_rw && d->render.g_weights != nullptr && nb < (1ll << 31);
+    for (int k = 0; k < d->n_geo_dec; ++k)
+        geo_span_rides = geo_span_rides && d->geo_dec[k].offset >= G_EB && d->geo_dec[k].offset + d->geo_dec[k].n <= G_EB + 288;
     auto enqueue_chunk = [&](int c) -> int {
         const int c0 = chunk_start(c);
         if (c0 >= d->iters) return LK_OK;
@@ -530,6 +534,7 @@
             fs.seg_list = reinterpret_cast<int32_t*>(W0 + wk.seg_list) + (size_t)it * Pn * LK_K;
             fs.seg_total = reinterpret_cast<int32_t*>(W0 + wk.seg_total) + it;
             fs.live_rays = reinterpret_cast<const int32_t*>(W0 + wk.n_live) + it; fs.S = d->render.S;
+            if (row_step && it < n_geo_l) fs.gap_flags = d->row_step_flags + (size_t)it * d->n_rows;
             rc = lk_launch_seg_sort(fs, counted, pst, nbatch);
             if (rc != LK_OK) return rc;
         }
@@ -544,7 +549,7 @@
         const int rc = enqueue_chunk(0);
         if (rc != LK_OK) return rc;
     }
-    auto build_segs = [&](int it, bool color, lk_adam_seg* seg, int& ns) -> bool {
+    auto build_segs = [&](int it, bool color, lk_adam_seg* seg, int& ns, bool with_rows) -> bool {
         const float* lr = d->lr[color ? 1 : 0];
         ns = 0;
         auto dec_seg = [&](const lk_blob_span& sp, int step) {
@@ -554,6 +559,7 @@
         };
         for (int k = 0; k < d->n_geo_dec; ++k) dec_seg(d->geo_dec[k], goff + it + 1);
         if (color) for (int k = 0; k < d->n_col_dec; ++k) dec_seg(d->col_dec[k], it - n_geo_l + 1);
+        if (!with_rows) return true;
         if (ns + 2 > LK_ADAM_MAX_SEG) return false;
         {
             lk_adam_seg& s = seg[ns++];
@@ -672,7 +678,7 @@
                 lk_adam_seg seg[LK_ADAM_MAX_SEG];
                 memset(seg, 0, sizeof(seg));
                 int ns = 0;
-                LK_REQUIRE(build_segs(it, color, seg, ns), "lk_map_frame: too many optimiser segments");
+                LK_REQUIRE(build_segs(it, color, seg, ns, true), "lk_map_frame: too many optimiser segments");
                 memset(&sr, 0, sizeof(sr));
                 sr.g = d->render.g_weights; sr.p = d->weights_rw; sr.w_next = W0 + wk.w_next; sr.m = d->adam_dec; sr.v = d->adam_dec + nb;
                 sr.beta1 = beta1; sr.beta2 = beta2; sr.eps = eps;
@@ -708,14 +714,43 @@
                 ex.xstep = &xa_early;
                 x_early = true;
             }
+            LkRowStep rs;
+            if (row_step && !color) {
+                lk_adam_seg seg[LK_ADAM_MAX_SEG];
+                memset(seg, 0, sizeof(seg));
+                int ns = 0;
+                LK_REQUIRE(build_segs(it, color, seg, ns, true), "lk_map_frame: too many optimiser segments");
+                memset(&rs, 0, sizeof(rs));
+                const lk_adam_seg& q = seg[ns - 1];
+                AdamSegDev& f = rs.tab;
+                f.p = q.p; f.g = nullptr; f.m = q.m; f.v = q.v; f.n = q.n; f.row_index = q.row_index; f.row_len = LK_C; f.p_f16 = q.p_f16;
+                adam_scalars(q.lr, q.step, beta1, beta2, &f.step_size, &f.bc2_sqrt);
+                f.row_flags = d->row_step_flags + (size_t)it * d->n_rows;
+                rs.on = 1; rs.beta1 = beta1; rs.beta2 = beta2; rs.eps = eps; rs.key_of = kn_h->row_rank;
+                rs.rider_blocks = lk_cdiv(q.n, 256) > 2048 ? 2048 : lk_cdiv(q.n, 256);
+                ex.row_step = &rs;
+            }
+            LkStepRider gsr;
+            if (geo_span_rides && !color && d->n_geo_dec > 0) {
+                memset(&gsr, 0, sizeof(gsr));
+                gsr.g = d->render.g_weights; gsr.p = d->weights_rw; gsr.w_next = d->weights_rw; gsr.m = d->adam_dec; gsr.v = d->adam_dec + nb;
+                gsr.beta1 = beta1; gsr.beta2 = beta2; gsr.eps = eps; gsr.feat_gx = 1;
+                for (int k = 0; k < d->n_geo_dec; ++k) {
+                    LkStepSpan& sp = gsr.span[gsr.n_span++];
+                    sp.off = (int)d->geo_dec[k].offset; sp.n = (int)d->geo_dec[k].n;
+                    adam_scalars(d->lr[0][0], goff + it + 1, beta1, beta2, &sp.step_size, &sp.bc2_sqrt);
+                }
+                ex.red_step = &gsr;
+            }
             rc = lk_render_bwd_impl(&rd, st, (xit ? 0 : LK_SKIP_COMPOSITE_BWD) | LK_SEG_SORTED | (comp_bwd ? LK_COMPOSITE_IN_BWD : 0), pre ? &ex : nullptr);
             if (rc != LK_OK) return rc;
         }
         if (phases & 2) {
+            if (geo_span_rides && !color) continue;
             lk_adam_seg seg[LK_ADAM_MAX_SEG];
             memset(seg, 0, sizeof(seg));
             int ns = 0;
-            LK_REQUIRE(build_segs(it, color, seg, ns), "lk_map_frame: too many optimiser segments");
+            LK_REQUIRE(build_segs(it, color, seg, ns, color || !row_step), "lk_map_frame: too many optimiser segments");
             if (d->grad_bucket && (phases & 3) == 2) {
                 LK_REQUIRE(d->rows != nullptr && !xd, "lk_map_frame: grad_bucket needs a row list and no exposure encoding");
                 int q = 0;
diff --git a/loopy_slam_amd/steps.py b/loopy_slam_amd/steps.py
--- a/loopy_slam_amd/steps.py
+++ b/loopy_slam_amd/steps.py
@@ -146,6 +146,9 @@
         self.native_loop = True
         self.max_call_iters = int(os.environ.get('LOOPY_MAX_CALL_ITERS', '384'))
         self._work = None
+        self.row_step = os.environ.get('LOOPY_ROW_STEP', '1') != '0'
+        self._row_flags = None
+        self._rows_clean = False
         self._nat, self._nat_dirty = None, False
         self._prepared = None
         self.exposure = ExposureState(eng, exposure[0], exposure[1]) if exposure is not None else None
@@ -161,6 +164,7 @@
 
     def iterate(self, stage, frames, rnd, frame_id, window, intr, H, W, log_row=None):
         eng, b, st, gs = self.eng, self.batch, self.st, self.gs
+        self._rows_clean = False
         depth_stack, color_stack, c2w_stack, r2_stack = frames
         optim.gather_rays(eng, depth_stack, color_stack, c2w_stack, frame_id, rnd, H, W, window, intr, b.as_out(), r2_stack)
         optim.inside_mask(eng, b.gt_depth, None, b.thr, b.scratch_u32, depth_filtered=b.gt_depth)
@@ -256,7 +260,7 @@
         self._prepared = None
         if not self._takes_native_loop() or self.dist is not None or self.R > 16384:
             return False
-        self.gs.zero_()
+        self._zero_grads()
         d, seg_iters = self._native_desc(n_iters, n_geo_iters, frames, rnd_all, frame_id, window, intr, H, W, log, rows_known=False)
         d.iters, d.it_offset = min(seg_iters, n_iters), 0
         self.eng.lib.check(self.eng.lib.dll.lk_map_prepare(_ffi.C.byref(d), self.eng.stream), 'lk_map_prepare')
@@ -329,6 +333,14 @@
         if need and (self._work is None or self._work.numel() < need):
             self._work = eng.empty(need)
         d.work = ptr(self._work) if need else 0
+        d.row_step_flags = 0
+        if rows_known:
+            if self.row_step and self.dist is None and need and self.rows is not None and n_rows > 0:
+                if self._row_flags is None or self._row_flags.numel() < seg_iters * n_rows:
+                    self._row_flags = eng.empty(seg_iters * n_rows, dtype=torch.uint8)
+                d.row_step_flags = ptr(self._row_flags)
+            else:
+                self._rows_clean = False
         d.union_rows_flagged = 1 if (self.dist is not None and self.rows is None and self.geo.shape[0] <= self.knn.capacity) else 0
         self._nat_lists = (int(eng.lib.dll.lk_map_work_nbr_idx(self.R, self.cfg.S, n_iters)), n_iters) if need else None
         self._keep_native = (depth_stack, color_stack, c2w_stack, r2_stack, frame_id, rnd_all, log)
@@ -360,11 +372,21 @@
         self.gs.row_mask = row_mask
         self.adam = optim.Adam(self.eng)
         if zero:
-            self.gs.zero_()
+            self._zero_grads()
         self._nat_dirty = True
 
     def begin_frame(self):
-        self.gs.zero_()
+        self._zero_grads()
+
+    def _zero_grads(self):
+        gs = self.gs
+        if self._rows_clean:
+            for t in (gs.g_weights, gs.g_affine):
+                if t is not None:
+                    t.zero_()
+        else:
+            gs.zero_()
+            self._rows_clean = True
 
 
 class TrackOptimizer:
```

New measurement: 20.26 million rays/s. No clear change (-0.4%).
